# Shadowfear36/SegHiero

Hardware: AMD Instinct MI355X
Metric: images/sec at 512x512 (ResNet-50 2-level), full train step (higher is better)
Workload: dtype f32 (convolutions: exact 3-way bf16 split of every fp32 operand, 6 bf16 MFMA products, f32 accumulate; rest plain f32)

## Files before the change

### include/seghiero_hip.h

```cpp
#ifndef SEGHIERO_HIP_H
#define SEGHIERO_HIP_H
#include <stdint.h>
#ifdef __cplusplus
extern "C" {
#endif

#define SH_OK 0
#define SH_EINVAL (-1)
#define SH_ELAUNCH (-2)
#define SH_EUNSUPPORTED (-3)

int sh_abi_version(void);
int sh_conv_tile_rows(void);

int sh_nchw_to_nhwc(const float* x, float* y, int N, int C, int H, int W, int Cpad, void* stream);
int sh_nhwc_to_nchw(const float* x, float* y, int N, int C, int H, int W, int Cpad, void* stream);

int sh_ingest_image_u8(const uint8_t* rgb, float* out, const uint8_t* flip, int N, int H, int W,
                       const float* mean3_host, const float* std3_host, void* stream);
int sh_resize_bilinear_coeffs(int in_size, int out_size, int* bounds, int* kk, int kk_capacity);
int sh_resize_bilinear_u8(const uint8_t* src, uint8_t* tmp, uint8_t* dst, int N, int H, int W, int Ho, int Wo,
                          const int* bounds_x, const int* kk_x, int ksize_x, const int* bounds_y, const int* kk_y,
                          int ksize_y, void* stream);
int sh_ingest_mask(const void* mask, int is_i64, uint8_t* out, const uint8_t* flip, int N, int Hs, int Ws, int H,
                   int W, void* stream);

int sh_conv_fprop(const float* x, int ldx, const float* w, const float* bias, float* y, int ldy,
                  float* stat_partials, int N, int H, int W, int Cin, int Cout, int KH, int KW,
                  int stride, int pad, int dil, void* stream);
int sh_conv_dgrad(const float* dy, int lddy, const float* w, const float* addend, int ldadd,
                  float* dx, int lddx, int N, int H, int W, int Cin, int Cout, int KH, int KW,
                  int stride, int pad, int dil, int mode, void* stream);
int64_t sh_conv_wgrad_workspace(int N, int H, int W, int Cin, int Cout, int KH, int KW,
                                int stride, int pad, int dil);
int sh_conv_wgrad(const float* x, int ldx, const float* dy, int lddy, float* dw, float* workspace,
                  int N, int H, int W, int Cin, int Cout, int KH, int KW, int stride, int pad,
                  int dil, void* stream);

int64_t sh_conv_x6_workspace(int which , int N, int H, int W, int Cin, int Cout, int KH, int KW,
                             int stride, int pad, int dil, int dgrad_mode);
int sh_conv_fprop_x6(const float* x, int ldx, const float* w, const float* bias, float* y, int ldy,
                     float* stat_partials, int N, int H, int W, int Cin, int Cout, int KH, int KW,
                     int stride, int pad, int dil, float* workspace, int64_t workspace_bytes, int act_flags, void* stream);
int sh_conv_fprop_x6_act(const float* x, int ldx, const float* w, const float* scale, const float* shift,
                         const float* residual, int ldr, int relu, float* out, int ldo, int N, int H, int W,
                         int Cin, int Cout, int KH, int KW, int stride, int pad, int dil, void* stream);
int sh_conv_fprop_x6_aff(const float* x, int ldx, const float* in_scale, const float* in_shift, const float* w,
                         const float* bias, float* y, int ldy, float* stat_partials, int N, int H, int W, int Cin, int Cout,
                         int KH, int KW, int stride, int pad, int dil, float* workspace, int64_t workspace_bytes, int act_flags,
                         void* stream);
int sh_conv1x1_grouped_fprop_x6(int ngroups, const float* const* x, const int* ldx, const float* const* in_scale,
                                const float* const* in_shift, const float* const* w, float* y, int ldy,
                                float* stat_partials, int N, int H, int W, int Cin, int Cout, void* stream);
int sh_weight_transpose(const float* w, float* wt, int Cout, int KH, int KW, int Cin, void* stream);
#define SH_WT_MAX 40
int sh_weight_transpose_multi(int n, const float* const* w, float* const* wt, const int* cout, const int* taps,
                              const int* cin, void* stream);
int sh_conv_dgrad_x6(const float* dy, int lddy, const float* wt, const float* addend, int ldadd,
                     float* dx, int lddx, int N, int H, int W, int Cin, int Cout, int KH, int KW,
                     int stride, int pad, int dil, int mode, float* workspace, int64_t workspace_bytes,
                     void* stream);
int sh_conv_dgrad_x6_bnb(const float* dy, int lddy, const float* wt, const float* addend, int ldadd, float* g, int ldg,
                         const float* y_prev, int ldyp, const float* out_prev, int ldop, const float* mean,
                         const float* invstd, const float* scale, const float* shift, int relu, float* stat_partials,
                         int N, int H, int W, int Cin, int Cout,
                         int KH, int KW, int stride, int pad, int dil, float* workspace, int64_t workspace_bytes, int act_flags,
                         void* stream);
int sh_conv_dgrad_x6_lin(const float* g, int ldg, const float* y, int ldy, const float* lin, const float* wt, const float* addend,
                         int ldadd, float* dx, int lddx, const float* y_prev, int ldyp, const float* mean, const float* invstd,
                         const float* scale, const float* shift, int relu, float* stat_partials, int N, int H, int W, int Cin,
                         int Cout, float* workspace, int64_t workspace_bytes, int act_flags, void* stream);
int sh_conv_wgrad_x6_lin(const float* x, int ldx, const float* in_scale, const float* in_shift, const float* g, int ldg,
                         const float* y, int ldy, const float* lin, float* dw, float* workspace, int N, int H, int W, int Cin,
                         int Cout, int KH, int KW, int stride, int pad, int dil, int act_flags, void* stream);
int64_t sh_conv_wgrad_x6_workspace(int N, int H, int W, int Cin, int Cout, int KH, int KW,
                                   int stride, int pad, int dil);
int sh_conv_wgrad_x6(const float* x, int ldx, const float* dy, int lddy, float* dw, float* workspace,
                     int N, int H, int W, int Cin, int Cout, int KH, int KW, int stride, int pad,
                     int dil, int act_flags, void* stream);
int sh_conv_wgrad_x6_aff(const float* x, int ldx, const float* in_scale, const float* in_shift, const float* dy, int lddy,
                         float* dw, float* workspace, int N, int H, int W, int Cin, int Cout, int KH, int KW,
                         int stride, int pad, int dil, int act_flags, void* stream);

int sh_dw_partials(int N, int H, int W);
int sh_dw_tile_rows(void);
int sh_dwconv_fprop(const float* x, int ldx, const float* in_scale, const float* in_shift, const float* w, float* y, int ldy,
                    float* stat_partials, int N, int H, int W, int C, int dil, int act_flags, void* stream);
int sh_dwconv_dgrad(const float* dy, int lddy, const float* y_lin, int ldyl, const float* lin, const float* w, float* dx, int lddx,
                    int N, int H, int W, int C, int dil, int accumulate, int act_flags, void* stream);
int sh_dwconv_dgrad_bnb(const float* dy, int lddy, const float* y_lin, int ldyl, const float* lin, const float* w, float* g, int ldg,
                        const float* y_prev, int ldyp, const float* mean, const float* invstd, const float* scale, const float* shift,
                        float* stat_partials, int N, int H, int W, int C, int dil, int act_flags, void* stream);
int sh_dwconv_wgrad(const float* x, int ldx, const float* in_scale, const float* in_shift, const float* dy, int lddy,
                    const float* y_lin, int ldyl, const float* lin, float* dw_partials, float* dw, int N, int H, int W, int C, int dil,
                    int act_flags, void* stream);

int sh_bn_finalize(const float* partials, int n_partials, int C, double count, const float* gamma,
                   const float* beta, float eps, float momentum, float* running_mean,
                   float* running_var, float* mean, float* invstd, float* scale, float* shift,
                   int rows_per_partial, int partials_ld, void* stream);
int sh_bn_finalize_scaled(const float* partials, int n_partials, int C, double count, const float* chan_mul,
                          int chan_stride, const float* gamma, const float* beta, float eps, float momentum,
                          float* running_mean, float* running_var, float* mean, float* invstd, float* scale,
                          float* shift, float* isy, int rows_per_partial, void* stream);
int sh_bn_finalize_multi(int k, const float* partials, int n_partials, int C, double count, int rows_per_partial,
                         int partials_ld, const int* partials_col, const float* const* gamma, const float* const* beta,
                         float* const* running_mean, float* const* running_var, float* const* mean, float* const* invstd,
                         float* const* scale, float* const* shift, const float* const* chan_mul, int chan_stride,
                         float* const* isy, float eps, float momentum, void* stream);
int sh_dw_center_wgrad(const float* dgamma, const float* gamma, const float* isy, const float* w, float eps, float* dw,
                       int C, const float* g, int ldg, const float* x, int ldx, const float* mean_x, int64_t M, void* stream);
int sh_bn_fold_partials(const float* partials, int n_partials, int C, double count, int rows_per_partial, int chunk,
                        float* out, void* stream);
int sh_bn_reduce_partials(const float* partials, int n_partials, int C, double count, int rows_per_partial, double* sq,
                          void* stream);
int sh_bn_finalize_sq(const double* sq, int C, const float* gamma, const float* beta, float eps,
                      float momentum, float* running_mean, float* running_var, float* mean, float* invstd,
                      float* scale, float* shift, void* stream);
int sh_bn_bwd_finalize_sq(const double* local_sq, const double* global_sq, int C, float* dgamma,
                          float* dbeta, float* c1, float* c2, const float* gamma, const float* invstd, const float* mean,
                          float* lin, void* stream);
int sh_bn_eval_coefs(const float* gamma, const float* beta, const float* running_mean,
                     const float* running_var, float eps, int C, float* scale, float* shift, void* stream);
int sh_stats_partials_count(int64_t M);
int sh_stats_tile_rows(void);
int sh_channel_stats(const float* y, int ldy, int64_t M, int C, float* partials, void* stream);
int sh_bn_act(const float* y, int ldy, const float* scale, const float* shift, const float* residual,
              int ldr, const float* res_scale, const float* res_shift, float* out, int ldo, int64_t M, int C, int relu,
              uint8_t* relu_mask, int act_flags, void* stream);
int sh_bn_bwd_reduce(const float* dout, int lddo, const float* out, int ldo, const float* y, int ldy,
                     const float* mean, const float* invstd, const float* scale, const float* shift,
                     float* partials, int64_t M, int C, int relu, float* g_out, int ldg, int act_flags, void* stream);
int sh_bn_bwd_finalize(const float* partials, int n_partials, int C, const float* gamma,
                       const float* invstd, double count, float* dgamma, float* dbeta, float* c1,
                       float* c2, const float* mean, float* lin, void* stream);
int sh_bn_bwd_apply(const float* dout, int lddo, const float* out, int ldo, const float* y, int ldy,
                    const float* mean, const float* invstd, const float* scale, const float* shift,
                    const float* gamma, const float* c1, const float* c2, float* dy, int lddy, float* dres,
                    int lddres, int64_t M, int C, int relu, int act_flags, void* stream);

int sh_maxpool_fwd(const float* x, const float* in_scale, const float* in_shift, float* y, uint8_t* argmax, int N, int H,
                   int W, int C, int act_flags, void* stream);
int sh_maxpool_bwd(const uint8_t* argmax, const float* dy, float* dx, int N, int H, int W, int C, void* stream);
int sh_avgpool_fwd(const float* x, int ldx, float* y, int N, int HW, int C, void* stream);
int sh_avgpool_bwd(const float* dy, float* dx, int lddx, int N, int HW, int C, float scale, int accumulate, void* stream);
int sh_broadcast_hw(const float* x, float* y, int ldy, int N, int HW, int C, void* stream);
int sh_sum_hw(const float* dy, int lddy, float* dx, int N, int HW, int C, void* stream);
int sh_bilinear_fwd(const float* x, int ldx, float* y, int ldy, int N, int h, int w, int H, int W, int C, int act_flags, void* stream);
int64_t sh_bilinear_bwd_workspace(int N, int h, int w, int C);
int sh_bilinear_bwd(const float* dy, int lddy, float* dx, int lddx, int N, int h, int w, int H, int W, int C, float* workspace,
                    int64_t workspace_bytes, void* stream);
int sh_l2norm_fwd(const float* x, float* y, float* norm, int64_t M, int C, void* stream);
int sh_l2norm_bwd(const float* dy, const float* y, const float* norm, float* dx, int64_t M, int C, void* stream);

int sh_hiera2_partials(int N, int H, int W);
int sh_label_counts(const uint8_t* labels, const int* buckets_host, int n_fine, int n_coarse, int64_t total, int64_t* counts,
                    void* stream);
int sh_hiera2_loss_fwd(const float* logits, int ldl, const uint8_t* labels, const int* buckets_host, int n_fine,
                       int n_coarse, double* sums, float* loss_out, float* partials, uint8_t* coarse_out,
                       int N, int h, int w, int H, int W, float* grad_out, int64_t grad_out_bytes, int ldg,
                       const int64_t* norm_counts, void* stream);
int64_t sh_loss_bwd_workspace(int N, int H, int W, int lddl);
int sh_hiera2_loss_bwd(const float* logits, int ldl, const uint8_t* labels, const int* buckets_host, int n_fine,
                       int n_coarse, const double* sums, const float* gscale_dev, float gscale, float* dlogits,
                       int lddl, int N, int h, int w, int H, int W, float* workspace, int64_t workspace_bytes,
                       int workspace_has_grad, void* stream);
int sh_ce_loss_fwd(const float* logits, int ldl, const uint8_t* labels, int C, double* sums, float* loss_out,
                   float* partials, int N, int h, int w, int H, int W, float* grad_out, int64_t grad_out_bytes, int ldg,
                   const int64_t* norm_count, void* stream);
int sh_ce_loss_bwd(const float* logits, int ldl, const uint8_t* labels, int C, const double* sums,
                   const float* gscale_dev, float gscale, float* dlogits, int lddl, int N, int h, int w, int H,
                   int W, float* workspace, int64_t workspace_bytes, int workspace_has_grad,
                   void* stream);
int sh_labels_to_u8(const int64_t* in, uint8_t* out, int64_t n, void* stream);
int64_t sh_triplet_workspace(int64_t M);
int sh_triplet_fwd(const float* emb, const uint8_t* labels, const uint64_t* masks, const uint64_t* anchor_ok,
                   int max_triplet, float margin, float* out, void* workspace, int N, int h, int w, int D, int H,
                   int W, void* stream);
int sh_triplet_bwd(const float* emb, const void* workspace, const float* out, const float* gscale_dev, float gscale,
                   float* demb, int N, int h, int w, int D, void* stream);
int sh_combine_loss(const float* main_loss, const float* trip_out, const float* ready_count, float factor,
                    float loss_weight, float* out, void* stream);
int sh_hiera3_loss_fwd(const float* logits, int ldl, const uint8_t* labels, const int* f2m_host, const int* f2h_host,
                       int n_fine, int n_mid, int n_high, double* sums, float* loss_out, float* partials, float* probs,
                       uint8_t* mid_out, uint8_t* high_out, int N, int h, int w, int H, int W, float* grad_out,
                       int64_t grad_out_bytes, int ldg, void* stream);
int64_t sh_rmi_workspace(int N, int C, int H, int W);
int64_t sh_rmi_values_offset(int N, int C, int H, int W);
int sh_rmi_loss(const float* probs, const uint8_t* labels, const int* f2m_host, const int* f2h_host, int n_fine, int n_mid,
                int n_high, void* workspace, float* rmi_out, float* dprob, int N, int H, int W, void* stream);
int sh_hiera3_loss_bwd(const float* logits, int ldl, const uint8_t* labels, const int* f2m_host, const int* f2h_host,
                       int n_fine, int n_mid, int n_high, const double* sums, const float* dprob, float rmi_coef,
                       const float* gscale_dev, float gscale, float* dlogits, int lddl, int N, int h, int w, int H, int W,
                       float* workspace, int64_t workspace_bytes, int workspace_has_grad, const float* probs, void* stream);
int sh_scalar_axpy(const float* a, const float* b, float alpha, float* out, void* stream);

int sh_pixel_metrics(const float* logits, int ldl, const uint8_t* labels, int n_fine, long long* counts,
                     int N, int h, int w, int H, int W, void* stream);

#define SH_SGD_MAX 48
int sh_sgd_step(int n_tensors, float* const* w, const float* const* g, float* const* v, const int64_t* numel,
                float lr, float momentum, float weight_decay, int first_step, float gscale, void* stream);

int sh_fill(float* p, float v, int64_t n, void* stream);
int sh_axpy(float* y, const float* x, float a, int64_t n, void* stream);
int sh_copy(void* dst, const void* src, int64_t bytes, void* stream);

int sh_weights_to_bf16_multi(int n, const float* const* w, void* const* wb, void* const* wtb, const int* cout, const int* taps,
                             const int* cin, void* stream);
int sh_conv_fprop_b16(const void* x, int ldx, const float* in_scale, const float* in_shift, const void* w_bf16, const float* bias,
                      void* y, int ldy, float* stat_partials, int N, int H, int W, int Cin, int Cout, int KH, int KW, int stride,
                      int pad, int dil, float* workspace, int64_t workspace_bytes, int act_flags, void* stream);
int sh_conv1x1_grouped_fprop_b16(int ngroups, const void* const* x, const int* ldx, const float* const* in_scale,
                                 const float* const* in_shift, const void* const* w_bf16, void* y, int ldy, float* stat_partials,
                                 int N, int H, int W, int Cin, int Cout, int act_flags, void* stream);
int sh_conv_dgrad_b16(const void* dy, int lddy, const void* y_lin, int ldyl, const float* lin, const void* wt_bf16, const void* addend,
                      int ldadd, void* dx, int lddx, const void* y_prev, int ldyp, const void* out_prev, int ldop, const float* mean,
                      const float* invstd, const float* scale, const float* shift, int relu, float* stat_partials, int N, int H,
                      int W, int Cin, int Cout, int KH, int KW, int stride, int pad, int dil, float* workspace,
                      int64_t workspace_bytes, int act_flags, void* stream);
int sh_conv_wgrad_b16(const void* x, int ldx, const float* in_scale, const float* in_shift, const void* dy, int lddy, const void* y_lin,
                      int ldyl, const float* lin, float* dw, float* workspace, int N, int H, int W, int Cin, int Cout, int KH, int KW,
                      int stride, int pad, int dil, int act_flags, void* stream);

int sh_comm_unique_id(void* id128);
int sh_comm_init(const void* id128, int world, int rank, void** comm_out);
int sh_comm_destroy(void* comm);
int sh_comm_all_reduce(void* comm, void* buf, int64_t count, int dtype, int op, void* stream);
int sh_comm_all_reduce_async(void* comm, void* buf, int64_t count, int dtype, int op, void* producer_stream);
int sh_comm_wait(void* comm, void* consumer_stream);
int sh_comm_broadcast(void* comm, void* buf, int64_t bytes, int root, void* stream);

#ifdef __cplusplus
}
#endif
#endif
```

### seghiero_amd/csrc/common.h

```cpp
#pragma once
#include <hip/hip_runtime.h>
#include <stdint.h>
#include "../../include/seghiero_hip.h"

typedef float f32x4 __attribute__((ext_vector_type(4)));
typedef float f32x16 __attribute__((ext_vector_type(16)));

#define SH_WAVE 64

static inline int sh_launch_status() {
    hipError_t e = hipGetLastError();
    return e == hipSuccess ? SH_OK : SH_ELAUNCH;
}

static inline int64_t sh_cdiv(int64_t a, int64_t b) { return (a + b - 1) / b; }

__device__ __forceinline__ float wave_sum(float v) {
#pragma unroll
    for (int o = 32; o > 0; o >>= 1) v += __shfl_xor(v, o, 64);
    return v;
}
__device__ __forceinline__ double wave_sum_d(double v) {
#pragma unroll
    for (int o = 32; o > 0; o >>= 1) v += __shfl_xor(v, o, 64);
    return v;
}

__device__ __forceinline__ unsigned xcd_remap(unsigned bid, unsigned nblk) {
    const unsigned q = nblk >> 3, r = nblk & 7u, xcd = bid & 7u, loc = bid >> 3;
    const unsigned base = xcd < r ? xcd * (q + 1) : r * (q + 1) + (xcd - r) * q;
    return base + loc;
}

__device__ __forceinline__ f32x4 ld4(const float* p) { return *reinterpret_cast<const f32x4*>(p); }
__device__ __forceinline__ void st4(float* p, f32x4 v) { *reinterpret_cast<f32x4*>(p) = v; }

typedef unsigned int sh_u32x2 __attribute__((ext_vector_type(2)));
__device__ __forceinline__ f32x4 bf16x4_to_f32(sh_u32x2 v) {
    return f32x4{__uint_as_float(v[0] << 16), __uint_as_float(v[0] & 0xffff0000u), __uint_as_float(v[1] << 16), __uint_as_float(v[1] & 0xffff0000u)};
}
__device__ __forceinline__ unsigned f32_to_bf16_rne(float f) {
    const unsigned u = __float_as_uint(f);
    return (f != f) ? ((u >> 16) | 0x40u) : ((u + 0x7fffu + ((u >> 16) & 1u)) >> 16);
}
__device__ __forceinline__ sh_u32x2 f32_to_bf16x4(f32x4 v) {
    return sh_u32x2{f32_to_bf16_rne(v[0]) | (f32_to_bf16_rne(v[1]) << 16), f32_to_bf16_rne(v[2]) | (f32_to_bf16_rne(v[3]) << 16)};
}
__device__ __forceinline__ f32x4 lda4(const float* base, long long idx, int bf) {
    if (bf) return bf16x4_to_f32(*reinterpret_cast<const sh_u32x2*>(reinterpret_cast<const unsigned short*>(base) + idx));
    return ld4(base + idx);
}
__device__ __forceinline__ unsigned quad_mask_bits(f32x4 v) {
    return (v[0] > 0.f ? 1u : 0u) | (v[1] > 0.f ? 2u : 0u) | (v[2] > 0.f ? 4u : 0u) | (v[3] > 0.f ? 8u : 0u);
}
__device__ __forceinline__ f32x4 quad_mask_load(const void* base, long long byte_idx) {
    const unsigned b = reinterpret_cast<const unsigned char*>(base)[byte_idx];
    return f32x4{(b & 1u) ? 1.f : 0.f, (b & 2u) ? 1.f : 0.f, (b & 4u) ? 1.f : 0.f, (b & 8u) ? 1.f : 0.f};
}
__device__ __forceinline__ void sta4(float* base, long long idx, f32x4 v, int bf) {
    if (bf) *reinterpret_cast<sh_u32x2*>(reinterpret_cast<unsigned short*>(base) + idx) = f32_to_bf16x4(v);
    else st4(base + idx, v);
}

struct sh_f8 { f32x4 lo, hi; };
typedef unsigned int sh_u32x4 __attribute__((ext_vector_type(4)));
__device__ __forceinline__ sh_f8 lda8(const float* base, long long idx, int bf) {
    sh_f8 r;
    if (bf) {
        const sh_u32x4 v = *reinterpret_cast<const sh_u32x4*>(reinterpret_cast<const unsigned short*>(base) + idx);
        r.lo = bf16x4_to_f32(sh_u32x2{v[0], v[1]}); r.hi = bf16x4_to_f32(sh_u32x2{v[2], v[3]});
    } else { r.lo = ld4(base + idx); r.hi = ld4(base + idx + 4); }
    return r;
}
__device__ __forceinline__ void sta8(float* base, long long idx, const sh_f8& v, int bf) {
    if (bf) {
        const sh_u32x2 a = f32_to_bf16x4(v.lo), b = f32_to_bf16x4(v.hi);
        *reinterpret_cast<sh_u32x4*>(reinterpret_cast<unsigned short*>(base) + idx) = sh_u32x4{a[0], a[1], b[0], b[1]};
    } else { st4(base + idx, v.lo); st4(base + idx + 4, v.hi); }
}
```

### seghiero_amd/csrc/dwconv.hip

```cpp
#include "common.h"
#include <stdlib.h>

#define DW_PIX 64
#define DW_CH 64

__device__ __forceinline__ f32x4 dw_in(const float* p, const float* isc, const float* ish, int c) {
    f32x4 v = ld4(p);
    if (isc != nullptr) {
        v = v * ld4(isc + c) + ld4(ish + c);
        v[0] = fmaxf(v[0], 0.f); v[1] = fmaxf(v[1], 0.f); v[2] = fmaxf(v[2], 0.f); v[3] = fmaxf(v[3], 0.f);
    }
    return v;
}

struct DwBnb { const float* y; long long ldy; const float* mean; const float* invstd; const float* scale; const float* shift; float* partials;
               int y_bf; };
struct DwBnbC { f32x4 scale, shift, mean, invstd; };
__device__ __forceinline__ DwBnbC dw_bnb_coefs(const DwBnb& b, int c, bool cok) {
    DwBnbC k; k.scale = k.shift = k.mean = k.invstd = f32x4{0.f, 0.f, 0.f, 0.f};
    if (b.y != nullptr && cok) { k.scale = ld4(b.scale + c); k.shift = ld4(b.shift + c); k.mean = ld4(b.mean + c); k.invstd = ld4(b.invstd + c); }
    return k;
}
__device__ __forceinline__ f32x4 dw_bnb_apply(const DwBnbC& k, f32x4 yv, f32x4 dx, f32x4& sg, f32x4& sq) {
    const f32x4 a = yv * k.scale + k.shift;
#pragma unroll
    for (int j = 0; j < 4; ++j) if (!(a[j] > 0.f)) dx[j] = 0.f;
    sg += dx;
    sq += dx * ((yv - k.mean) * k.invstd);
    return dx;
}
__device__ __forceinline__ f32x4 dw_bnb_apply(const DwBnb& b, long long m, int c, f32x4 dx, f32x4& sg, f32x4& sq) {
    const f32x4 yv = lda4(b.y, m * b.ldy + c, b.y_bf);
    const f32x4 a = yv * ld4(b.scale + c) + ld4(b.shift + c);
#pragma unroll
    for (int j = 0; j < 4; ++j) if (!(a[j] > 0.f)) dx[j] = 0.f;
    sg += dx;
    sq += dx * ((yv - ld4(b.mean + c)) * ld4(b.invstd + c));
    return dx;
}
__device__ __forceinline__ void dw_bnb_store(const DwBnb& b, float (*red)[64], f32x4 sg, f32x4 sq, long long pidx, int C, int c0, int t, int cq, int pl) {
#pragma unroll
    for (int pass = 0; pass < 2; ++pass) {
        __syncthreads();
#pragma unroll
        for (int j = 0; j < 4; ++j) red[pl][cq * 4 + j] = pass == 0 ? sg[j] : sq[j];
        __syncthreads();
        if (t < 64 && c0 + t < C) {
            float a = 0.f;
#pragma unroll
            for (int k = 0; k < 16; ++k) a += red[k][t];
            b.partials[(pidx * 2 + pass) * C + c0 + t] = a;
        }
    }
}

extern "C" int sh_dw_partials(int N, int H, int W) { return (int)sh_cdiv((long long)N * H * W, DW_PIX); }
extern "C" int sh_dw_tile_rows(void) { return DW_PIX; }

template <int MODE>
__global__ __launch_bounds__(256) void dwconv_kernel(const float* __restrict__ x, long long ldx, const float* __restrict__ w,
                                                     float* __restrict__ y, long long ldy, float* __restrict__ partials,
                                                     int H, int W, int C, int dil, long long M, int accumulate,
                                                     const float* __restrict__ isc, const float* __restrict__ ish, const DwBnb bnb) {
    __shared__ float ws[9][DW_CH];
    __shared__ float red[16][DW_CH];
    __shared__ float colmean[DW_CH];
    const int t = threadIdx.x, cq = t & 15, pl = t >> 4;
    const int c0 = blockIdx.y * DW_CH;
    for (int i = t; i < 9 * DW_CH; i += 256) {
        const int tap = i / DW_CH, cc = i % DW_CH;
        const int src_tap = MODE == 0 ? tap : 8 - tap;
        ws[tap][cc] = (c0 + cc < C) ? w[(long long)(c0 + cc) * 9 + src_tap] : 0.f;
    }
    __syncthreads();
    const int c = c0 + cq * 4;
    const bool cok = c < C;
    f32x4 s = {0.f, 0.f, 0.f, 0.f};
    f32x4 bsg = s, bsq = s;
    f32x4 kept[DW_PIX / 16];
    bool kept_ok[DW_PIX / 16];
    const bool tap_row_ok = dil < H, tap_col_ok = dil < W;
#pragma unroll
    for (int it = 0; it < DW_PIX / 16; ++it) {
        const long long m = (long long)blockIdx.x * DW_PIX + it * 16 + pl;
        kept_ok[it] = false;
        kept[it] = f32x4{0.f, 0.f, 0.f, 0.f};
        if (m < M && cok) {
            const int ow = (int)(m % W);
            const long long r = m / W;
            const int oh = (int)(r % H);
            const long long n = r / H;
            f32x4 acc = {0.f, 0.f, 0.f, 0.f};
#pragma unroll
            for (int kh = 0; kh < 3; ++kh) {
                if (kh != 1 && !tap_row_ok) continue;
                const int ih = oh + (kh - 1) * dil;
                if ((unsigned)ih >= (unsigned)H) continue;
#pragma unroll
                for (int kw = 0; kw < 3; ++kw) {
                    if (kw != 1 && !tap_col_ok) continue;
                    const int iw = ow + (kw - 1) * dil;
                    if ((unsigned)iw >= (unsigned)W) continue;
                    const f32x4 v = dw_in(x + ((n * H + ih) * W + iw) * ldx + c, isc, ish, c);
                    const f32x4 wv = ld4(&ws[kh * 3 + kw][cq * 4]);
                    acc += v * wv;
                }
            }
            if (MODE == 1 && accumulate) acc += ld4(y + m * ldy + c);
            if (MODE == 1 && bnb.y != nullptr) acc = dw_bnb_apply(bnb, m, c, acc, bsg, bsq);
            st4(y + m * ldy + c, acc);
            s += acc; kept[it] = acc; kept_ok[it] = true;
        }
    }
    if (MODE == 1 && bnb.y != nullptr) dw_bnb_store(bnb, red, bsg, bsq, blockIdx.x, C, c0, t, cq, pl);
    if (MODE == 0 && partials != nullptr) {
        const long long left = M - (long long)blockIdx.x * DW_PIX;
        const float nvalid = (float)(left < DW_PIX ? left : DW_PIX);
#pragma unroll
        for (int j = 0; j < 4; ++j) red[pl][cq * 4 + j] = s[j];
        __syncthreads();
        float colsum = 0.f;
        if (t < DW_CH) {
#pragma unroll
            for (int k = 0; k < 16; ++k) colsum += red[k][t];
            colmean[t] = colsum / nvalid;
        }
        __syncthreads();
        f32x4 q = {0.f, 0.f, 0.f, 0.f};
        const f32x4 mu = ld4(&colmean[cq * 4]);
#pragma unroll
        for (int it = 0; it < DW_PIX / 16; ++it)
            if (kept_ok[it]) { const f32x4 dv = kept[it] - mu; q += dv * dv; }
#pragma unroll
        for (int j = 0; j < 4; ++j) red[pl][cq * 4 + j] = q[j];
        __syncthreads();
        if (t < DW_CH && c0 + t < C) {
            float m2 = 0.f;
#pragma unroll
            for (int k = 0; k < 16; ++k) m2 += red[k][t];
            partials[((long long)blockIdx.x * 2 + 0) * C + c0 + t] = colsum;
            partials[((long long)blockIdx.x * 2 + 1) * C + c0 + t] = m2;
        }
    }
}

#define DT 8
template <int MODE>
__global__ __launch_bounds__(256) void dwconv_tile_kernel(const float* __restrict__ x, long long ldx, const float* __restrict__ w,
                                                          float* __restrict__ y, long long ldy, float* __restrict__ partials,
                                                          int H, int W, int C, int accumulate,
                                                          const float* __restrict__ isc, const float* __restrict__ ish, const DwBnb bnb) {
    __shared__ __attribute__((aligned(16))) float xs[(DT + 2) * (DT + 2)][DW_CH];
    __shared__ float ws[9][DW_CH];
    __shared__ float red[16][DW_CH];
    __shared__ float colmean[DW_CH];
    const int t = threadIdx.x, cq = t & 15, pl = t >> 4;
    const unsigned nch = (unsigned)((C + DW_CH - 1) / DW_CH);
    const unsigned tile = blockIdx.x / nch;
    const int c0 = (int)(blockIdx.x % nch) * DW_CH;
    const int tiles_x = W / DT, tiles_y = H / DT;
    const int tx = tile % tiles_x, ty = (tile / tiles_x) % tiles_y;
    const long long n = tile / (tiles_x * tiles_y);
    for (int i = t; i < 9 * DW_CH; i += 256) {
        const int tap = i / DW_CH, cc = i % DW_CH;
        ws[tap][cc] = (c0 + cc < C) ? w[(long long)(c0 + cc) * 9 + (MODE == 0 ? tap : 8 - tap)] : 0.f;
    }
    const int c = c0 + cq * 4;
    const bool cok = c < C;
    for (int i = pl; i < (DT + 2) * (DT + 2); i += 16) {
        const int hy = i / (DT + 2), hx = i - hy * (DT + 2);
        const int iy = ty * DT + hy - 1, ix = tx * DT + hx - 1;
        f32x4 v = {0.f, 0.f, 0.f, 0.f};
        if (cok && (unsigned)iy < (unsigned)H && (unsigned)ix < (unsigned)W) v = dw_in(x + ((n * H + iy) * W + ix) * ldx + c, isc, ish, c);
        st4(&xs[i][cq * 4], v);
    }
    __syncthreads();
    f32x4 s = {0.f, 0.f, 0.f, 0.f};
    f32x4 bsg = s, bsq = s;
    f32x4 kept[4];
#pragma unroll
    for (int it = 0; it < 4; ++it) {
        const int pidx = it * 16 + pl, py = pidx / DT, px = pidx - py * DT;
        f32x4 acc = {0.f, 0.f, 0.f, 0.f};
#pragma unroll
        for (int kh = 0; kh < 3; ++kh)
#pragma unroll
            for (int kw = 0; kw < 3; ++kw)
                acc += ld4(&xs[(py + kh) * (DT + 2) + px + kw][cq * 4]) * ld4(&ws[kh * 3 + kw][cq * 4]);
        kept[it] = acc;
        if (cok) {
            const long long m = (n * H + ty * DT + py) * W + tx * DT + px;
            float* dst = y + m * ldy + c;
            if (MODE == 1 && accumulate) acc += ld4(dst);
            if (MODE == 1 && bnb.y != nullptr) acc = dw_bnb_apply(bnb, m, c, acc, bsg, bsq);
            st4(dst, acc);
        }
        s += kept[it];
    }
    if (MODE == 1 && bnb.y != nullptr) dw_bnb_store(bnb, red, bsg, bsq, tile, C, c0, t, cq, pl);
    if (MODE == 0 && partials != nullptr) {
#pragma unroll
        for (int j = 0; j < 4; ++j) red[pl][cq * 4 + j] = s[j];
        __syncthreads();
        float colsum = 0.f;
        if (t < DW_CH) {
#pragma unroll
            for (int k = 0; k < 16; ++k) colsum += red[k][t];
            colmean[t] = colsum / (float)(DT * DT);
        }
        __syncthreads();
        f32x4 q = {0.f, 0.f, 0.f, 0.f};
        const f32x4 mu = ld4(&colmean[cq * 4]);
#pragma unroll
        for (int it = 0; it < 4; ++it) { const f32x4 dv = kept[it] - mu; q += dv * dv; }
#pragma unroll
        for (int j = 0; j < 4; ++j) red[pl][cq * 4 + j] = q[j];
        __syncthreads();
        if (t < DW_CH && c0 + t < C) {
            float m2 = 0.f;
#pragma unroll
            for (int k = 0; k < 16; ++k) m2 += red[k][t];
            partials[((long long)tile * 2 + 0) * C + c0 + t] = colsum;
            partials[((long long)tile * 2 + 1) * C + c0 + t] = m2;
        }
    }
}
__global__ __launch_bounds__(256) void dwconv_wgrad_tile_kernel(const float* __restrict__ x, long long ldx, const float* __restrict__ dy,
                                                               long long lddy, float* __restrict__ partials, int H, int W, int C,
                                                               long long ntiles, const float* __restrict__ isc, const float* __restrict__ ish) {
    __shared__ __attribute__((aligned(16))) float xs[(DT + 2) * (DT + 2)][DW_CH];
    __shared__ float red[16][DW_CH];
    const int t = threadIdx.x, cq = t & 15, pl = t >> 4;
    const unsigned nch = (unsigned)((C + DW_CH - 1) / DW_CH), group = blockIdx.x / nch, ngroups = gridDim.x / nch;
    const int c0 = (int)(blockIdx.x % nch) * DW_CH, c = c0 + cq * 4;
    const bool cok = c < C;
    const int tiles_x = W / DT, tiles_y = H / DT;
    f32x4 acc[9];
#pragma unroll
    for (int k = 0; k < 9; ++k) acc[k] = f32x4{0.f, 0.f, 0.f, 0.f};
    for (long long tile = group; tile < ntiles; tile += ngroups) {
        const int tx = (int)(tile % tiles_x), ty = (int)((tile / tiles_x) % tiles_y);
        const long long n = tile / (tiles_x * tiles_y);
        __syncthreads();
        for (int i = pl; i < (DT + 2) * (DT + 2); i += 16) {
            const int hy = i / (DT + 2), hx = i - hy * (DT + 2);
            const int iy = ty * DT + hy - 1, ix = tx * DT + hx - 1;
            f32x4 v = {0.f, 0.f, 0.f, 0.f};
            if (cok && (unsigned)iy < (unsigned)H && (unsigned)ix < (unsigned)W) v = dw_in(x + ((n * H + iy) * W + ix) * ldx + c, isc, ish, c);
            st4(&xs[i][cq * 4], v);
        }
        __syncthreads();
        if (cok) {
#pragma unroll
            for (int it = 0; it < 4; ++it) {
                const int pidx = it * 16 + pl, py = pidx / DT, px = pidx - py * DT;
                const f32x4 g = ld4(dy + ((n * H + ty * DT + py) * W + tx * DT + px) * lddy + c);
#pragma unroll
                for (int kh = 0; kh < 3; ++kh)
#pragma unroll
                    for (int kw = 0; kw < 3; ++kw) acc[kh * 3 + kw] += g * ld4(&xs[(py + kh) * (DT + 2) + px + kw][cq * 4]);
            }
        }
    }
#pragma unroll
    for (int k = 0; k < 9; ++k) {
        __syncthreads();
#pragma unroll
        for (int j = 0; j < 4; ++j) red[pl][cq * 4 + j] = acc[k][j];
        __syncthreads();
        if (t < DW_CH) {
            float a = 0.f;
#pragma unroll
            for (int r = 0; r < 16; ++r) a += red[r][t];
            if (c0 + t < C) partials[((long long)group * 9 + k) * C + c0 + t] = a;
        }
    }
}

#define DWR 10
__device__ __forceinline__ int dw_slot(int base, int k) { const int i = base + k; return i >= DWR ? i - DWR : i; }
struct DwWalk {
    int n, ty, c0, c, tiles_x, tiles_y;
    bool cok;
    long long t0, t1;
};
__device__ __forceinline__ void dw_walk_init(DwWalk& q, int H, int W, int C, int N, int cq) {
    const unsigned nch = (unsigned)((C + DW_CH - 1) / DW_CH), nb = gridDim.x / nch, k = blockIdx.x / nch;
    q.c0 = (int)(blockIdx.x % nch) * DW_CH; q.c = q.c0 + cq * 4; q.cok = q.c < C;
    q.tiles_x = W / DT; q.tiles_y = H / DT;
    const long long T = (long long)N * q.tiles_y * q.tiles_x;
    q.t0 = T * k / nb; q.t1 = T * (k + 1) / nb;
}
__device__ __forceinline__ void dw_walk_strip(DwWalk& q, long long strip) { q.ty = (int)(strip % q.tiles_y); q.n = (int)(strip / q.tiles_y); }
__device__ __forceinline__ bool dw_walk_inside(const DwWalk& q, int H, int W, int hy, int ix) {
    return q.cok && (unsigned)(q.ty * DT + hy - 1) < (unsigned)H && (unsigned)ix < (unsigned)W;
}
__device__ __forceinline__ f32x4 dw_walk_fetch(const float* __restrict__ x, long long ldx, const DwWalk& q, int H, int W, int hy, int ix, int bf = 0) {
    f32x4 v = {0.f, 0.f, 0.f, 0.f};
    if (dw_walk_inside(q, H, W, hy, ix)) v = lda4(x, (((long long)q.n * H + q.ty * DT + hy - 1) * W + ix) * ldx + q.c, bf);
    return v;
}
struct DwLin { const float* y; long long ldy; const float* lin; int y_bf; };
struct DwLinC { f32x4 a, b, mu, d; };
__device__ __forceinline__ DwLinC dw_lin_coefs(const DwLin& L, int C, int c, bool cok) {
    DwLinC k; k.a = k.b = k.mu = k.d = f32x4{0.f, 0.f, 0.f, 0.f};
    if (L.lin != nullptr && cok) { k.a = ld4(L.lin + c); k.b = ld4(L.lin + C + c); k.mu = ld4(L.lin + 2 * C + c); k.d = ld4(L.lin + 3 * C + c); }
    return k;
}
__device__ __forceinline__ f32x4 dw_lin_eval(f32x4 g, f32x4 y, bool inside, const DwLinC& k) {
    f32x4 r;
#pragma unroll
    for (int e = 0; e < 4; ++e) r[e] = inside ? fmaf(y[e] - k.mu[e], k.b[e], fmaf(g[e], k.a[e], k.d[e])) : 0.f;
    return r;
}
__device__ __forceinline__ f32x4 dw_walk_act(f32x4 v, bool aff, bool inside, const f32x4& sc, const f32x4& sh) {
    if (aff && inside) {
        v = v * sc + sh;
        v[0] = fmaxf(v[0], 0.f); v[1] = fmaxf(v[1], 0.f); v[2] = fmaxf(v[2], 0.f); v[3] = fmaxf(v[3], 0.f);
    }
    return v;
}
template <int LIN, int XBF, int YBF>
__device__ __forceinline__ void dw_walk_prologue(float (*xs)[DWR][DW_CH], const float* __restrict__ x, long long ldx, bool aff,
                                                 const f32x4& sc, const f32x4& sh, const DwWalk& q, int H, int W, int tx, int rb, int pl, int cq,
                                                 const DwLin* L = nullptr, const DwLinC* lc = nullptr) {
    for (int i = pl; i < (DT + 2) * (DT + 2); i += 16) {
        const int hy = i / (DT + 2), hx = i - hy * (DT + 2), ix = tx * DT + hx - 1;
        f32x4 v = dw_walk_fetch(x, ldx, q, H, W, hy, ix, XBF);
        if constexpr (LIN) v = dw_lin_eval(v, dw_walk_fetch(L->y, L->ldy, q, H, W, hy, ix, YBF), dw_walk_inside(q, H, W, hy, ix), *lc);
        st4(&xs[hy][dw_slot(rb, hx)][cq * 4], dw_walk_act(v, aff, dw_walk_inside(q, H, W, hy, ix), sc, sh));
    }
}
template <int MODE, int LIN, int BNB, int BF>
__global__ __launch_bounds__(256, (LIN && BNB) ? 2 : 3) void dwconv_walk_kernel(const float* __restrict__ x, long long ldx, const float* __restrict__ w,
                                                          float* __restrict__ y, long long ldy, float* __restrict__ partials,
                                                          int N, int H, int W, int C, int accumulate,
                                                          const float* __restrict__ isc, const float* __restrict__ ish, const DwBnb bnb,
                                                          const DwLin lin, int af) {
    __shared__ __attribute__((aligned(16))) float xs[DT + 2][DWR][DW_CH];
    __shared__ float red[16][DW_CH];
    __shared__ float colmean[DW_CH];
    static_assert(MODE == 1 || (LIN == 0 && BNB == 0), "the loader / epilogue hooks belong to the dgrad");
    constexpr int x_bf = MODE == 0 ? (BF & 1) : 0, y_bf = MODE == 0 ? (BF & 2) : 0, ly_bf = MODE == 1 ? (BF & 1) : 0, by_bf = MODE == 1 ? (BF & 2) : 0;
    constexpr bool has_lin = LIN != 0;
    (void)af;
    const int t = threadIdx.x, cq = t & 15, pl = t >> 4;
    DwWalk q;
    dw_walk_init(q, H, W, C, N, cq);
    const DwLinC lc = dw_lin_coefs(lin, C, q.c, q.cok);
    const DwBnbC bc = dw_bnb_coefs(bnb, q.c, q.cok);
    f32x4 wr[9];
#pragma unroll
    for (int k = 0; k < 9; ++k)
#pragma unroll
        for (int j = 0; j < 4; ++j) wr[k][j] = q.cok ? w[(long long)(q.c + j) * 9 + (MODE == 0 ? k : 8 - k)] : 0.f;
    const bool aff = MODE == 0 && isc != nullptr;
    f32x4 sc = {0.f, 0.f, 0.f, 0.f}, sh = sc;
    if (aff && q.cok) { sc = ld4(isc + q.c); sh = ld4(ish + q.c); }
    int tx = (int)(q.t0 % q.tiles_x), rb = (tx * DT) % DWR;
    for (long long tile = q.t0; tile < q.t1; ++tile) {
        if (tile == q.t0 || tx == 0) {
            dw_walk_strip(q, tile / q.tiles_x);
            dw_walk_prologue<LIN, x_bf, ly_bf>(xs, x, ldx, aff, sc, sh, q, H, W, tx, rb, pl, cq, &lin, &lc);
            __syncthreads();
        }
        f32x4 nx[5];
        [[maybe_unused]] f32x4 ny[5];
        const bool more = tx + 1 < q.tiles_x && tile + 1 < q.t1;
        if (more) {
#pragma unroll
            for (int it = 0; it < 5; ++it) {
                const int i = it * 16 + pl;
                nx[it] = dw_walk_fetch(x, ldx, q, H, W, i >> 3, tx * DT + 9 + (i & 7), x_bf);
                if constexpr (has_lin) ny[it] = dw_walk_fetch(lin.y, lin.ldy, q, H, W, i >> 3, tx * DT + 9 + (i & 7), ly_bf);
            }
        }
        f32x4 s = {0.f, 0.f, 0.f, 0.f};
        f32x4 bsg = s, bsq = s;
        f32x4 kept[4];
#pragma unroll
        for (int it = 0; it < 4; ++it) {
            const int pidx = it * 16 + pl, py = pidx / DT, px = pidx - py * DT;
            f32x4 acc = {0.f, 0.f, 0.f, 0.f};
#pragma unroll
            for (int kh = 0; kh < 3; ++kh)
#pragma unroll
                for (int kw = 0; kw < 3; ++kw)
                    acc += ld4(&xs[py + kh][dw_slot(rb, px + kw)][cq * 4]) * wr[kh * 3 + kw];
            kept[it] = acc;
            if (q.cok) {
                const long long m = (((long long)q.n * H + q.ty * DT + py) * W + tx * DT + px);
                float* dst = y + m * ldy + q.c;
                if (MODE == 1 && accumulate) acc += ld4(dst);
                if constexpr (BNB) acc = dw_bnb_apply(bc, lda4(bnb.y, m * bnb.ldy + q.c, by_bf), acc, bsg, bsq);
                if (MODE == 0) sta4(y, m * ldy + q.c, acc, y_bf);
                else st4(dst, acc);
            }
            s += kept[it];
        }
        if constexpr (BNB) dw_bnb_store(bnb, red, bsg, bsq, tile, C, q.c0, t, cq, pl);
        if (MODE == 0 && partials != nullptr) {
#pragma unroll
            for (int j = 0; j < 4; ++j) red[pl][cq * 4 + j] = s[j];
            __syncthreads();
            float colsum = 0.f;
            if (t < DW_CH) {
#pragma unroll
                for (int k = 0; k < 16; ++k) colsum += red[k][t];
                colmean[t] = colsum / (float)(DT * DT);
            }
            __syncthreads();
            f32x4 qq = {0.f, 0.f, 0.f, 0.f};
            const f32x4 mu = ld4(&colmean[cq * 4]);
#pragma unroll
            for (int it = 0; it < 4; ++it) { const f32x4 dv = kept[it] - mu; qq += dv * dv; }
#pragma unroll
            for (int j = 0; j < 4; ++j) red[pl][cq * 4 + j] = qq[j];
            __syncthreads();
            if (t < DW_CH && q.c0 + t < C) {
                float m2 = 0.f;
#pragma unroll
                for (int k = 0; k < 16; ++k) m2 += red[k][t];
                partials[(tile * 2 + 0) * C + q.c0 + t] = colsum;
                partials[(tile * 2 + 1) * C + q.c0 + t] = m2;
            }
        }
        __syncthreads();
        if (more) {
#pragma unroll
            for (int it = 0; it < 5; ++it) {
                const int i = it * 16 + pl;
                const bool inside = dw_walk_inside(q, H, W, i >> 3, tx * DT + 9 + (i & 7));
                f32x4 v = nx[it];
                if constexpr (has_lin) v = dw_lin_eval(v, ny[it], inside, lc);
                st4(&xs[i >> 3][dw_slot(rb, i & 7)][cq * 4], dw_walk_act(v, aff, inside, sc, sh));
            }
            __syncthreads();
        }
        if (++tx == q.tiles_x) { tx = 0; rb = 0; } else rb = rb >= 2 ? rb - 2 : rb + 8;
    }
}
template <int LIN, int BF>
__global__ __launch_bounds__(256, 3) void dwconv_wgrad_walk_kernel(const float* __restrict__ x, long long ldx, const float* __restrict__ dy,
                                                               long long lddy, float* __restrict__ partials, int N, int H, int W, int C,
                                                               const float* __restrict__ isc, const float* __restrict__ ish, const DwLin lin) {
    constexpr int x_bf = BF & 1, ly_bf = BF & 2;
    __shared__ __attribute__((aligned(16))) float xs[DT + 2][DWR][DW_CH];
    __shared__ float red[16][DW_CH];
    const int t = threadIdx.x, cq = t & 15, pl = t >> 4;
    DwWalk q;
    dw_walk_init(q, H, W, C, N, cq);
    constexpr bool has_lin = LIN != 0;
    const DwLinC lc = dw_lin_coefs(lin, C, q.c, q.cok);
    f32x4 acc[9];
#pragma unroll
    for (int k = 0; k < 9; ++k) acc[k] = f32x4{0.f, 0.f, 0.f, 0.f};
    const bool aff = isc != nullptr;
    f32x4 sc = {0.f, 0.f, 0.f, 0.f}, sh = sc;
    if (aff && q.cok) { sc = ld4(isc + q.c); sh = ld4(ish + q.c); }
    f32x4 g[4];
    [[maybe_unused]] f32x4 gy[4];
    auto fetch_dy = [&](long long tile) {
        const long long strip = tile / q.tiles_x;
        const int ftx = (int)(tile - strip * q.tiles_x), fty = (int)(strip % q.tiles_y);
        const long long fn = strip / q.tiles_y;
#pragma unroll
        for (int it = 0; it < 4; ++it) {
            const int pidx = it * 16 + pl, py = pidx / DT, px = pidx - py * DT;
            const long long m = (fn * H + fty * DT + py) * W + ftx * DT + px;
            g[it] = q.cok ? ld4(dy + m * lddy + q.c) : f32x4{0.f, 0.f, 0.f, 0.f};
            if constexpr (has_lin) gy[it] = q.cok ? lda4(lin.y, m * lin.ldy + q.c, ly_bf) : f32x4{0.f, 0.f, 0.f, 0.f};
        }
    };
    if (q.t0 < q.t1) fetch_dy(q.t0);
    int tx = (int)(q.t0 % q.tiles_x), rb = (tx * DT) % DWR;
    for (long long tile = q.t0; tile < q.t1; ++tile) {
        if (tile == q.t0 || tx == 0) {
            dw_walk_strip(q, tile / q.tiles_x);
            dw_walk_prologue<0, x_bf, 0>(xs, x, ldx, aff, sc, sh, q, H, W, tx, rb, pl, cq);
            __syncthreads();
        }
        f32x4 nx[5];
        const bool more = tx + 1 < q.tiles_x && tile + 1 < q.t1;
        if (more) {
#pragma unroll
            for (int it = 0; it < 5; ++it) {
                const int i = it * 16 + pl;
                nx[it] = dw_walk_fetch(x, ldx, q, H, W, i >> 3, tx * DT + 9 + (i & 7), x_bf);
            }
        }
#pragma unroll
        for (int it = 0; it < 4; ++it) {
            const int pidx = it * 16 + pl, py = pidx / DT, px = pidx - py * DT;
            f32x4 gv = g[it];
            if constexpr (has_lin) gv = dw_lin_eval(g[it], gy[it], q.cok, lc);
#pragma unroll
            for (int kh = 0; kh < 3; ++kh)
#pragma unroll
                for (int kw = 0; kw < 3; ++kw)
                    acc[kh * 3 + kw] += gv * ld4(&xs[py + kh][dw_slot(rb, px + kw)][cq * 4]);
#pragma unroll
            for (int k = 0; k < 9; ++k) asm volatile("" : "+v"(acc[k]));
        }
        if (tile + 1 < q.t1) fetch_dy(tile + 1);
        __syncthreads();
        if (more) {
#pragma unroll
            for (int it = 0; it < 5; ++it) {
                const int i = it * 16 + pl;
                st4(&xs[i >> 3][dw_slot(rb, i & 7)][cq * 4],
                    dw_walk_act(nx[it], aff, dw_walk_inside(q, H, W, i >> 3, tx * DT + 9 + (i & 7)), sc, sh));
            }
            __syncthreads();
        }
        if (++tx == q.tiles_x) { tx = 0; rb = 0; } else rb = rb >= 2 ? rb - 2 : rb + 8;
    }
#pragma unroll
    for (int k = 0; k < 9; ++k) {
        __syncthreads();
#pragma unroll
        for (int j = 0; j < 4; ++j) red[pl][cq * 4 + j] = acc[k][j];
        __syncthreads();
        if (t < DW_CH) {
            float a = 0.f;
#pragma unroll
            for (int r = 0; r < 16; ++r) a += red[r][t];
            if (q.c0 + t < C) partials[((long long)(blockIdx.x / ((C + DW_CH - 1) / DW_CH)) * 9 + k) * C + q.c0 + t] = a;
        }
    }
}

__global__ __launch_bounds__(256) void dwconv_wgrad_kernel(const float* __restrict__ x, long long ldx, const float* __restrict__ dy,
                                                           long long lddy, float* __restrict__ partials, int H, int W, int C,
                                                           int dil, long long M, const float* __restrict__ isc, const float* __restrict__ ish) {
    __shared__ float red[16][DW_CH];
    const int t = threadIdx.x, cq = t & 15, pl = t >> 4;
    const int c0 = blockIdx.y * DW_CH, c = c0 + cq * 4;
    const bool cok = c < C;
    f32x4 acc[9];
#pragma unroll
    for (int k = 0; k < 9; ++k) acc[k] = f32x4{0.f, 0.f, 0.f, 0.f};
    const long long nchunks = (M + DW_PIX - 1) / DW_PIX;
    for (long long chunk = blockIdx.x; chunk < nchunks; chunk += gridDim.x) {
#pragma unroll
        for (int it = 0; it < DW_PIX / 16; ++it) {
            const long long m = chunk * DW_PIX + it * 16 + pl;
            if (m < M && cok) {
                const int ow = (int)(m % W);
                const long long r = m / W;
                const int oh = (int)(r % H);
                const long long n = r / H;
                const f32x4 g = ld4(dy + m * lddy + c);
#pragma unroll
                for (int kh = 0; kh < 3; ++kh) {
                    const int ih = oh + (kh - 1) * dil;
                    if ((unsigned)ih >= (unsigned)H) continue;
#pragma unroll
                    for (int kw = 0; kw < 3; ++kw) {
                        const int iw = ow + (kw - 1) * dil;
                        if ((unsigned)iw >= (unsigned)W) continue;
                        acc[kh * 3 + kw] += g * dw_in(x + ((n * H + ih) * W + iw) * ldx + c, isc, ish, c);
                    }
                }
            }
        }
    }
#pragma unroll
    for (int k = 0; k < 9; ++k) {
        __syncthreads();
#pragma unroll
        for (int j = 0; j < 4; ++j) red[pl][cq * 4 + j] = acc[k][j];
        __syncthreads();
        if (t < DW_CH) {
            float a = 0.f;
#pragma unroll
            for (int r = 0; r < 16; ++r) a += red[r][t];
            if (c0 + t < C) partials[((long long)blockIdx.x * 9 + k) * C + c0 + t] = a;
        }
    }
}
__global__ __launch_bounds__(256) void dwconv_wgrad_reduce_kernel(const float* __restrict__ partials, float* __restrict__ dw, int P, int C) {
    __shared__ double red[4][64];
    const int t = threadIdx.x, cl = t & 63, g = t >> 6;
    const int col = blockIdx.x * 64 + cl;
    double s = 0;
    if (col < 9 * C)
        for (int p = g; p < P; p += 4) s += (double)partials[(long long)p * 9 * C + col];
    red[g][cl] = s;
    __syncthreads();
    if (t < 64 && col < 9 * C) {
        const int tap = col / C, c = col % C;
        dw[(long long)c * 9 + tap] = (float)((red[0][t] + red[1][t]) + (red[2][t] + red[3][t]));
    }
}

template <typename... A>
static void dw_launch_fprop_walk(int bf, unsigned blocks, hipStream_t st, A... a) {
    switch (bf & 3) {
    case 0: dwconv_walk_kernel<0, 0, 0, 0><<<blocks, 256, 0, st>>>(a...); break;
    case 1: dwconv_walk_kernel<0, 0, 0, 1><<<blocks, 256, 0, st>>>(a...); break;
    case 2: dwconv_walk_kernel<0, 0, 0, 2><<<blocks, 256, 0, st>>>(a...); break;
    default: dwconv_walk_kernel<0, 0, 0, 3><<<blocks, 256, 0, st>>>(a...); break;
    }
}
template <int LIN, int BNB, typename... A>
static void dw_launch_dgrad_walk_bf(int bf, unsigned blocks, hipStream_t st, A... a) {
    switch (bf & 3) {
    case 0: dwconv_walk_kernel<1, LIN, BNB, 0><<<blocks, 256, 0, st>>>(a...); break;
    case 1: dwconv_walk_kernel<1, LIN, BNB, 1><<<blocks, 256, 0, st>>>(a...); break;
    case 2: dwconv_walk_kernel<1, LIN, BNB, 2><<<blocks, 256, 0, st>>>(a...); break;
    default: dwconv_walk_kernel<1, LIN, BNB, 3><<<blocks, 256, 0, st>>>(a...); break;
    }
}
template <typename... A>
static void dw_launch_dgrad_walk(bool lin, bool bnb, int bf, unsigned blocks, hipStream_t st, A... a) {
    if (!lin) bf &= ~1;
    if (!bnb) bf &= ~2;
    if (lin && bnb) dw_launch_dgrad_walk_bf<1, 1>(bf, blocks, st, a...);
    else if (lin) dw_launch_dgrad_walk_bf<1, 0>(bf, blocks, st, a...);
    else if (bnb) dw_launch_dgrad_walk_bf<0, 1>(bf, blocks, st, a...);
    else dw_launch_dgrad_walk_bf<0, 0>(bf, blocks, st, a...);
}
template <typename... A>
static void dw_launch_wgrad_walk(bool lin, int bf, unsigned blocks, hipStream_t st, A... a) {
    if (!lin) bf &= ~2;
    if (lin) {
        switch (bf & 3) {
        case 0: dwconv_wgrad_walk_kernel<1, 0><<<blocks, 256, 0, st>>>(a...); break;
        case 1: dwconv_wgrad_walk_kernel<1, 1><<<blocks, 256, 0, st>>>(a...); break;
        case 2: dwconv_wgrad_walk_kernel<1, 2><<<blocks, 256, 0, st>>>(a...); break;
        default: dwconv_wgrad_walk_kernel<1, 3><<<blocks, 256, 0, st>>>(a...); break;
        }
    } else if (bf & 1) dwconv_wgrad_walk_kernel<0, 1><<<blocks, 256, 0, st>>>(a...);
    else dwconv_wgrad_walk_kernel<0, 0><<<blocks, 256, 0, st>>>(a...);
}
static bool dw_walk_on() {
    static const bool on = [] { const char* e = getenv("SEGHIERO_DW_WALK"); return !(e && e[0] == '0'); }();
    return on;
}
static unsigned dw_walk_blocks(int N, int H, int W, int C) { (void)W; (void)C; return (unsigned)(N * (H / DT)); }
static bool dw_args_ok(const void* a, const void* b, const void* c, int N, int H, int W, int C, int dil, int ld1, int ld2) {
    return a && b && c && N > 0 && H > 0 && W > 0 && C > 0 && (C & 3) == 0 && dil > 0 && ld1 >= C && ld2 >= C && !(ld1 & 3) && !(ld2 & 3);
}
extern "C" int sh_dwconv_fprop(const float* x, int ldx, const float* in_scale, const float* in_shift, const float* w, float* y, int ldy,
                               float* stat_partials, int N, int H, int W, int C, int dil, int act_flags, void* stream) {
    if (!dw_args_ok(x, w, y, N, H, W, C, dil, ldx, ldy) || (act_flags & ~3)) return SH_EINVAL;
    if (act_flags && !(dil == 1 && H % DT == 0 && W % DT == 0 && dw_walk_on())) return SH_EUNSUPPORTED;
    if ((in_scale == nullptr) != (in_shift == nullptr) || (((uintptr_t)in_scale | (uintptr_t)in_shift) & 15)) return SH_EINVAL;
    const long long M = (long long)N * H * W;
    dim3 grid((unsigned)sh_cdiv(M, DW_PIX), (unsigned)sh_cdiv(C, DW_CH));
    if (dil == 1 && H % DT == 0 && W % DT == 0 && dw_walk_on())
        dw_launch_fprop_walk(act_flags, dw_walk_blocks(N, H, W, C) * grid.y, (hipStream_t)stream, x, (long long)ldx, w, y, (long long)ldy, stat_partials, N, H, W, C, 0, in_scale,
                             in_shift, DwBnb{}, DwLin{}, act_flags);
    else if (dil == 1 && H % DT == 0 && W % DT == 0)
        dwconv_tile_kernel<0><<<grid.x * grid.y, 256, 0, (hipStream_t)stream>>>(x, ldx, w, y, ldy, stat_partials, H, W, C, 0, in_scale, in_shift, DwBnb{});
    else
        dwconv_kernel<0><<<grid, 256, 0, (hipStream_t)stream>>>(x, ldx, w, y, ldy, stat_partials, H, W, C, dil, M, 0, in_scale, in_shift, DwBnb{});
    return sh_launch_status();
}
static bool dw_lin_args_ok(const float* y_lin, int ldyl, const float* lin, int C) {
    return (lin == nullptr && y_lin == nullptr) || (lin && y_lin && ldyl >= C && !(ldyl & 3) && !(((uintptr_t)y_lin | (uintptr_t)lin) & 15));
}
static int dw_dgrad_any(const float* dy, int lddy, const float* w, float* dx, int lddx, int N, int H, int W, int C, int dil, int accumulate,
                        const DwBnb& bnb, void* stream, const DwLin lin = DwLin{}) {
    const long long M = (long long)N * H * W;
    dim3 grid((unsigned)sh_cdiv(M, DW_PIX), (unsigned)sh_cdiv(C, DW_CH));
    if (dil == 1 && H % DT == 0 && W % DT == 0 && dw_walk_on())
        dw_launch_dgrad_walk(lin.lin != nullptr, bnb.y != nullptr, (lin.y_bf ? 1 : 0) | (bnb.y_bf ? 2 : 0), dw_walk_blocks(N, H, W, C) * grid.y, (hipStream_t)stream,
                             dy, (long long)lddy, w, dx, (long long)lddx, (float*)nullptr, N, H, W, C, accumulate, (const float*)nullptr, (const float*)nullptr, bnb, lin, 0);
    else if (lin.lin != nullptr || bnb.y_bf) return SH_EUNSUPPORTED;
    else if (dil == 1 && H % DT == 0 && W % DT == 0)
        dwconv_tile_kernel<1><<<grid.x * grid.y, 256, 0, (hipStream_t)stream>>>(dy, lddy, w, dx, lddx, nullptr, H, W, C, accumulate, nullptr, nullptr, bnb);
    else
        dwconv_kernel<1><<<grid, 256, 0, (hipStream_t)stream>>>(dy, lddy, w, dx, lddx, nullptr, H, W, C, dil, M, accumulate, nullptr, nullptr, bnb);
    return sh_launch_status();
}
extern "C" int sh_dwconv_dgrad(const float* dy, int lddy, const float* y_lin, int ldyl, const float* lin, const float* w, float* dx, int lddx,
                               int N, int H, int W, int C, int dil, int accumulate, int act_flags, void* stream) {
    if (!dw_args_ok(dy, w, dx, N, H, W, C, dil, lddy, lddx) || !dw_lin_args_ok(y_lin, ldyl, lin, C) || (act_flags & ~1)) return SH_EINVAL;
    return dw_dgrad_any(dy, lddy, w, dx, lddx, N, H, W, C, dil, accumulate, DwBnb{}, stream, DwLin{y_lin, ldyl, lin, act_flags & 1});
}
extern "C" int sh_dwconv_dgrad_bnb(const float* dy, int lddy, const float* y_lin, int ldyl, const float* lin, const float* w, float* g, int ldg,
                                   const float* y_prev, int ldyp, const float* mean, const float* invstd, const float* scale, const float* shift,
                                   float* stat_partials, int N, int H, int W, int C, int dil, int act_flags, void* stream) {
    if (!dw_args_ok(dy, w, g, N, H, W, C, dil, lddy, ldg) || !y_prev || !mean || !invstd || !scale || !shift || !stat_partials ||
        !dw_lin_args_ok(y_lin, ldyl, lin, C) || (act_flags & ~3)) return SH_EINVAL;
    if (ldyp < C || (ldyp & 3) || (((uintptr_t)y_prev | (uintptr_t)mean | (uintptr_t)invstd | (uintptr_t)scale | (uintptr_t)shift) & 15)) return SH_EINVAL;
    return dw_dgrad_any(dy, lddy, w, g, ldg, N, H, W, C, dil, 0, DwBnb{y_prev, ldyp, mean, invstd, scale, shift, stat_partials, (act_flags >> 1) & 1}, stream,
                        DwLin{y_lin, ldyl, lin, act_flags & 1});
}
extern "C" int sh_dwconv_wgrad(const float* x, int ldx, const float* in_scale, const float* in_shift, const float* dy, int lddy,
                               const float* y_lin, int ldyl, const float* lin, float* dw_partials, float* dw, int N, int H, int W, int C, int dil,
                               int act_flags, void* stream) {
    if (!dw_args_ok(x, dy, dw, N, H, W, C, dil, ldx, lddy) || !dw_partials || !dw_lin_args_ok(y_lin, ldyl, lin, C) || (act_flags & ~3)) return SH_EINVAL;
    if (act_flags && !(dil == 1 && H % DT == 0 && W % DT == 0 && dw_walk_on())) return SH_EUNSUPPORTED;
    if ((in_scale == nullptr) != (in_shift == nullptr) || (((uintptr_t)in_scale | (uintptr_t)in_shift) & 15)) return SH_EINVAL;
    const long long M = (long long)N * H * W;
    int P = (int)sh_cdiv(M, DW_PIX);
    const int cap = (int)sh_cdiv(1024, sh_cdiv(C, DW_CH));
    if (P > cap) P = cap < 1 ? 1 : cap;
    dim3 grid((unsigned)P, (unsigned)sh_cdiv(C, DW_CH));
    if (dil == 1 && H % DT == 0 && W % DT == 0 && dw_walk_on()) {
        P = (int)dw_walk_blocks(N, H, W, C);
        dw_launch_wgrad_walk(lin != nullptr, act_flags & 3, (unsigned)P * grid.y, (hipStream_t)stream, x, (long long)ldx, dy, (long long)lddy, dw_partials, N, H, W, C, in_scale,
                             in_shift, DwLin{y_lin, ldyl, lin, (act_flags >> 1) & 1});
    } else if (lin != nullptr) return SH_EUNSUPPORTED;
    else if (dil == 1 && H % DT == 0 && W % DT == 0)
        dwconv_wgrad_tile_kernel<<<grid.x * grid.y, 256, 0, (hipStream_t)stream>>>(x, ldx, dy, lddy, dw_partials, H, W, C, M / (DT * DT), in_scale, in_shift);
    else
        dwconv_wgrad_kernel<<<grid, 256, 0, (hipStream_t)stream>>>(x, ldx, dy, lddy, dw_partials, H, W, C, dil, M, in_scale, in_shift);
    int rc = sh_launch_status();
    if (rc != SH_OK) return rc;
    dwconv_wgrad_reduce_kernel<<<(unsigned)sh_cdiv(9 * C, 64), 256, 0, (hipStream_t)stream>>>(dw_partials, dw, P, C);
    return sh_launch_status();
}
```

### seghiero_amd/csrc/loss_common.h

```cpp
#pragma once
#include "common.h"

#define IGN 255
#define LOSS_PIX_PER_BLOCK 1024

struct Lerp { int i0, i1; float w0, w1; };
__device__ __forceinline__ Lerp lerp_src(int dst, float scale, int in) {
    float s = scale * ((float)dst + 0.5f) - 0.5f;
    s = s < 0.f ? 0.f : s;
    Lerp L;
    L.i0 = (int)s;
    if (L.i0 > in - 1) L.i0 = in - 1;
    L.i1 = L.i0 + (L.i0 < in - 1 ? 1 : 0);
    L.w1 = s - (float)L.i0;
    L.w0 = 1.f - L.w1;
    return L;
}
__device__ __forceinline__ void contrib_range(int i, float inv_scale, int out, int& lo, int& hi) {
    lo = (int)floorf(((float)i - 0.5f) * inv_scale - 0.5f);
    hi = (int)ceilf(((float)i + 1.5f) * inv_scale - 0.5f);
    if (i == 0) lo = 0;
    lo = lo < 0 ? 0 : lo;
    hi = hi > out - 1 ? out - 1 : hi;
}
__device__ __forceinline__ float sigmoidf_(float x) { return 1.f / (1.f + expf(-x)); }

template <int MAXC>
__device__ __forceinline__ void fetch_logits(const float* __restrict__ base, long long ldl, int w, const Lerp& ly, const Lerp& lx,
                                             bool identity, int C, float (&z)[MAXC]) {
    const bool vec = (MAXC % 4 == 0) && (ldl & 3) == 0 && ldl >= ((C + 3) & ~3) && ((uintptr_t)base & 15) == 0;
    if (identity) {
        const float* p = base + ((long long)ly.i0 * w + lx.i0) * ldl;
        if (vec) {
#pragma unroll
            for (int j = 0; j < MAXC; j += 4) {
                if (j < C) {
                    const f32x4 v = ld4(p + j);
#pragma unroll
                    for (int e = 0; e < 4; ++e) z[j + e] = j + e < C ? v[e] : 0.f;
                } else {
#pragma unroll
                    for (int e = 0; e < 4; ++e) z[j + e] = 0.f;
                }
            }
            return;
        }
#pragma unroll
        for (int j = 0; j < MAXC; ++j) z[j] = j < C ? p[j] : 0.f;
    } else {
        const float* p00 = base + ((long long)ly.i0 * w + lx.i0) * ldl;
        const float* p01 = base + ((long long)ly.i0 * w + lx.i1) * ldl;
        const float* p10 = base + ((long long)ly.i1 * w + lx.i0) * ldl;
        const float* p11 = base + ((long long)ly.i1 * w + lx.i1) * ldl;
        if (vec) {
#pragma unroll
            for (int j = 0; j < MAXC; j += 4) {
                if (j < C) {
                    const f32x4 a = ld4(p00 + j), b = ld4(p01 + j), c = ld4(p10 + j), d = ld4(p11 + j);
#pragma unroll
                    for (int e = 0; e < 4; ++e)
                        z[j + e] = j + e < C ? ly.w0 * (lx.w0 * a[e] + lx.w1 * b[e]) + ly.w1 * (lx.w0 * c[e] + lx.w1 * d[e]) : 0.f;
                } else {
#pragma unroll
                    for (int e = 0; e < 4; ++e) z[j + e] = 0.f;
                }
            }
            return;
        }
#pragma unroll
        for (int j = 0; j < MAXC; ++j)
            z[j] = j < C ? ly.w0 * (lx.w0 * p00[j] + lx.w1 * p01[j]) + ly.w1 * (lx.w0 * p10[j] + lx.w1 * p11[j]) : 0.f;
    }
}

int sh_launch_resize_adjoint_gather(const float* gfull, float* dlogits, int lddl, int N, int h, int w, int H, int W, hipStream_t st);
int sh_launch_gather_from_grad(const float* gfull, const float* gscale_dev, float gscale, float* dlogits, int lddl, int N, int h, int w,
                               int H, int W, hipStream_t st);

template <int MAXC, bool GRAD>
__device__ __forceinline__ float softmax_ce(const float (&z)[MAXC], int off, int n, int tgt, float coef, float (&g)[MAXC]) {
    float mx = -INFINITY;
#pragma unroll
    for (int j = 0; j < MAXC; ++j) if (j >= off && j < off + n) mx = fmaxf(mx, z[j]);
    float se = 0.f;
#pragma unroll
    for (int j = 0; j < MAXC; ++j) if (j >= off && j < off + n) se += expf(z[j] - mx);
    const float lse = mx + logf(se);
    float zt = 0.f;
#pragma unroll
    for (int j = 0; j < MAXC; ++j) {
        if (j >= off && j < off + n) {
            if (j - off == tgt) zt = z[j];
            if (GRAD) g[j] += coef * (expf(z[j] - lse) - (j - off == tgt ? 1.f : 0.f));
        }
    }
    return lse - zt;
}

template <int NV>
__device__ __forceinline__ void block_reduce_store(float (&v)[NV], float* __restrict__ partials) {
    __shared__ float red[NV][4];
    const int t = threadIdx.x;
#pragma unroll
    for (int j = 0; j < NV; ++j) v[j] = wave_sum(v[j]);
    if ((t & 63) == 0) {
#pragma unroll
        for (int j = 0; j < NV; ++j) red[j][t >> 6] = v[j];
    }
    __syncthreads();
    if (t < 8) partials[(long long)blockIdx.x * 8 + t] = t < NV ? (red[t][0] + red[t][1]) + (red[t][2] + red[t][3]) : 0.f;
}
```

### seghiero_amd/csrc/pool_resample.hip

```cpp
#include "common.h"

static inline unsigned grid_for(long long work_items, int block = 256, int cap = 8192) {
    long long g = sh_cdiv(work_items, block);
    if (g > cap) g = cap;
    if (g < 1) g = 1;
    return (unsigned)g;
}
#define GRID_STRIDE(i, total) for (long long i = (long long)blockIdx.x * 256 + threadIdx.x; i < (total); i += (long long)gridDim.x * 256)

__global__ __launch_bounds__(256) void maxpool_fwd_kernel(const float* __restrict__ x, float* __restrict__ y, unsigned* __restrict__ argmax,
                                                          int H, int W, int Ho, int Wo, int C4, long long total,
                                                          const float* __restrict__ isc, const float* __restrict__ ish, int af) {
    GRID_STRIDE(i, total) {
        const int c = (int)(i % C4);
        long long q = i / C4;
        const int ow = (int)(q % Wo); q /= Wo;
        const int oh = (int)(q % Ho);
        const long long n = q / Ho;
        f32x4 m = {-INFINITY, -INFINITY, -INFINITY, -INFINITY};
        unsigned idx = 0;
#pragma unroll
        for (int kh = 0; kh < 3; ++kh) {
            const int ih = oh * 2 - 1 + kh;
            if ((unsigned)ih >= (unsigned)H) continue;
#pragma unroll
            for (int kw = 0; kw < 3; ++kw) {
                const int iw = ow * 2 - 1 + kw;
                if ((unsigned)iw >= (unsigned)W) continue;
                f32x4 v = lda4(x, (((n * H + ih) * W + iw) * C4 + c) * 4, af & 1);
                if (isc != nullptr) {
                    v = v * ld4(isc + 4 * c) + ld4(ish + 4 * c);
                    v[0] = fmaxf(v[0], 0.f); v[1] = fmaxf(v[1], 0.f); v[2] = fmaxf(v[2], 0.f); v[3] = fmaxf(v[3], 0.f);
                }
#pragma unroll
                for (int j = 0; j < 4; ++j)
                    if (v[j] > m[j] || v[j] != v[j]) { m[j] = v[j]; idx = (idx & ~(0xffu << (8 * j))) | ((unsigned)(kh * 3 + kw) << (8 * j)); }
            }
        }
        sta4(y, i * 4, m, af & 2);
        if (argmax != nullptr) argmax[i] = idx;
    }
}
__global__ __launch_bounds__(256) void maxpool_bwd_kernel(const unsigned* __restrict__ argmax, const float* __restrict__ dy,
                                                          float* __restrict__ dx, int H, int W, int Ho, int Wo, int C4,
                                                          long long total) {
    GRID_STRIDE(i, total) {
        const int c = (int)(i % C4);
        long long q = i / C4;
        const int iw = (int)(q % W); q /= W;
        const int ih = (int)(q % H);
        const long long n = q / H;
        f32x4 acc = {0.f, 0.f, 0.f, 0.f};
        for (int oh = (ih + 1) / 2 - 1; oh <= (ih + 1) / 2; ++oh) {
            if (oh < 0 || oh >= Ho) continue;
            const int kh = ih - (oh * 2 - 1);
            if (kh < 0 || kh > 2) continue;
            for (int ow = (iw + 1) / 2 - 1; ow <= (iw + 1) / 2; ++ow) {
                if (ow < 0 || ow >= Wo) continue;
                const int kw = iw - (ow * 2 - 1);
                if (kw < 0 || kw > 2) continue;
                const long long o = ((n * Ho + oh) * Wo + ow) * C4 + c;
                const unsigned idx = argmax[o], want = (unsigned)(kh * 3 + kw);
                const f32x4 g = ld4(dy + o * 4);
#pragma unroll
                for (int j = 0; j < 4; ++j)
                    if (((idx >> (8 * j)) & 0xffu) == want) acc[j] += g[j];
            }
        }
        st4(dx + i * 4, acc);
    }
}
extern "C" int sh_maxpool_fwd(const float* x, const float* in_scale, const float* in_shift, float* y, uint8_t* argmax, int N, int H, int W,
                              int C, int act_flags, void* stream) {
    if (!x || !y || N <= 0 || H <= 0 || W <= 0 || C <= 0 || (C & 3) || ((uintptr_t)argmax & 3)) return SH_EINVAL;
    if ((in_scale == nullptr) != (in_shift == nullptr) || (((uintptr_t)in_scale | (uintptr_t)in_shift) & 15)) return SH_EINVAL;
    const int Ho = (H + 2 - 3) / 2 + 1, Wo = (W + 2 - 3) / 2 + 1;
    const long long total = (long long)N * Ho * Wo * (C / 4);
    maxpool_fwd_kernel<<<grid_for(total), 256, 0, (hipStream_t)stream>>>(x, y, reinterpret_cast<unsigned*>(argmax), H, W, Ho, Wo, C / 4, total,
                                                                         in_scale, in_shift, act_flags);
    return sh_launch_status();
}
extern "C" int sh_maxpool_bwd(const uint8_t* argmax, const float* dy, float* dx, int N, int H, int W, int C, void* stream) {
    if (!argmax || !dy || !dx || N <= 0 || H <= 0 || W <= 0 || C <= 0 || (C & 3) || ((uintptr_t)argmax & 3)) return SH_EINVAL;
    const int Ho = (H + 2 - 3) / 2 + 1, Wo = (W + 2 - 3) / 2 + 1;
    const long long total = (long long)N * H * W * (C / 4);
    maxpool_bwd_kernel<<<grid_for(total), 256, 0, (hipStream_t)stream>>>(reinterpret_cast<const unsigned*>(argmax), dy, dx, H, W, Ho, Wo, C / 4, total);
    return sh_launch_status();
}

__global__ __launch_bounds__(256) void avgpool_fwd_kernel(const float* __restrict__ x, long long ldx, float* __restrict__ y,
                                                          int HW, int C, float inv) {
    __shared__ double red[4][64];
    const int t = threadIdx.x, cl = t & 63, g = t >> 6, c = blockIdx.y * 64 + cl;
    const long long n = blockIdx.x;
    double s = 0;
    if (c < C) {
        const float* base = x + n * HW * ldx + c;
        int r = g;
        for (; r + 28 < HW; r += 32) {
            float v[8];
#pragma unroll
            for (int u = 0; u < 8; ++u) v[u] = base[(long long)(r + 4 * u) * ldx];
            s += (double)(((v[0] + v[1]) + (v[2] + v[3])) + ((v[4] + v[5]) + (v[6] + v[7])));
        }
        float part = 0.f;
        for (; r < HW; r += 4) part += base[(long long)r * ldx];
        s += part;
    }
    red[g][cl] = s;
    __syncthreads();
    if (t < 64 && c < C) y[n * C + c] = (float)(((red[0][t] + red[1][t]) + (red[2][t] + red[3][t])) * (double)inv);
}
extern "C" int sh_avgpool_fwd(const float* x, int ldx, float* y, int N, int HW, int C, void* stream) {
    if (!x || !y || N <= 0 || HW <= 0 || C <= 0 || ldx < C) return SH_EINVAL;
    dim3 grid(N, (unsigned)sh_cdiv(C, 64));
    avgpool_fwd_kernel<<<grid, 256, 0, (hipStream_t)stream>>>(x, ldx, y, HW, C, 1.0f / (float)HW);
    return sh_launch_status();
}
extern "C" int sh_sum_hw(const float* dy, int lddy, float* dx, int N, int HW, int C, void* stream) {
    if (!dy || !dx || N <= 0 || HW <= 0 || C <= 0 || lddy < C) return SH_EINVAL;
    dim3 grid(N, (unsigned)sh_cdiv(C, 64));
    avgpool_fwd_kernel<<<grid, 256, 0, (hipStream_t)stream>>>(dy, lddy, dx, HW, C, 1.0f);
    return sh_launch_status();
}
__global__ __launch_bounds__(256) void bcast_kernel(const float* __restrict__ v, float* __restrict__ out, long long ldo, int HW,
                                                    int C, float scale, int accumulate, long long total) {
    GRID_STRIDE(i, total) {
        const int c = (int)(i % C);
        const long long q = i / C, n = q / HW;
        const float val = v[n * C + c] * scale;
        float* dst = out + q * ldo + c;
        *dst = accumulate ? *dst + val : val;
    }
}
extern "C" int sh_avgpool_bwd(const float* dy, float* dx, int lddx, int N, int HW, int C, float scale, int accumulate, void* stream) {
    if (!dy || !dx || N <= 0 || HW <= 0 || C <= 0 || lddx < C) return SH_EINVAL;
    const long long total = (long long)N * HW * C;
    bcast_kernel<<<grid_for(total), 256, 0, (hipStream_t)stream>>>(dy, dx, lddx, HW, C, scale, accumulate, total);
    return sh_launch_status();
}
extern "C" int sh_broadcast_hw(const float* x, float* y, int ldy, int N, int HW, int C, void* stream) {
    return sh_avgpool_bwd(x, y, ldy, N, HW, C, 1.0f, 0, stream);
}

struct Lerp { int i0, i1; float w0, w1; };
__device__ __forceinline__ Lerp lerp_src(int dst, float scale, int in) {
    float s = scale * ((float)dst + 0.5f) - 0.5f;
    s = s < 0.f ? 0.f : s;
    Lerp L;
    L.i0 = (int)s;
    if (L.i0 > in - 1) L.i0 = in - 1;
    L.i1 = L.i0 + (L.i0 < in - 1 ? 1 : 0);
    L.w1 = s - (float)L.i0;
    L.w0 = 1.f - L.w1;
    return L;
}
__global__ __launch_bounds__(256) void bilinear_fwd_kernel(const float* __restrict__ x, long long ldx, float* __restrict__ y,
                                                           long long ldy, int h, int w, int H, int W, int C4, float sy, float sx,
                                                           long long total, int y_bf) {
    GRID_STRIDE(i, total) {
        const int c = (int)(i % C4) * 4;
        long long q = i / C4;
        const int ox = (int)(q % W); q /= W;
        const int oy = (int)(q % H);
        const long long n = q / H;
        const Lerp ly = lerp_src(oy, sy, h), lx = lerp_src(ox, sx, w);
        const float* b = x + n * h * w * ldx + c;
        const f32x4 v00 = ld4(b + ((long long)ly.i0 * w + lx.i0) * ldx), v01 = ld4(b + ((long long)ly.i0 * w + lx.i1) * ldx);
        const f32x4 v10 = ld4(b + ((long long)ly.i1 * w + lx.i0) * ldx), v11 = ld4(b + ((long long)ly.i1 * w + lx.i1) * ldx);
        const f32x4 r = ly.w0 * (lx.w0 * v00 + lx.w1 * v01) + ly.w1 * (lx.w0 * v10 + lx.w1 * v11);
        sta4(y, ((n * H + oy) * W + ox) * ldy + c, r, y_bf);
    }
}
__device__ __forceinline__ void contrib_range(int i, float inv_scale, int out, int& lo, int& hi) {
    lo = (int)floorf(((float)i - 0.5f) * inv_scale - 0.5f) - 1;
    hi = (int)ceilf(((float)i + 1.5f) * inv_scale - 0.5f) + 1;
    if (i == 0) lo = 0;
    lo = lo < 0 ? 0 : lo;
    hi = hi > out - 1 ? out - 1 : hi;
}
__global__ __launch_bounds__(256) void bilinear_bwd_kernel(const float* __restrict__ dy, long long lddy, float* __restrict__ dx,
                                                           long long lddx, int h, int w, int H, int W, int C4, float sy, float sx,
                                                           long long total) {
    GRID_STRIDE(i, total) {
        const int c = (int)(i % C4) * 4;
        long long q = i / C4;
        const int ix = (int)(q % w); q /= w;
        const int iy = (int)(q % h);
        const long long n = q / h;
        int ylo, yhi, xlo, xhi;
        contrib_range(iy, 1.f / sy, H, ylo, yhi);
        contrib_range(ix, 1.f / sx, W, xlo, xhi);
        f32x4 acc = {0.f, 0.f, 0.f, 0.f};
        for (int oy = ylo; oy <= yhi; ++oy) {
            const Lerp ly = lerp_src(oy, sy, h);
            const float wy = (ly.i0 == iy ? ly.w0 : 0.f) + (ly.i1 == iy ? ly.w1 : 0.f);
            if (wy == 0.f) continue;
            const float* row = dy + ((n * H + oy) * W) * lddy + c;
            for (int ox = xlo; ox <= xhi; ++ox) {
                const Lerp lx = lerp_src(ox, sx, w);
                const float wx = (lx.i0 == ix ? lx.w0 : 0.f) + (lx.i1 == ix ? lx.w1 : 0.f);
                if (wx == 0.f) continue;
                acc += (wy * wx) * ld4(row + (long long)ox * lddy);
            }
        }
        st4(dx + ((n * h + iy) * w + ix) * lddx + c, acc);
    }
}
extern "C" int sh_bilinear_fwd(const float* x, int ldx, float* y, int ldy, int N, int h, int w, int H, int W, int C, int act_flags, void* stream) {
    if (!x || !y || N <= 0 || h <= 0 || w <= 0 || H <= 0 || W <= 0 || C <= 0 || (C & 3) || ldx < C || ldy < C || (ldx & 3) || (ldy & 3)) return SH_EINVAL;
    const long long total = (long long)N * H * W * (C / 4);
    bilinear_fwd_kernel<<<grid_for(total), 256, 0, (hipStream_t)stream>>>(x, ldx, y, ldy, h, w, H, W, C / 4, (float)h / (float)H, (float)w / (float)W, total, act_flags & 1);
    return sh_launch_status();
}
__global__ __launch_bounds__(256) void bilinear_bwd_rows_kernel(const float* __restrict__ dy, long long lddy, float* __restrict__ p0,
                                                                float* __restrict__ p1, int h, int w, int H, int W, int C, float sy, float sx) {
    const int t = threadIdx.x, cq = t & 15, il = t >> 4;
    const unsigned nch = (unsigned)((C + 63) / 64), nxb = (unsigned)((w + 15) / 16);
    unsigned b = blockIdx.x;
    const int c = (int)(b % nch) * 64 + cq * 4; b /= nch;
    const int ix = (int)(b % nxb) * 16 + il; b /= nxb;
    const int iy = (int)(b % (unsigned)h);
    const long long n = b / (unsigned)h;
    if (c >= C || ix >= w) return;
    int ylo, yhi, xlo, xhi;
    contrib_range(iy, 1.f / sy, H, ylo, yhi);
    contrib_range(ix, 1.f / sx, W, xlo, xhi);
    f32x4 a0 = {0.f, 0.f, 0.f, 0.f}, a1 = a0;
    for (int oy = ylo; oy <= yhi; ++oy) {
        const Lerp ly = lerp_src(oy, sy, h);
        if (ly.i0 != iy) continue;
        const float wy0 = ly.w0 + (ly.i1 == iy ? ly.w1 : 0.f), wy1 = ly.i1 != iy ? ly.w1 : 0.f;
        const float* row = dy + ((n * H + oy) * W) * lddy + c;
        f32x4 r = {0.f, 0.f, 0.f, 0.f};
        for (int ox0 = xlo; ox0 <= xhi; ox0 += 8) {
            f32x4 v[8];
            float wx[8];
#pragma unroll
            for (int k = 0; k < 8; ++k) {
                const int ox = ox0 + k, oxc = ox <= xhi ? ox : xhi;
                const Lerp lx = lerp_src(oxc, sx, w);
                wx[k] = ox <= xhi ? (lx.i0 == ix ? lx.w0 : 0.f) + (lx.i1 == ix ? lx.w1 : 0.f) : 0.f;
                v[k] = ld4(row + (long long)oxc * lddy);
            }
#pragma unroll
            for (int k = 0; k < 8; ++k) r += wx[k] * v[k];
        }
        a0 += wy0 * r;
        a1 += wy1 * r;
    }
    const long long o = ((n * h + iy) * w + ix) * (long long)C + c;
    st4(p0 + o, a0);
    st4(p1 + o, a1);
}
__global__ __launch_bounds__(256) void bilinear_bwd_combine_kernel(const float* __restrict__ p0, const float* __restrict__ p1, float* __restrict__ dx,
                                                                   long long lddx, int h, int w, int C4, long long total) {
    GRID_STRIDE(i, total) {
        const int c = (int)(i % C4) * 4;
        const long long pix = i / C4;
        const int iy = (int)((pix / w) % h);
        f32x4 v = ld4(p0 + pix * C4 * 4 + c);
        if (iy > 0) v += ld4(p1 + (pix - w) * C4 * 4 + c);
        st4(dx + pix * lddx + c, v);
    }
}
extern "C" int64_t sh_bilinear_bwd_workspace(int N, int h, int w, int C) {
    if (N <= 0 || h <= 0 || w <= 0 || C <= 0) return SH_EINVAL;
    return (int64_t)2 * N * h * w * C * 4;
}
extern "C" int sh_bilinear_bwd(const float* dy, int lddy, float* dx, int lddx, int N, int h, int w, int H, int W, int C, float* workspace,
                               int64_t workspace_bytes, void* stream) {
    if (!dy || !dx || N <= 0 || h <= 0 || w <= 0 || H <= 0 || W <= 0 || C <= 0 || (C & 3) || lddx < C || lddy < C || (lddx & 3) || (lddy & 3)) return SH_EINVAL;
    const long long total = (long long)N * h * w * (C / 4);
    const float sy = (float)h / (float)H, sx = (float)w / (float)W;
    const long long nblk = (long long)N * h * sh_cdiv(w, 16) * sh_cdiv(C, 64);
    if (workspace && ((uintptr_t)workspace & 15) == 0 && workspace_bytes >= sh_bilinear_bwd_workspace(N, h, w, C) && H >= 2 * h && W >= 2 * w &&
        nblk < (1LL << 31)) {
        float* p0 = workspace;
        float* p1 = workspace + (long long)N * h * w * C;
        bilinear_bwd_rows_kernel<<<(unsigned)nblk, 256, 0, (hipStream_t)stream>>>(dy, lddy, p0, p1, h, w, H, W, C, sy, sx);
        bilinear_bwd_combine_kernel<<<grid_for(total), 256, 0, (hipStream_t)stream>>>(p0, p1, dx, lddx, h, w, C / 4, total);
        return sh_launch_status();
    }
    bilinear_bwd_kernel<<<grid_for(total), 256, 0, (hipStream_t)stream>>>(dy, lddy, dx, lddx, h, w, H, W, C / 4, sy, sx, total);
    return sh_launch_status();
}

__global__ __launch_bounds__(256) void l2norm_fwd_kernel(const float* __restrict__ x, float* __restrict__ y, float* __restrict__ norm,
                                                         long long M, int C) {
    const int lane = threadIdx.x & 63;
    const long long row = (long long)blockIdx.x * 4 + (threadIdx.x >> 6);
    if (row >= M) return;
    const float* xr = x + row * C;
    float s = 0.f;
    for (int c = lane; c < C; c += 64) { const float v = xr[c]; s += v * v; }
    s = wave_sum(s);
    const float nrm = fmaxf(sqrtf(s), 1e-12f);
    for (int c = lane; c < C; c += 64) y[row * C + c] = xr[c] / nrm;
    if (lane == 0) norm[row] = nrm;
}
__global__ __launch_bounds__(256) void l2norm_bwd_kernel(const float* __restrict__ dy, const float* __restrict__ y,
                                                         const float* __restrict__ norm, float* __restrict__ dx, long long M, int C) {
    const int lane = threadIdx.x & 63;
    const long long row = (long long)blockIdx.x * 4 + (threadIdx.x >> 6);
    if (row >= M) return;
    float d = 0.f;
    for (int c = lane; c < C; c += 64) d += dy[row * C + c] * y[row * C + c];
    d = wave_sum(d);
    const float nrm = norm[row];
    const bool clamped = !(nrm > 1e-12f);
    for (int c = lane; c < C; c += 64) {
        const float g = dy[row * C + c];
        dx[row * C + c] = clamped ? g / nrm : (g - y[row * C + c] * d) / nrm;
    }
}
extern "C" int sh_l2norm_fwd(const float* x, float* y, float* norm, int64_t M, int C, void* stream) {
    if (!x || !y || !norm || M <= 0 || C <= 0) return SH_EINVAL;
    l2norm_fwd_kernel<<<(unsigned)sh_cdiv(M, 4), 256, 0, (hipStream_t)stream>>>(x, y, norm, M, C);
    return sh_launch_status();
}
extern "C" int sh_l2norm_bwd(const float* dy, const float* y, const float* norm, float* dx, int64_t M, int C, void* stream) {
    if (!dy || !y || !norm || !dx || M <= 0 || C <= 0) return SH_EINVAL;
    l2norm_bwd_kernel<<<(unsigned)sh_cdiv(M, 4), 256, 0, (hipStream_t)stream>>>(dy, y, norm, dx, M, C);
    return sh_launch_status();
}

__global__ __launch_bounds__(256) void ingest_image_kernel(const unsigned char* __restrict__ rgb, float* __restrict__ out,
                                                           const unsigned char* __restrict__ flip, long long NHW, int HW, int W,
                                                           float m0, float m1, float m2, float s0, float s1, float s2) {
    for (long long i = (long long)blockIdx.x * 256 + threadIdx.x; i < NHW; i += (long long)gridDim.x * 256) {
        const long long n = i / HW;
        const int x = (int)(i % W);
        long long src = i;
        if (flip != nullptr && flip[n]) src = i - x + (W - 1 - x);
        const unsigned char* q = rgb + src * 3;
        f32x4 v;
        v[0] = ((float)q[0] / 255.0f - m0) / s0;
        v[1] = ((float)q[1] / 255.0f - m1) / s1;
        v[2] = ((float)q[2] / 255.0f - m2) / s2;
        v[3] = 0.f;
        st4(out + i * 4, v);
    }
}
extern "C" int sh_ingest_image_u8(const uint8_t* rgb, float* out, const uint8_t* flip, int N, int H, int W, const float* mean3_host,
                                  const float* std3_host, void* stream) {
    if (!rgb || !out || !mean3_host || !std3_host || N <= 0 || H <= 0 || W <= 0) return SH_EINVAL;
    if (std3_host[0] == 0.f || std3_host[1] == 0.f || std3_host[2] == 0.f) return SH_EINVAL;
    const long long nhw = (long long)N * H * W;
    long long g = sh_cdiv(nhw, 256);
    if (g > 16384) g = 16384;
    ingest_image_kernel<<<(unsigned)g, 256, 0, (hipStream_t)stream>>>(rgb, out, flip, nhw, H * W, W, mean3_host[0], mean3_host[1], mean3_host[2],
                                                                      std3_host[0], std3_host[1], std3_host[2]);
    return sh_launch_status();
}
template <typename T>
__global__ __launch_bounds__(256) void ingest_mask_kernel(const T* __restrict__ mask, unsigned char* __restrict__ out,
                                                          const unsigned char* __restrict__ flip, int N, int Hs, int Ws, int H, int W) {
    const float sy = (float)Hs / (float)H, sx = (float)Ws / (float)W;
    const long long total = (long long)N * H * W;
    for (long long i = (long long)blockIdx.x * 256 + threadIdx.x; i < total; i += (long long)gridDim.x * 256) {
        int x = (int)(i % W);
        const long long r = i / W;
        const int y = (int)(r % H);
        const long long n = r / H;
        if (flip != nullptr && flip[n]) x = W - 1 - x;
        const int yy = min((int)floorf((float)y * sy), Hs - 1), xx = min((int)floorf((float)x * sx), Ws - 1);
        out[i] = (unsigned char)mask[(n * Hs + yy) * Ws + xx];
    }
}
extern "C" int sh_ingest_mask(const void* mask, int is_i64, uint8_t* out, const uint8_t* flip, int N, int Hs, int Ws, int H, int W,
                              void* stream) {
    if (!mask || !out || N <= 0 || Hs <= 0 || Ws <= 0 || H <= 0 || W <= 0) return SH_EINVAL;
    long long g = sh_cdiv((long long)N * H * W, 256);
    if (g > 16384) g = 16384;
    if (is_i64) ingest_mask_kernel<long long><<<(unsigned)g, 256, 0, (hipStream_t)stream>>>((const long long*)mask, out, flip, N, Hs, Ws, H, W);
    else ingest_mask_kernel<unsigned char><<<(unsigned)g, 256, 0, (hipStream_t)stream>>>((const unsigned char*)mask, out, flip, N, Hs, Ws, H, W);
    return sh_launch_status();
}

#define SH_RZ_BITS 22
extern "C" int sh_resize_bilinear_coeffs(int in_size, int out_size, int* bounds, int* kk, int kk_capacity) {
    if (in_size <= 0 || out_size <= 0) return SH_EINVAL;
    double scale, filterscale;
    filterscale = scale = (double)in_size / (double)out_size;
    if (filterscale < 1.0) filterscale = 1.0;
    const double support = 1.0 * filterscale;
    const int ksize = (int)ceil(support) * 2 + 1;
    if (!bounds || !kk) return ksize;
    if ((long long)ksize * out_size > kk_capacity) return SH_EINVAL;
    const double ss = 1.0 / filterscale;
    for (int xx = 0; xx < out_size; ++xx) {
        const double center = (xx + 0.5) * scale;
        double ww = 0.0;
        int xmin = (int)(center - support + 0.5);
        if (xmin < 0) xmin = 0;
        int xmax = (int)(center + support + 0.5);
        if (xmax > in_size) xmax = in_size;
        xmax -= xmin;
        int* k = kk + (long long)xx * ksize;
        double w[64];
        if (xmax > 64) return SH_EINVAL;
        for (int x = 0; x < xmax; ++x) {
            double t = (x + xmin - center + 0.5) * ss;
            if (t < 0.0) t = -t;
            w[x] = t < 1.0 ? 1.0 - t : 0.0;
            ww += w[x];
        }
        for (int x = 0; x < ksize; ++x) {
            if (x < xmax) {
                const double v = ww != 0.0 ? w[x] / ww : w[x];
                k[x] = v < 0 ? (int)(-0.5 + v * (1 << SH_RZ_BITS)) : (int)(0.5 + v * (1 << SH_RZ_BITS));
            } else k[x] = 0;
        }
        bounds[2 * xx] = xmin; bounds[2 * xx + 1] = xmax;
    }
    return ksize;
}
template <int AXIS>
__global__ __launch_bounds__(256) void resize_u8_pass_kernel(const unsigned char* __restrict__ src, unsigned char* __restrict__ dst,
                                                             const int* __restrict__ bounds, const int* __restrict__ kk, int ksize,
                                                             int H, int W, int Ho, int Wo, long long total) {
    GRID_STRIDE(i, total) {
        const int ox = (int)(i % Wo);
        const long long q = i / Wo;
        const int oy = (int)(q % Ho);
        const long long n = q / Ho;
        const int o = AXIS == 0 ? ox : oy;
        const int lo = bounds[2 * o], cnt = bounds[2 * o + 1];
        const int* k = kk + (long long)o * ksize;
        int a0 = 1 << (SH_RZ_BITS - 1), a1 = a0, a2 = a0;
        for (int t = 0; t < cnt; ++t) {
            const long long pix = AXIS == 0 ? (n * H + oy) * W + lo + t : (n * H + lo + t) * W + ox;
            const unsigned char* sp = src + pix * 3;
            const int kv = k[t];
            a0 += sp[0] * kv; a1 += sp[1] * kv; a2 += sp[2] * kv;
        }
        unsigned char* dp = dst + i * 3;
        dp[0] = (unsigned char)min(255, max(0, a0 >> SH_RZ_BITS));
        dp[1] = (unsigned char)min(255, max(0, a1 >> SH_RZ_BITS));
        dp[2] = (unsigned char)min(255, max(0, a2 >> SH_RZ_BITS));
    }
}
extern "C" int sh_resize_bilinear_u8(const uint8_t* src, uint8_t* tmp, uint8_t* dst, int N, int H, int W, int Ho, int Wo,
                                     const int* bounds_x, const int* kk_x, int ksize_x, const int* bounds_y, const int* kk_y, int ksize_y,
                                     void* stream) {
    if (!src || !dst || N <= 0 || H <= 0 || W <= 0 || Ho <= 0 || Wo <= 0) return SH_EINVAL;
    if ((Wo != W && (!bounds_x || !kk_x || ksize_x <= 0)) || (Ho != H && (!bounds_y || !kk_y || ksize_y <= 0))) return SH_EINVAL;
    if (Wo != W && Ho != H && !tmp) return SH_EINVAL;
    hipStream_t st = (hipStream_t)stream;
    const uint8_t* cur = src;
    if (Wo != W) {
        uint8_t* out = Ho != H ? tmp : dst;
        const long long total = (long long)N * H * Wo;
        resize_u8_pass_kernel<0><<<grid_for(total), 256, 0, st>>>(cur, out, bounds_x, kk_x, ksize_x, H, W, H, Wo, total);
        cur = out;
    }
    if (Ho != H) {
        const long long total = (long long)N * Ho * Wo;
        resize_u8_pass_kernel<1><<<grid_for(total), 256, 0, st>>>(cur, dst, bounds_y, kk_y, ksize_y, H, Wo, Ho, Wo, total);
// ... 6 lines not shown
```

### seghiero_amd/head.py

```python
import torch
import torch.nn as nn

from . import layers as L
from . import ops
from ._lib import SegHieroHipError

G1 = (1, 0, 1)


def _cbr(cin, cout):
    return nn.Sequential(nn.Conv2d(cin, cout, 1, bias=False), nn.BatchNorm2d(cout), nn.ReLU(inplace=True))


class ProjectionHead(nn.Module):
    def __init__(self, dim_in, proj_dim=256, proj="convmlp"):
        super().__init__()
        if proj == "linear":
            self.proj = nn.Conv2d(dim_in, proj_dim, kernel_size=1, bias=False)
        elif proj == "convmlp":
            self.proj = nn.Sequential(nn.Conv2d(dim_in, dim_in, kernel_size=1, bias=False), nn.BatchNorm2d(dim_in),
                                      nn.ReLU(inplace=True), nn.Conv2d(dim_in, proj_dim, kernel_size=1, bias=False))
        else:
            raise ValueError(f"Unknown proj type: {proj}")


class DepthwiseSeparableConv(nn.Module):
    def __init__(self, in_channels, out_channels, kernel_size=3, dilation=1, padding=1, bias=False):
        super().__init__()
        if kernel_size != 3 or padding != dilation or bias:
            raise SegHieroHipError("HIP depthwise kernel: 3x3, padding == dilation, no bias (all the reference uses)")
        self.depthwise = nn.Conv2d(in_channels, in_channels, kernel_size=kernel_size, padding=padding,
                                   dilation=dilation, groups=in_channels, bias=bias)
        self.bn_dw = nn.BatchNorm2d(in_channels)
        self.act_dw = nn.ReLU(inplace=True)
        self.pointwise = nn.Conv2d(in_channels, out_channels, kernel_size=1, bias=bias)
        self.bn_pw = nn.BatchNorm2d(out_channels)
        self.act_pw = nn.ReLU(inplace=True)


class DepthwiseSeparableASPPModule(nn.Module):

    def __init__(self, dilations, in_channels, channels):
        super().__init__()
        self.dilations = dilations
        self.branches = nn.ModuleList([_cbr(in_channels, channels)])
        for d in dilations[1:]:
            nn.Conv2d(in_channels, channels, kernel_size=3, padding=d, dilation=d, bias=False)
            self.branches.append(None)
        self.image_pool = nn.AdaptiveAvgPool2d(1)
        self.image_pool_conv = _cbr(in_channels, channels)
        for i, d in enumerate(dilations[1:], start=1):
            self.branches[i] = nn.Sequential(DepthwiseSeparableConv(in_channels, channels, kernel_size=3,
                                                                    dilation=d, padding=d, bias=False))


ASPP_GROUPED = True


def _aspp_branches_grouped(aspp, c4, cat, A, training, R, c4b=None):
    n, cin, h, w = c4.shape
    nbr = len(aspp.dilations)
    if not (ASPP_GROUPED and training and not ops._sync_on() and A % 128 == 0 and cin % 16 == 0
            and nbr <= 6):
        return False
    dev = c4.device
    m = n * h * w
    src4 = c4 if c4b is None else c4b
    sources, weights, bns = [(src4, None)], [aspp.branches[0][0].weight], [aspp.branches[0][1]]
    centre = [i for i, d in enumerate(aspp.dilations[1:], start=1) if d >= h and d >= w]
    if centre:
        x_stats = ops.channel_stats(c4)
        cfs = [torch.empty((4, cin), device=dev, dtype=torch.float32) for _ in centre]
        isys = [torch.empty((cin,), device=dev, dtype=torch.float32) for _ in centre]
        ops.bn_finalize_multi(x_stats, m, ops.LIB.raw("sh_stats_tile_rows")(), [aspp.branches[i][0].bn_dw for i in centre], cfs,
                              dw_weights=[aspp.branches[i][0].depthwise.weight for i in centre], isy_list=isys)
        for i, cf, isy in zip(centre, cfs, isys):
            R[f"dwc{i}"] = (cf, isy)
    for i, d in enumerate(aspp.dilations[1:], start=1):
        ds = aspp.branches[i][0]
        if i in centre:
            sources.append((src4, R[f"dwc{i}"][0]))
        else:
            with ops.stored_as(torch.float32):
                t, R[f"dw{i}"] = L.dw_fwd(c4, ds.depthwise.weight, d, ds.bn_dw, training, lazy=True)
            sources.append((t.y if c4b is None else t.y.to(torch.bfloat16), t.coefs))
        weights.append(ds.pointwise.weight)
        bns.append(ds.bn_pw)
    ycat = ops.new_act(n, nbr * A, h, w, dev)
    partials = ops.conv_partials(m, nbr * A, dev)
    if not ops.conv1x1_grouped_fprop(sources, weights, ycat, partials):
        raise SegHieroHipError("grouped ASPP launch rejected an eligible geometry")
    coefs_cat = torch.empty((4, nbr * A), device=dev, dtype=torch.float32)
    ops.bn_finalize_multi(partials, m, 64, bns, [coefs_cat[:, g * A:(g + 1) * A] for g in range(nbr)], partials_ld=nbr * A,
                          cols=[g * A for g in range(nbr)])
    ops.bn_act(ycat, coefs_cat, cat[:, A:(nbr + 1) * A], True)
    for g in range(nbr):
        rec = L.CBARec()
        src, cf = sources[g]
        rec.x = src if cf is None else L.Lazy(src, cf, grad32=True)
        rec.y, rec.out, rec.coefs = ycat[:, g * A:(g + 1) * A], None, coefs_cat[:, g * A:(g + 1) * A]
        rec.relu, rec.geom, rec.weight, rec.has_res, rec.mask = True, G1, weights[g], False, None
        R["b0" if g == 0 else f"pw{g}"] = rec
    return True


class _HeadFn(torch.autograd.Function):
    @staticmethod
    def forward(ctx, mod, c1, c4, *params):
        with ops.compute_as(mod.compute_dtype):
            return _HeadFn._forward(ctx, mod, c1, c4, *params)

    @staticmethod
    def backward(ctx, dlogits, demb):
        with ops.compute_as(ctx.mod.compute_dtype):
            return _HeadFn._backward(ctx, dlogits, demb)

    @staticmethod
    def _forward(ctx, mod, c1, c4, *params):
        training = mod.training
        c4 = ops.to_nhwc(c4)
        if ops.pm(c4)[1] != c4.shape[1]:
            c4 = ops.dense_copy(c4)
        n, cin, h, w = c4.shape
        dev = c4.device
        R = {}
        b16 = ops.b16() and training and mod.act_dtype == torch.bfloat16 and cin % 8 == 0
        c4b = c4.to(torch.bfloat16) if b16 else None
        proj = mod.proj_head.proj
        with ops.stored_as(torch.bfloat16 if b16 else torch.float32):
            if isinstance(proj, nn.Sequential):
                p1, R["p1"] = L.cba_fwd(c4b if b16 else c4, proj[0].weight, G1, proj[1], True, training, lazy=True)
                e_raw = L.conv_fwd(p1, proj[3].weight, None, G1)
                R["p1_out"] = p1
            else:
                e_raw = L.conv_fwd(c4b if b16 else c4, proj.weight, None, G1)
                R["emb_in"] = c4b if b16 else c4
        if ops.pm(e_raw)[1] != e_raw.shape[1]:
            e_raw = ops.dense_copy(e_raw)
        emb, norm = ops.l2norm_fwd(e_raw)
        R["emb"], R["norm"] = emb, norm
        aspp = mod.aspp
        A = aspp.image_pool_conv[0].out_channels
        nb = len(aspp.dilations) + 1
        cat = ops.new_act(n, A * nb, h, w, dev, dtype=torch.bfloat16 if b16 else torch.float32)
        pooled = ops.avgpool_fwd(c4)
        ip, R["ip"] = L.cba_fwd(pooled, aspp.image_pool_conv[0].weight, G1, aspp.image_pool_conv[1], True, training)
        if b16:
            cat[:, 0:A].copy_(ip.expand(n, A, h, w))
        else:
            ops.broadcast_hw(ip, cat[:, 0:A])
        if not _aspp_branches_grouped(aspp, c4, cat, A, training, R, c4b):
            _, R["b0"] = L.cba_fwd(c4, aspp.branches[0][0].weight, G1, aspp.branches[0][1], True, training, out=cat[:, A:2 * A])
            for i, d in enumerate(aspp.dilations[1:], start=1):
                ds = aspp.branches[i][0]
                t, R[f"dw{i}"] = L.dw_fwd(c4, ds.depthwise.weight, d, ds.bn_dw, training, lazy=True)
                _, R[f"pw{i}"] = L.cba_fwd(t, ds.pointwise.weight, G1, ds.bn_pw, True, training, out=cat[:, (i + 1) * A:(i + 2) * A])
        b, R["bt"] = L.cba_fwd(cat, mod.bottleneck[0].weight, G1, mod.bottleneck[1], True, training)
        H1, W1 = (c1.shape[2:] if mod.c1_bottleneck is not None else (h, w))
        stored = mod.act_dtype if (training and ops.dw_lin_ok((n, A, H1, W1), 1)) else torch.float32
        with ops.stored_as(stored):
            if mod.c1_bottleneck is not None:
                c1 = ops.to_nhwc(c1)
                c1ch = mod.c1_bottleneck[0].out_channels
                cat2 = ops.new_act(n, A + c1ch, H1, W1, dev, dtype=stored)
                _, R["c1"] = L.cba_fwd(c1, mod.c1_bottleneck[0].weight, G1, mod.c1_bottleneck[1], True, training, out=cat2[:, A:])
                ops.bilinear_fwd(b, cat2[:, :A])
                xin = cat2
            else:
                xin = b
            for j, ds in enumerate(mod.sep_bottleneck):
                t, R[f"sdw{j}"] = L.dw_fwd(xin, ds.depthwise.weight, 1, ds.bn_dw, training, lazy=True)
                xin, R[f"spw{j}"] = L.cba_fwd(t, ds.pointwise.weight, G1, ds.bn_pw, True, training, lazy=True)
        logits = L.conv_fwd(xin, mod.cls_seg.weight, mod.cls_seg.bias, G1)
        R["cls_in"] = xin
        if training:
            bns = mod.__dict__.get("_bn_list")
            if bns is None:
                bns = mod.__dict__["_bn_list"] = [m for m in mod.modules() if isinstance(m, nn.BatchNorm2d)]
            L.bump_bn_counters(bns)
        ctx.mod, ctx.R, ctx.params, ctx.training = mod, R, params, training
        ctx.hw = (h, w)
        ctx.c1_needs = c1 is not None and torch.is_tensor(c1) and ctx.needs_input_grad[1]
        return logits, emb

    @staticmethod
    def _backward(ctx, dlogits, demb):
        if not ctx.training:
            raise SegHieroHipError("backward through eval-mode BatchNorm is not on the SegHiero hot path")
        mod, R = ctx.mod, ctx.R
        aspp = mod.aspp
        A = aspp.image_pool_conv[0].out_channels
        h, w = ctx.hw
        gm = L.GradMap()

        def put_cba(conv_w, bn, res):
            gm.put(conv_w, res[1]); gm.put(bn.weight, res[2]); gm.put(bn.bias, res[3])

        dc1 = dc4 = None
        if dlogits is not None:
            C = mod.cls_seg.out_channels
            dl = L.grad_as_nhwc_padded(dlogits, C)
            dx, dw = L.conv_bwd(R["cls_in"], mod.cls_seg.weight, G1, dl)
            gm.put(mod.cls_seg.weight, dw)
            part = ops.channel_stats(dl)
            red = torch.empty((4, C), device=dl.device, dtype=torch.float32)
            ops._call("sh_bn_bwd_finalize", part.data_ptr(), part.shape[0], C, None, None, 1.0, red[0].data_ptr(),
                      red[1].data_ptr(), red[2].data_ptr(), red[3].data_ptr(), None, None, ops._st())
            gm.put(mod.cls_seg.bias, red[1])
            for j in range(len(mod.sep_bottleneck) - 1, -1, -1):
                ds = mod.sep_bottleneck[j]
                res = L.cba_bwd(R[f"spw{j}"], ds.bn_pw, dx)
                put_cba(ds.pointwise.weight, ds.bn_pw, res)
                dx, dww, dg, db = L.dw_bwd(R[f"sdw{j}"], ds.bn_dw, res[0])
                gm.put(ds.depthwise.weight, dww); gm.put(ds.bn_dw.weight, dg); gm.put(ds.bn_dw.bias, db)
            if mod.c1_bottleneck is not None:
                dbt = ops.bilinear_bwd(dx[:, :A], h, w)
                res = L.cba_bwd(R["c1"], mod.c1_bottleneck[1], dx[:, A:], need_dx=ctx.c1_needs)
                put_cba(mod.c1_bottleneck[0].weight, mod.c1_bottleneck[1], res)
                dc1 = res[0]
            else:
                dbt = dx
            res = L.cba_bwd(R["bt"], mod.bottleneck[1], dbt)
            put_cba(mod.bottleneck[0].weight, mod.bottleneck[1], res)
            dcat = res[0]
            res = L.cba_bwd(R["b0"], aspp.branches[0][1], dcat[:, A:2 * A], dx32=True)
            put_cba(aspp.branches[0][0].weight, aspp.branches[0][1], res)
            dc4 = res[0]
            for i in range(1, len(aspp.dilations)):
                ds = aspp.branches[i][0]
                res = L.cba_bwd(R[f"pw{i}"], ds.bn_pw, dcat[:, (i + 1) * A:(i + 2) * A])
                put_cba(ds.pointwise.weight, ds.bn_pw, res)
                if f"dwc{i}" in R:
                    coefs_x, isy = R[f"dwc{i}"]
                    xin = R[f"pw{i}"].x.y
                    dxc, dg, db, _ = ops.bn_backward(res[0], None, xin, coefs_x, ds.bn_dw.weight, 2, grad32=True)
                    ops._call("sh_axpy", dc4.data_ptr(), dxc.data_ptr(), 1.0, dc4.numel(), ops._st())
                    dww = L.new_grad(ds.depthwise.weight)
                    gmask = res[0].g if isinstance(res[0], L.GradPack) and xin.dtype == torch.float32 else None
                    ops.dw_center_wgrad(dg, ds.bn_dw.weight, isy, ds.depthwise.weight, ds.bn_dw.eps, dww, g=gmask, x=xin, mean_x=coefs_x[0])
                else:
                    _, dww, dg, db = L.dw_bwd(R[f"dw{i}"], ds.bn_dw, res[0], dx_accumulate_into=dc4)
                gm.put(ds.depthwise.weight, dww); gm.put(ds.bn_dw.weight, dg); gm.put(ds.bn_dw.bias, db)
            dip = ops.sum_hw(ops.f32(dcat[:, 0:A]))
            res = L.cba_bwd(R["ip"], aspp.image_pool_conv[1], dip)
            put_cba(aspp.image_pool_conv[0].weight, aspp.image_pool_conv[1], res)
            ops.avgpool_bwd(res[0], dc4, accumulate=True)
        if demb is not None:
            de = ops.l2norm_bwd(demb, R["emb"], R["norm"])
            proj = mod.proj_head.proj
            if isinstance(proj, nn.Sequential):
                dp1, dw3 = L.conv_bwd(R["p1_out"], proj[3].weight, G1, L.grad_as_nhwc_padded(de, de.shape[1]))
                gm.put(proj[3].weight, dw3)
                res = L.cba_bwd(R["p1"], proj[1], dp1, addend=dc4, dx32=True)
                put_cba(proj[0].weight, proj[1], res)
                dc4 = res[0]
            else:
                dc4n, dwp = L.conv_bwd(R["emb_in"], proj.weight, G1, L.grad_as_nhwc_padded(de, de.shape[1]), addend=dc4, dx32=True)
                gm.put(proj.weight, dwp)
                dc4 = dc4n
        ctx.R = None
        gm.flush(ctx.params)
        return (None, dc1, dc4) + gm.ordered(ctx.params)


class DepthwiseSeparableASPPContrastHead(nn.Module):
    def __init__(self, in_channels: int, c1_in_channels: int, c1_channels: int, aspp_channels: int, dilations: tuple,
                 num_classes: int, proj_dim: int = 256, proj_type: str = "convmlp"):
        super().__init__()
        self.proj_head = ProjectionHead(dim_in=in_channels, proj_dim=proj_dim, proj=proj_type)
        self.register_buffer("step", torch.zeros(1, dtype=torch.long))
        self.aspp = DepthwiseSeparableASPPModule(dilations=dilations, in_channels=in_channels, channels=aspp_channels)
        total_aspp_ch = aspp_channels * (len(dilations) + 1)
        self.bottleneck = _cbr(total_aspp_ch, aspp_channels)
        if c1_in_channels > 0:
            self.c1_bottleneck = _cbr(c1_in_channels, c1_channels)
        else:
            self.c1_bottleneck = None
            c1_channels = 0
        self.sep_bottleneck = nn.Sequential(
            DepthwiseSeparableConv(aspp_channels + c1_channels, aspp_channels, kernel_size=3, padding=1, bias=False),
            DepthwiseSeparableConv(aspp_channels, aspp_channels, kernel_size=3, padding=1, bias=False))
        self.cls_seg = nn.Conv2d(aspp_channels, num_classes, kernel_size=1)
        self.act_dtype = torch.float32
        self.compute_dtype = torch.float32
        self.align_corners = False
        for name, v in (("in_channels", in_channels), ("aspp_channels", aspp_channels), ("c1_channels", c1_channels),
                        ("proj_dim", proj_dim), ("c1_in_channels", max(c1_in_channels, 0))):
            if v % 4:
                raise SegHieroHipError(f"{name}={v}: the HIP kernels need channel counts that are multiples of 4")

    def forward(self, inputs: list):
        ops._require_gpu(inputs[-1])
        self.step += 1
        c1 = inputs[0] if self.c1_bottleneck is not None else None
        return _HeadFn.apply(self, c1, inputs[-1], *L.params_of(self))


class _AuxFn(torch.autograd.Function):
    @staticmethod
    def forward(ctx, mod, c3, *params):
        c3 = ops.to_nhwc(c3)
        out, rec = L.cba_fwd(c3, mod[0].weight, G1, mod[1], True, mod.training)
        if mod.training:
            L.bump_bn_counters([mod[1]])
        ctx.mod, ctx.rec, ctx.params, ctx.training = mod, rec, params, mod.training
        return out

    @staticmethod
    def backward(ctx, dout):
        if not ctx.training:
            raise SegHieroHipError("backward through eval-mode BatchNorm is not on the SegHiero hot path")
        mod = ctx.mod
        d = L.grad_as_nhwc_padded(dout, dout.shape[1])
        dx, dw, dg, db, _ = L.cba_bwd(ctx.rec, mod[1], d, need_dx=ctx.needs_input_grad[1])
        gm = L.GradMap()
        gm.put(mod[0].weight, dw); gm.put(mod[1].weight, dg); gm.put(mod[1].bias, db)
        ctx.rec = None
        gm.flush(ctx.params)
        return (None, dx) + gm.ordered(ctx.params)


class AuxHead(nn.Sequential):

    def __init__(self, in_channels: int, n_fine: int):
        super().__init__(nn.Conv2d(in_channels, n_fine, kernel_size=1, bias=False), nn.BatchNorm2d(n_fine),
                         nn.ReLU(inplace=True))

    def forward(self, c3):
        ops._require_gpu(c3)
        return _AuxFn.apply(self, c3, *L.params_of(self))
```

### seghiero_amd/layers.py

```python
import torch
import torch.nn as nn

from . import ops


def conv_geom(conv):
    return conv.stride[0], conv.padding[0], conv.dilation[0]


def W(m):
    return m._parameters["weight"]


def Bi(m):
    return m._parameters["bias"]


def to_native_layout(module):
    for m in module.modules():
        if isinstance(m, nn.Conv2d) and m.groups == 1 and m.kernel_size != (1, 1) and m.in_channels % 4 == 0:
            if not m.weight.data.is_contiguous(memory_format=torch.channels_last):
                m.weight.data = m.weight.data.contiguous(memory_format=torch.channels_last)
    return module


def params_of(mod):
    ps = mod.__dict__.get("_param_list")
    if ps is None:
        ps = mod.__dict__["_param_list"] = list(mod.parameters())
    return ps


def bump_bn_counters(bns):
    ctrs = [b.num_batches_tracked for b in bns if b.num_batches_tracked is not None]
    if ctrs:
        torch._foreach_add_(ctrs, 1)


class Lazy:
    __slots__ = ("y", "coefs", "_out", "grad32")

    def __init__(self, y, coefs, grad32=False):
        self.y, self.coefs, self._out, self.grad32 = y, coefs, None, grad32

    @property
    def shape(self):
        return self.y.shape

    @property
    def device(self):
        return self.y.device

    def materialize(self):
        if self._out is None:
            n, c, h, w = self.y.shape
            ld = ops.pad4(c)
            self._out = ops.new_act(n, c, h, w, self.y.device, ld=ld, zero=ld != c, dtype=self.y.dtype)
            ops.bn_act(self.y, self.coefs, self._out, True)
        return self._out


class LazyAffine:
    __slots__ = ("y", "coefs")

    def __init__(self, y, coefs):
        self.y, self.coefs = y, coefs


class GradPack:
    __slots__ = ("g", "partials")

    def __init__(self, g, partials):
        self.g, self.partials = g, partials


def dense(x):
    return x.materialize() if isinstance(x, Lazy) else x


class CBARec:
    __slots__ = ("x", "y", "out", "coefs", "relu", "geom", "weight", "has_res", "mask")


def _bn_coefs(bn, partials, count, training, c, device):
    if training:
        mom = 0.1 if bn.momentum is None else bn.momentum
        pr, bf = bn._parameters, bn._buffers
        return ops.bn_finalize(partials, count, pr["weight"], pr["bias"], bn.eps, mom, bf["running_mean"], bf["running_var"], c, device)
    return ops.bn_eval_coefs(bn.weight, bn.bias, bn.running_mean, bn.running_var, bn.eps)


def _fprop(x, weight, bias, y, partials, s, p, d):
    if isinstance(x, Lazy):
        if ops.conv_fprop_aff(x.y, x.coefs, weight, bias, y, partials, s, p, d):
            return
        x = x.materialize()
    ops.conv_fprop(x, weight, bias, y, partials, s, p, d)


def _wgrad(x, dy, dw, s, p, d):
    if isinstance(dy, ops.DeferredDy) and isinstance(x, Lazy) and not (x._out is None and ops.wgrad_aff_ok(x.y, dw, s, p, d)):
        dy = dy.materialize()
    if isinstance(x, Lazy):
        if x._out is None and ops.wgrad_aff_ok(x.y, dw, s, p, d):
            ops.conv_wgrad(x.y, dy, dw, s, p, d, side=True, aff=x.coefs)
            return
        x = x.materialize()
    ops.conv_wgrad(x, dy, dw, s, p, d, side=True)


def _dgrad(rec_x, dy, weight, s, p, d, addend=None, pack_for=None, grad32=False):
    like = rec_x.y if isinstance(rec_x, Lazy) else rec_x
    g32 = grad32 or (isinstance(rec_x, Lazy) and rec_x.grad32)
    if ops.grad_dtype(like, g32) == torch.bfloat16:
        out = _dgrad_as(torch.bfloat16, rec_x, dy, weight, s, p, d, addend, pack_for)
        if out is not None:
            return out
    return _dgrad_as(torch.float32, rec_x, dy, weight, s, p, d, addend, pack_for)


def _dgrad_as(gdt, rec_x, dy, weight, s, p, d, addend, pack_for):
    n, c, h, w = rec_x.shape
    dev = (rec_x.y if isinstance(rec_x, Lazy) else rec_x).device
    strict = gdt != torch.float32
    new = lambda: ops.new_act(n, c, h, w, dev, dtype=gdt)
    parts = lambda: torch.empty((-(-n * h * w // 64), 2, c), device=dev, dtype=torch.float32)

    def plain(cur, dx):
        if not strict:
            ops.conv_dgrad(cur, weight, dx, s, p, d, addend=addend)
            return dx
        return dx if ops._dgrad_b16(cur, weight, dx, s, p, d, addend=addend) else None

    if isinstance(dy, ops.DeferredDy):
        if pack_for is None:
            if isinstance(rec_x, Lazy):
                g, partials = new(), parts()
                if ops.conv_dgrad_lin(dy, weight, g, addend=addend, bnb=(rec_x.y, rec_x.coefs, partials)):
                    return GradPack(g, partials)
            else:
                dx = new()
                if ops.conv_dgrad_lin(dy, weight, dx, addend=addend):
                    return dx
        dy = dy.materialize()
    if pack_for is not None and not isinstance(rec_x, Lazy):
        g, partials = new(), parts()
        if ops.conv_dgrad_bnb(dy, weight, g, pack_for.y, pack_for.coefs, True, partials, s, p, d, addend=addend,
                              out_prev=pack_for.out if pack_for.mask is None else pack_for.mask):
            return GradPack(g, partials)
        return plain(dy, g)
    if isinstance(rec_x, Lazy):
        g, partials = new(), parts()
        if ops.conv_dgrad_bnb(dy, weight, g, rec_x.y, rec_x.coefs, True, partials, s, p, d, addend=addend):
            return GradPack(g, partials)
        return plain(dy, g)
    return plain(dy, new())


def cba_fwd(x, weight, geom, bn, relu, training, residual=None, out=None, lazy=False):
    s, p, d = geom
    n, _, h, w = x.shape
    o, _, kh, kw = weight.shape
    ho, wo = ops.conv_out_hw(h, w, kh, kw, s, p, d)
    ld = ops.pad4(o)
    m = n * ho * wo
    mask = None
    if not training and ops.FUSE_EVAL:
        coefs = _bn_coefs(bn, None, m, False, o, x.device)
        if out is None:
            out = ops.new_act(n, o, ho, wo, x.device, ld=ld, zero=ld != o)
        ops.conv_fprop_act(dense(x), weight, coefs, out, relu, residual, s, p, d)
        y = None
    else:
        y = ops.new_act(n, o, ho, wo, x.device, ld=ld, zero=ld != o, dtype=ops.stored_dtype())
        partials = ops.conv_partials(m, o, x.device) if training else None
        _fprop(x, weight, None, y, partials, s, p, d)
        coefs = _bn_coefs(bn, partials, m, training, o, x.device)
        if lazy and training and relu and residual is None and out is None:
            out = Lazy(y, coefs)
        elif lazy and training and not relu and residual is None and out is None:
            out = LazyAffine(y, coefs)
        else:
            if out is None:
                out = ops.new_act(n, o, ho, wo, x.device, ld=ld, zero=ld != o, dtype=ops.stored_dtype())
            if training and relu and residual is not None and o % 4 == 0:
                mask = ops.new_relu_mask(n, o, ho, wo, x.device)
            if isinstance(residual, LazyAffine):
                ops.bn_act(y, coefs, out, relu, residual.y, res_coefs=residual.coefs, mask=mask)
            else:
                ops.bn_act(y, coefs, out, relu, residual, mask=mask)
    rec = CBARec()
    rec.x, rec.y, rec.coefs, rec.relu, rec.geom, rec.weight = x, y, coefs, relu, geom, weight
    rec.out = None if isinstance(out, (Lazy, LazyAffine)) else out
    rec.has_res = residual is not None
    rec.mask = mask
    return out, rec


def new_grad(param):
    from . import ddp
    buf = ddp.grad_buffer(param)
    return torch.empty_like(param) if buf is None else buf


def cba_bwd(rec, bn, dout, need_dx=True, addend=None, want_dres=False, scatter_into=None, pack_for=None, dx32=False):
    s, p, d = rec.geom
    xin = rec.x.y if isinstance(rec.x, Lazy) else rec.x
    strided = s > 1 or scatter_into is not None
    dy32 = xin.dtype == torch.float32 or (strided and not ops.strided_dgrad_b16_ok(rec.weight, xin.shape[1], s, p, d, scatter_into is not None))
    mode = 0 if not rec.relu else (1 if rec.has_res else 2)
    defer = scatter_into is None and pack_for is None and ops.lin_ok(rec.x.shape, rec.weight, s, p, d)
    dy, dgamma, dbeta, dres = ops.bn_backward(dout, (rec.out if rec.mask is None else rec.mask) if mode == 1 else None, rec.y, rec.coefs,
                                              W(bn), mode, want_dres, defer=defer, grad32=dy32)
    dw = new_grad(rec.weight)
    dx = None
    if scatter_into is not None:
        ops.conv_dgrad(dy, rec.weight, scatter_into, s, p, d, mode=1)
        dx = scatter_into
    elif need_dx:
        dx = _dgrad(rec.x, dy, rec.weight, s, p, d, addend=addend, pack_for=pack_for, grad32=dx32)
    _wgrad(rec.x, dy, dw, s, p, d)
    return dx, dw, dgamma, dbeta, dres


class DWRec:
    __slots__ = ("x", "y", "out", "coefs", "dil", "weight")


def dw_fwd(x, weight, dil, bn, training, lazy=False):
    n, c, h, w = x.shape
    y = ops.new_act(n, c, h, w, x.device, dtype=ops.stored_dtype())
    partials = torch.empty((ops.dw_partials_rows(n, h, w), 2, c), device=x.device) if training else None
    if isinstance(x, Lazy) and x._out is None:
        ops.dwconv_fprop(x.y, weight, y, partials, dil, aff=x.coefs)
    else:
        x = dense(x)
        ops.dwconv_fprop(x, weight, y, partials, dil)
    coefs = _bn_coefs(bn, partials, n * h * w, training, c, x.device)
    if lazy and training:
        out = Lazy(y, coefs, grad32=True)
    else:
        out = ops.new_act(n, c, h, w, x.device)
        ops.bn_act(y, coefs, out, True)
    rec = DWRec()
    rec.x, rec.y, rec.coefs, rec.dil, rec.weight = x, y, coefs, dil, weight
    rec.out = None if isinstance(out, Lazy) else out
    return out, rec


def dw_bwd(rec, bn, dout, dx_accumulate_into=None):
    if hasattr(dout, "partials"):
        dout.g = ops.f32(dout.g)
    else:
        dout = ops.f32(dout)
    dy, dgamma, dbeta, _ = ops.bn_backward(dout, None, rec.y, rec.coefs, W(bn), 2, defer=ops.dw_lin_ok(rec.y.shape, rec.dil),
                                           grad32=True)
    dw = new_grad(rec.weight)
    if isinstance(rec.x, Lazy) and rec.x._out is None:
        ops.dwconv_wgrad(rec.x.y, dy, dw, rec.dil, side=True, aff=rec.x.coefs)
    else:
        ops.dwconv_wgrad(dense(rec.x), dy, dw, rec.dil, side=True)
    if dx_accumulate_into is not None:
        ops.dwconv_dgrad(dy, rec.weight, dx_accumulate_into, rec.dil, accumulate=True)
        dx = dx_accumulate_into
    else:
        n, c, h, w = rec.x.shape
        dx = ops.new_act(n, c, h, w, rec.x.device)
        if isinstance(rec.x, Lazy):
            partials = torch.empty((ops.dw_partials_rows(n, h, w), 2, c), device=dx.device, dtype=torch.float32)
            ops.dwconv_dgrad_bnb(dy, rec.weight, dx, rec.x.y, rec.x.coefs, partials, rec.dil)
            dx = GradPack(dx, partials)
        else:
            ops.dwconv_dgrad(dy, rec.weight, dx, rec.dil)
    return dx, dw, dgamma, dbeta


def conv_fwd(x, weight, bias, geom):
    s, p, d = geom
    n, _, h, w = x.shape
    o, _, kh, kw = weight.shape
    ho, wo = ops.conv_out_hw(h, w, kh, kw, s, p, d)
    ld = ops.pad8(o) if ops.b16() else ops.pad4(o)
    y = ops.new_act(n, o, ho, wo, x.device, ld=ld, zero=ld != o)
    _fprop(x, weight, bias, y, None, s, p, d)
    return y


def conv_bwd(x, weight, geom, dy, need_dx=True, addend=None, dx32=False):
    s, p, d = geom
    dw = new_grad(weight)
    _wgrad(x, dy, dw, s, p, d)
    dx = None
    if need_dx:
        dx = _dgrad(x, dy, weight, s, p, d, addend=addend, grad32=dx32)
    return dx, dw


def grad_as_nhwc_padded(g, c):
    g = ops.to_nhwc(g)
    ld = ops.pm(g)[1]
    q = 8 if ops.b16() else 4
    if ld == c and c % q == 0:
        return g
    return ops.dense_copy(g, ld=ops.pad8(c) if q == 8 else ops.pad4(c))


class GradMap:

    def __init__(self):
        self.g = {}

    def put(self, param, grad):
        if grad is None:
            return
        if grad.shape != param.shape:
            grad = grad.reshape(param.shape)
        key = id(param)
        if key in self.g:
            ops.join_wgrad()
            grad = self.g[key] + grad
        self.g[key] = grad

    def ordered(self, params):
        ops.join_wgrad()
        return tuple(self.g.get(id(p)) for p in params)

    def flush(self, params):
        from . import ddp
        if ddp._ACTIVE is not None:
            ops.join_wgrad()
            ddp.early_flush([(p, self.g.get(id(p))) for p in params])
```

### seghiero_amd/ops.py

```python
import contextlib
import ctypes

import torch

from ._lib import LIB, SegHieroHipError, status_text

import os

_PROF = None


def _call(name, *args, cost=None, key=None):
    if _PROF is None:
        return LIB.call(name, *args)
    e0, e1 = torch.cuda.Event(enable_timing=True), torch.cuda.Event(enable_timing=True)
    e0.record()
    rc = LIB.call(name, *args)
    e1.record()
    _PROF.append((name, cost, e0, e1, key))
    return rc


class profile:

# ... 362 lines not shown
        _call("sh_weights_to_bf16_multi", *args, st)


def prepare_bf16_weights(weights, cache):
    global _WB_ACTIVE
    sig = tuple(w.data_ptr() for w in weights)
    plan = cache.get("__plan__")
    if plan is None or plan[0] != sig:
        todo = []
        for w in weights:
            hit = cache.get(id(w))
            if hit is None or hit[0] is not w or hit[1].device != w.device:
                hit = (w,) + _wb_buffers(w)
                cache[id(w)] = hit
            todo.append(hit)
        plan = cache["__plan__"] = (sig, _wb_tables(todo))
    st = _st()
    for args in plan[1]:
        _call("sh_weights_to_bf16_multi", *args, st)
    _WB_ACTIVE = cache


def weights_bf16(weight):
    if _WB_ACTIVE is not None:
        hit = _WB_ACTIVE.get(id(weight))
        if hit is not None and hit[0] is weight:
            return hit[1], hit[2]
    item = (weight,) + _wb_buffers(weight)
    _wb_launch([item])
    return item[1], item[2]


def _dgrad_b16(dy, weight, dx, stride, pad, dil, addend=None, lin=None, bnb=None, scatter=False):
    n, cin, h, w = dx.shape
    o, _, kh, kw = weight.shape
    dyp, lddy, dyb = pmx(dy)
    if lddy < pad8(o):
        return False
    if (stride != 1 or scatter) and (addend is not None or lin is not None or bnb is not None):
        return False
    dxp, lddx, dxb = pmx(dx)
    ap, lda, ab = (None, 0, 0) if addend is None else pmx(addend)
    flags = dyb | (dxb << 1) | (ab << 2) | (64 if scatter else 0)
    ylp, ldyl, linp = None, 0, None
    if lin is not None:
        ylp, ldyl, ylb = pmx(lin[0])
        if not (ylb and dyb):
            return False
        linp = lin[1].data_ptr()
    bargs = (None, 0, None, 0, None, None, None, None, 0, None)
    if bnb is not None:
        y_prev, cf, relu, partials, out_prev = bnb
        ypp, ldyp, ypb = pmx(y_prev)
        flags |= ypb << 3
        if out_prev is not None and out_prev.dtype == torch.uint8:
            opp, ldop = out_prev.data_ptr(), cin // 4
            flags |= 32
        elif out_prev is not None:
            opp, ldop, opb = pmx(out_prev)
            flags |= opb << 4
        else:
            opp, ldop = None, 0
        bargs = (ypp, ldyp, opp, ldop, _rp(cf, 0), _rp(cf, 1), _rp(cf, 2), _rp(cf, 3), int(bool(relu)), partials.data_ptr())
    ho, wo = conv_out_hw(h, w, kh, kw, stride, pad, dil)
    m = n * ho * wo
    ws, nb = _splitk_ws(1, n, h, w, cin, o, kh, kw, stride, pad, dil, 0, dx.device)
    _, wtb = weights_bf16(weight)
    cost = (2.0 * m * o * cin * kh * kw, float((2 if dxb else 4) * n * h * w * cin * (1 + (addend is not None)) + (2 if dyb else 4) * m * o * (2 if lin else 1)
                                                + 2 * o * cin * kh * kw + (2 * n * h * w * cin if bnb else 0)))
    return _call_fused("sh_conv_dgrad_b16", dyp, lddy, ylp, ldyl, linp, wtb.data_ptr(), ap, lda, dxp, lddx, *bargs, n, h, w, cin, o, kh, kw,
                       stride, pad, dil, ws, nb, flags, _st(), cost=cost, key=_ckey(n, h, w, cin, o, kh, stride, dil))


def conv_dgrad(dy, weight, dx, stride, pad, dil, addend=None, mode=0):
    n, cin, h, w = dx.shape
    o, _, kh, kw = weight.shape
    if _B16 and mode == 0 and _dgrad_b16(dy, weight, dx, stride, pad, dil, addend=addend):
        return
    if _B16 and mode == 1 and addend is None and _dgrad_b16(dy, weight, dx, stride, pad, dil, scatter=True):
        return
    if dx.dtype != torch.float32:
        raise SegHieroHipError("the fp32-accurate input-gradient kernels write fp32 tensors")
    dy, addend = f32(dy), f32(addend)
    dyp, lddy = pm(dy)
    dxp, lddx = pm(dx)
    ap, lda = (None, 0) if addend is None else pm(addend)
    ho, wo = conv_out_hw(h, w, kh, kw, stride, pad, dil)
    m = n * ho * wo
    x6 = lddy >= pad4(o)
    wptr = weight_transpose(weight).data_ptr() if x6 else w_ohwi(weight).data_ptr()
    cost = (2.0 * m * o * cin * kh * kw, 4.0 * (n * h * w * cin * (2 if addend is not None or mode else 1) + m * o + o * cin * kh * kw))
    args = (dyp, lddy, wptr, ap, lda, dxp, lddx, n, h, w, cin, o, kh, kw, stride, pad, dil, mode)
    if x6:
        ws, nb = _splitk_ws(1, n, h, w, cin, o, kh, kw, stride, pad, dil, mode, dx.device)
        _call("sh_conv_dgrad_x6", *args, ws, nb, _st(), cost=cost, key=_ckey(n, h, w, cin, o, kh, stride, dil))
    else:
        _call("sh_conv_dgrad", *args, _st(), cost=cost, key=_ckey(n, h, w, cin, o, kh, stride, dil))


def conv_dgrad_bnb(dy, weight, g, y_prev, coefs, relu, partials, stride, pad, dil, addend=None, out_prev=None):
    n, cin, h, w = g.shape
    o, _, kh, kw = weight.shape
    if _B16 and _dgrad_b16(dy, weight, g, stride, pad, dil, addend=addend, bnb=(y_prev, coefs, relu, partials, out_prev)):
        return True
    if g.dtype != torch.float32:
        return False
    dy, addend = f32(dy), f32(addend)
    dyp, lddy = pm(dy)
    gp, ldg = pm(g)
    ypp, ldyp, ypb = pmx(y_prev)
    if lddy < pad4(o):
        return False
    ap, lda = (None, 0) if addend is None else pm(addend)
    if out_prev is not None and out_prev.dtype == torch.uint8:
        opp, ldop, opb = out_prev.data_ptr(), cin // 4, 2
    else:
        opp, ldop, opb = (None, 0, 0) if out_prev is None else pmx(out_prev)
    ho, wo = conv_out_hw(h, w, kh, kw, stride, pad, dil)
    m = n * ho * wo
    cost = (2.0 * m * o * cin * kh * kw, 4.0 * (n * h * w * cin * (3 if addend is not None else 2) + m * o + o * cin * kh * kw))
    ws, nb = _splitk_ws(1, n, h, w, cin, o, kh, kw, stride, pad, dil, 0, g.device)
    return _call_fused("sh_conv_dgrad_x6_bnb", dyp, lddy, weight_transpose(weight).data_ptr(), ap, lda, gp, ldg, ypp, ldyp, opp, ldop,
                       _rp(coefs, 0), _rp(coefs, 1), _rp(coefs, 2), _rp(coefs, 3), int(bool(relu)),
                       partials.data_ptr(), n, h, w, cin, o, kh, kw, stride, pad, dil, ws, nb, ypb | (opb << 1), _st(), cost=cost,
                       key=_ckey(n, h, w, cin, o, kh, stride, dil))


def conv_dgrad_lin(dd, weight, dx, addend=None, bnb=None):
    n, cin, h, w = dx.shape
    o = weight.shape[0]
    if _B16 and dd.g.dtype == torch.bfloat16:
        return _dgrad_b16(dd.g, weight, dx, 1, 0, 1, addend=addend, lin=(dd.y, dd.lin),
                          bnb=None if bnb is None else (bnb[0], bnb[1], True, bnb[2], None))
    if dx.dtype != torch.float32 or dd.g.dtype != torch.float32:
        return False
    addend = f32(addend)
    gp, ldg = pm(dd.g)
    yp, ldy, yb = pmx(dd.y)
    dxp, lddx = pm(dx)
    ap, lda = (None, 0) if addend is None else pm(addend)
    ypb = 0
    if bnb is None:
        bargs = (None, 0, None, None, None, None, 0, None)
    else:
        y_prev, cf, partials = bnb
        ypp, ldyp, ypb = pmx(y_prev)
        bargs = (ypp, ldyp, _rp(cf, 0), _rp(cf, 1), _rp(cf, 2), _rp(cf, 3), 1, partials.data_ptr())
    m = n * h * w
    cost = (2.0 * m * o * cin, 4.0 * (m * cin * (1 + (addend is not None) + (bnb is not None)) + 2 * m * o + o * cin))
    ws, nb = _splitk_ws(1, n, h, w, cin, o, 1, 1, 1, 0, 1, 0, dx.device)
    return _call_fused("sh_conv_dgrad_x6_lin", gp, ldg, yp, ldy, dd.lin.data_ptr(), weight_transpose(weight).data_ptr(), ap, lda, dxp, lddx,
                       *bargs, n, h, w, cin, o, ws, nb, yb | (ypb << 1), _st(), cost=cost, key=_ckey(n, h, w, cin, o, 1, 1, 1))


_WS = {}


def workspace(nbytes, device, tag="ws"):
    st = _st()
    key = (device, tag, st)
    buf = _WS.get(key)
    if buf is None or buf.numel() < nbytes:
        side = _SIDE.get(device.index)
        with torch.cuda.stream(side) if side is not None and side.cuda_stream == st else contextlib.nullcontext():
            buf = torch.empty(max(int(nbytes), 1 << 20), dtype=torch.uint8, device=device)
        _WS[key] = buf
    return buf


WGRAD_ASYNC = os.environ.get("SEGHIERO_WGRAD_STREAM", "1") != "0"
_SIDE = {}
_PENDING = False


def _wgrad_launch(side, launch, reads):
    global _STREAM, _PENDING
    if not (side and WGRAD_ASYNC):
        return launch()
    dev = reads[0].device
    st = _SIDE.get(dev.index)
    if st is None:
        st = _SIDE[dev.index] = torch.cuda.Stream(device=dev)
    st.wait_stream(torch.cuda.current_stream(dev))
    prev, _STREAM = _STREAM, st.cuda_stream
    try:
        rc = launch()
    finally:
        _STREAM = prev
    for t in reads:
        t.record_stream(st)
    _PENDING = True
    return rc


def join_wgrad():
    global _PENDING
    if _PENDING:
        for idx, st in _SIDE.items():
            torch.cuda.current_stream(idx).wait_stream(st)
        _PENDING = False


def wgrad_aff_ok(x, dweight, stride, pad, dil):
    n, cin, h, w = x.shape
    o, _, kh, kw = dweight.shape
    return _wgrad_pipelined_ok(x, o, kh, kw, stride, pad, dil)


def _wgrad_pipelined_ok(x, o, kh, kw, stride, pad, dil):
    n, cin, h, w = x.shape
    ho, wo = conv_out_hw(h, w, kh, kw, stride, pad, dil)
    ldx = _pm(x, True)[1] if x.dim() == 4 else cin
    return (cin % 4 == 0 and wo >= 16 and n * h * w * ldx * 4 < (1 << 31) and n * ho * wo * pad4(o) * 4 < (1 << 31))


def conv_wgrad(x, dy, dweight, stride, pad, dil, side=False, aff=None):
    n, cin, h, w = x.shape
    o, _, kh, kw = dweight.shape
    dd = dy if isinstance(dy, DeferredDy) else None
    if _B16 and x.dtype == torch.bfloat16 and _wgrad_b16(x, dy, dweight, stride, pad, dil, side, aff):
        return
    if dd is not None and dd.g.dtype != torch.float32:
        dy, dd = dd.materialize(), None
    if dd is None:
        dy = f32(dy)
    if (x.dtype == torch.bfloat16 or dd is not None) and not _wgrad_pipelined_ok(x, o, kh, kw, stride, pad, dil):
        if x.dtype == torch.bfloat16:
            x = x.float()
        if dd is not None:
            dy, dd = dd.materialize(), None
    if dd is not None and (dd.y.dtype == torch.bfloat16) != (x.dtype == torch.bfloat16):
        dy, dd = dd.materialize(), None
    if dd is not None:
        dy = dd.g
    x6 = o >= 32 and (cin * kh * kw >= 128 or (cin * kh * kw == 64 and o >= 128))
    if aff is not None or dd is not None or x.dtype == torch.bfloat16:
        x6 = True
    need = LIB.raw("sh_conv_wgrad_x6_workspace" if x6 else "sh_conv_wgrad_workspace")(n, h, w, cin, o, kh, kw, stride, pad, dil)
    if need < 0:
        raise SegHieroHipError("sh_conv_wgrad_workspace rejected the geometry")
    xp, ldx, xb = pmx(x)
    dyp, lddy = pm(dy)
    ho, wo = conv_out_hw(h, w, kh, kw, stride, pad, dil)
    m = n * ho * wo
    cost = (2.0 * m * o * cin * kh * kw, 4.0 * (n * h * w * cin + m * o + o * cin * kh * kw))
    aff2, aff3 = (None, None) if aff is None else (_rp(aff, 2), _rp(aff, 3))
    if dd is not None:
        y2p, ldy2, y2b = pmx(dd.y)
        name, head, flags = "sh_conv_wgrad_x6_lin", (xp, ldx, aff2, aff3, dyp, lddy, y2p, ldy2, dd.lin.data_ptr()), (xb | (y2b << 1),)
    elif aff is not None:
        name, head, flags = "sh_conv_wgrad_x6_aff", (xp, ldx, aff2, aff3, dyp, lddy), (xb,)
    else:
        name, head, flags = ("sh_conv_wgrad_x6", (xp, ldx, dyp, lddy), (xb,)) if x6 else ("sh_conv_wgrad", (xp, ldx, dyp, lddy), ())
    key = _ckey(n, h, w, cin, o, kh, stride, dil)
    launch = lambda: _call_fused(name, *head, dweight.data_ptr(), workspace(need, x.device, "wgrad").data_ptr(),
                                 n, h, w, cin, o, kh, kw, stride, pad, dil, *flags, _st(), cost=cost, key=key)
    if not _wgrad_launch(side, launch, (x, dy, dweight) + (() if dd is None else (dd.y, dd.lin))):
        raise SegHieroHipError(f"{name}: unsupported geometry (check lin_ok / wgrad_aff_ok before deferring dy / the activation)")


def _wgrad_b16(x, dy, dweight, stride, pad, dil, side, aff):
    n, cin, h, w = x.shape
    o, _, kh, kw = dweight.shape
    dd = dy if isinstance(dy, DeferredDy) else None
    g = dd.g if dd is not None else dy
    if dd is not None and not (dd.g.dtype == torch.bfloat16 and dd.y.dtype == torch.bfloat16):
        return False
    if cin % 8 or not dweight.is_contiguous(memory_format=torch.channels_last if kh * kw > 1 and cin > 1 else torch.contiguous_format):
        return False
    need = LIB.raw("sh_conv_wgrad_x6_workspace")(n, h, w, cin, o, kh, kw, stride, pad, dil)
    if need < 0:
        return False
    xp, ldx, _ = pmx(x)
    gp, ldg, gb = pmx(g)
    if ldg < pad8(o) or (o % 8 and dd is not None):
        return False
    ylp, ldyl = (None, 0) if dd is None else pmx(dd.y)[:2]
    ho, wo = conv_out_hw(h, w, kh, kw, stride, pad, dil)
    m = n * ho * wo
    cost = (2.0 * m * o * cin * kh * kw, float(2 * n * h * w * cin + (2 if gb else 4) * m * o * (2 if dd is not None else 1) + 4 * o * cin * kh * kw))
    key = _ckey(n, h, w, cin, o, kh, stride, dil)
    launch = lambda: _call_fused("sh_conv_wgrad_b16", xp, ldx, None if aff is None else _rp(aff, 2), None if aff is None else _rp(aff, 3),
                                 gp, ldg, ylp, ldyl, None if dd is None else dd.lin.data_ptr(), dweight.data_ptr(),
                                 workspace(need, x.device, "wgrad").data_ptr(), n, h, w, cin, o, kh, kw, stride, pad, dil, gb, _st(),
                                 cost=cost, key=key)
    return _wgrad_launch(side, launch, (x, g, dweight) + (() if dd is None else (dd.y, dd.lin)))


def conv_partials(m, cout, device):
    return torch.empty((-(-m // 64), 2, cout), device=device, dtype=torch.float32)


def dw_partials_rows(n, h, w):
    return LIB.raw("sh_dw_partials")(n, h, w)


def dwconv_fprop(x, weight, y, partials, dil, aff=None):
    n, c, h, w = x.shape
    xp, ldx, xb = pmx(x)
    yp, ldy, yb = pmx(y)
    _call("sh_dwconv_fprop", xp, ldx, None if aff is None else _rp(aff, 2), None if aff is None else _rp(aff, 3),
          weight.data_ptr(), yp, ldy, None if partials is None else partials.data_ptr(), n, h, w, c, dil, xb | (yb << 1), _st(),
          key=(None if _PROF is None else f"{n}x{h}x{w} C{c} d{dil}"))


def dw_lin_ok(shape, dil):
    n, c, h, w = shape
    return dil == 1 and h % 8 == 0 and w % 8 == 0 and c % 4 == 0


def _lin_args(dy):
    if isinstance(dy, DeferredDy):
        yp, ldy, yb = pmx(dy.y)
        return pm(dy.g) + (yp, ldy, dy.lin.data_ptr()), yb
    return pm(dy) + (None, 0, None), 0


def dwconv_dgrad(dy, weight, dx, dil, accumulate=False):
    n, c, h, w = dx.shape
    dxp, lddx = pm(dx)
    largs, yb = _lin_args(dy)
    _call("sh_dwconv_dgrad", *largs, weight.data_ptr(), dxp, lddx, n, h, w, c, dil, int(accumulate), yb, _st(), key=(None if _PROF is None else f"{n}x{h}x{w} C{c} d{dil}"))


def dwconv_dgrad_bnb(dy, weight, g, y_prev, coefs, partials, dil):
    n, c, h, w = g.shape
    gp, ldg = pm(g)
    ypp, ldyp, ypb = pmx(y_prev)
    largs, yb = _lin_args(dy)
    _call("sh_dwconv_dgrad_bnb", *largs, weight.data_ptr(), gp, ldg, ypp, ldyp, _rp(coefs, 0), _rp(coefs, 1),
          _rp(coefs, 2), _rp(coefs, 3), partials.data_ptr(), n, h, w, c, dil, yb | (ypb << 1), _st(), key=(None if _PROF is None else f"{n}x{h}x{w} C{c} d{dil}"))


def dwconv_wgrad(x, dy, dweight, dil, side=False, aff=None):
    n, c, h, w = x.shape
    p = dw_partials_rows(n, h, w)
    xp, ldx, xb = pmx(x)
    largs, yb = _lin_args(dy)
    key = None if _PROF is None else f"{n}x{h}x{w} C{c} d{dil}"
    launch = lambda: _call("sh_dwconv_wgrad", xp, ldx, None if aff is None else _rp(aff, 2), None if aff is None else _rp(aff, 3), *largs,
                           workspace(p * 9 * c * 4, x.device, "dwwgrad").data_ptr(), dweight.data_ptr(), n, h, w, c, dil, xb | (yb << 1),
                           _st(), key=key)
    _wgrad_launch(side, launch, (x, dy.g, dweight, dy.y, dy.lin) if isinstance(dy, DeferredDy) else (x, dy, dweight))


SYNC_BN = False


def _sync_on():
    if not SYNC_BN:
        return False
    from . import ddp
    return ddp.collectives_on()


def _all_reduce_sq(sq):
    from . import ddp
    ddp.all_reduce_small(sq)
    return sq


FOLD_MIN = 4096
FOLD_CHUNK = 64


def _fold_partials(partials, c, count, rows):
    p = partials.shape[0]
    if p < FOLD_MIN or partials.shape[-1] != c or not partials.is_contiguous():
        return partials, rows
    out = torch.empty((-(-p // FOLD_CHUNK), 2, c), device=partials.device, dtype=torch.float32)
    if not _call_fused("sh_bn_fold_partials", partials.data_ptr(), p, c, float(count), rows, FOLD_CHUNK, out.data_ptr(), _st(), key=(None if _PROF is None else f"P{p} C{c}")):
        return partials, rows
    return out, rows * FOLD_CHUNK


def bn_finalize(partials, count, gamma, beta, eps, momentum, running_mean, running_var, c, device, rows=64, coefs=None,
                partials_ld=0, partials_col=0):
    if coefs is None:
        coefs = torch.empty((4, c), device=device, dtype=torch.float32)
    pptr = partials.data_ptr() + 4 * partials_col
    if _sync_on():
        if partials_ld:
            raise SegHieroHipError("SyncBN does not take column slices of grouped partials")
        sq = torch.empty((2 * c + 1,), device=device, dtype=torch.float64)
        _call("sh_bn_reduce_partials", partials.data_ptr(), partials.shape[0], c, float(count), rows, sq.data_ptr(), _st())
        _all_reduce_sq(sq)
        _call("sh_bn_finalize_sq", sq.data_ptr(), c, None if gamma is None else gamma.data_ptr(),
              None if beta is None else beta.data_ptr(), eps, momentum,
              None if running_mean is None else running_mean.data_ptr(),
              None if running_var is None else running_var.data_ptr(),
              _rp(coefs, 0), _rp(coefs, 1), _rp(coefs, 2), _rp(coefs, 3), _st())
        return coefs
    if not partials_ld and not partials_col:
        partials, rows = _fold_partials(partials, c, count, rows)
        pptr = partials.data_ptr()
    _call("sh_bn_finalize", pptr, partials.shape[0], c, float(count),
          None if gamma is None else gamma.data_ptr(), None if beta is None else beta.data_ptr(), eps, momentum,
          None if running_mean is None else running_mean.data_ptr(),
          None if running_var is None else running_var.data_ptr(),
          _rp(coefs, 0), _rp(coefs, 1), _rp(coefs, 2), _rp(coefs, 3), rows, int(partials_ld), _st(),
          key=(None if _PROF is None else f"P{partials.shape[0]} C{c}"))
    return coefs


def bn_finalize_scaled(partials, count, dw_weight, gamma, beta, eps, momentum, running_mean, running_var, c, device, rows):
    coefs = torch.empty((4, c), device=device, dtype=torch.float32)
    isy = torch.empty((c,), device=device, dtype=torch.float32)
    _call("sh_bn_finalize_scaled", partials.data_ptr(), partials.shape[0], c, float(count), dw_weight.data_ptr() + 16, 9,
          gamma.data_ptr(), beta.data_ptr(), eps, momentum, None if running_mean is None else running_mean.data_ptr(),
          None if running_var is None else running_var.data_ptr(), _rp(coefs, 0), _rp(coefs, 1), _rp(coefs, 2),
          _rp(coefs, 3), isy.data_ptr(), rows, _st())
    return coefs, isy


def bn_finalize_multi(partials, count, rows, bns, coefs_list, partials_ld=0, cols=None, dw_weights=None, isy_list=None):
    k = len(bns)
    c = coefs_list[0].shape[1]
    eps, mom = bns[0].eps, 0.1 if bns[0].momentum is None else bns[0].momentum
    if any(b.eps != eps or (0.1 if b.momentum is None else b.momentum) != mom for b in bns) or k > 8:
        raise SegHieroHipError("bn_finalize_multi needs <= 8 layers with one eps / momentum")
    vp = ctypes.c_void_p
    arr = lambda vals: (vp * k)(*vals)
    ptr = lambda t: None if t is None else t.data_ptr()
    cols = [0] * k if cols is None else cols
    dw_weights = [None] * k if dw_weights is None else dw_weights
    isy_list = [None] * k if isy_list is None else isy_list
    _call("sh_bn_finalize_multi", k, partials.data_ptr(), partials.shape[0], c, float(count), rows, int(partials_ld),
          (ctypes.c_int * k)(*cols), arr([b.weight.data_ptr() for b in bns]), arr([b.bias.data_ptr() for b in bns]),
          arr([ptr(b.running_mean) for b in bns]), arr([ptr(b.running_var) for b in bns]),
          arr([_rp(cf, 0) for cf in coefs_list]), arr([_rp(cf, 1) for cf in coefs_list]),
          arr([_rp(cf, 2) for cf in coefs_list]), arr([_rp(cf, 3) for cf in coefs_list]),
          arr([None if w is None else w.data_ptr() + 16 for w in dw_weights]), 9, arr([ptr(t) for t in isy_list]),
          float(eps), float(mom), _st())


def dw_center_wgrad(dgamma, gamma, isy, dw_weight, eps, dweight, g=None, x=None, mean_x=None):
    gp, ldg = (None, 0) if g is None else pm(g)
    xp, ldx = (None, 0) if g is None else pm(x)
    m = 0 if g is None else g.shape[0] * g.shape[2] * g.shape[3]
    _call("sh_dw_center_wgrad", dgamma.data_ptr(), gamma.data_ptr(), isy.data_ptr(), dw_weight.data_ptr(), float(eps),
          dweight.data_ptr(), dw_weight.shape[0], gp, ldg, xp, ldx, None if g is None else mean_x.data_ptr(), m, _st())


def conv1x1_grouped_fprop(sources, weights, y, partials):
    k = len(sources)
    n, cin, h, w = sources[0][0].shape
    a = weights[0].shape[0]
    if _B16 and all(x.dtype == torch.bfloat16 for x, _ in sources):
        xs, lds = zip(*[pmx(x)[:2] for x, _ in sources])
        yp, ldy, yb = pmx(y)
        vp = ctypes.c_void_p
        arr = lambda vals: (vp * k)(*vals)
        cost = (2.0 * n * h * w * cin * a * k, float(n * h * w * (2 * cin + (2 if yb else 4) * a) * k + 2 * a * cin * k))
        wbs = [weights_bf16(wt)[0] for wt in weights]
        return _call_fused("sh_conv1x1_grouped_fprop_b16", k, arr(xs), (ctypes.c_int * k)(*lds),
                           arr([None if c is None else _rp(c, 2) for _, c in sources]),
                           arr([None if c is None else _rp(c, 3) for _, c in sources]),
                           arr([t.data_ptr() for t in wbs]), yp, ldy, partials.data_ptr(), n, h, w, cin, a, yb << 1, _st(),
                           cost=cost, key=(None if _PROF is None else f"{k} x ({n}x{h}x{w} {cin}->{a} k1)"))
    xs, lds = zip(*[pm(x) for x, _ in sources])
    yp, ldy = pm(y)
    vp = ctypes.c_void_p
    arr = lambda vals: (vp * k)(*vals)
    cost = (2.0 * n * h * w * cin * a * k, 4.0 * (n * h * w * (cin + a) * k + a * cin * k))
    return _call_fused("sh_conv1x1_grouped_fprop_x6", k, arr(xs), (ctypes.c_int * k)(*lds),
                       arr([None if c is None else _rp(c, 2) for _, c in sources]),
                       arr([None if c is None else _rp(c, 3) for _, c in sources]),
                       arr([w_ohwi(wt).data_ptr() for wt in weights]), yp, ldy, partials.data_ptr(), n, h, w, cin, a, _st(),
                       cost=cost, key=(None if _PROF is None else f"{k} x ({n}x{h}x{w} {cin}->{a} k1)"))



def bn_eval_coefs(gamma, beta, running_mean, running_var, eps):
    c = running_mean.numel()
    coefs = torch.empty((4, c), device=running_mean.device, dtype=torch.float32)
    _call("sh_bn_eval_coefs", gamma.data_ptr(), beta.data_ptr(), running_mean.data_ptr(), running_var.data_ptr(), eps, c,
          _rp(coefs, 2), _rp(coefs, 3), _st())
    return coefs


def channel_stats(y):
    n, c, h, w = y.shape
    m = n * h * w
    p = LIB.raw("sh_stats_partials_count")(m)
    partials = torch.empty((p, 2, c), device=y.device, dtype=torch.float32)
    yp, ldy = pm(y)
    _call("sh_channel_stats", yp, ldy, m, c, partials.data_ptr(), _st())
    return partials


def new_relu_mask(n, c, h, w, device):
    return torch.empty((n, h, w, c // 4), device=device, dtype=torch.uint8)


def bn_act(y, coefs, out, relu, residual=None, res_coefs=None, mask=None):
    n, c, h, w = y.shape
    yp, ldy, yb = pmx(y)
    op, ldo, ob = pmx(out)
    rp, ldr, rb = (None, 0, 0) if residual is None else pmx(residual)
    _call("sh_bn_act", yp, ldy, _rp(coefs, 2), _rp(coefs, 3), rp, ldr,
          None if res_coefs is None else _rp(res_coefs, 2), None if res_coefs is None else _rp(res_coefs, 3),
          op, ldo, n * h * w, c, int(relu), None if mask is None else mask.data_ptr(), yb | (rb << 1) | (ob << 2), _st(),
          key=(None if _PROF is None else f"{n}x{h}x{w} C{c}" + (" +res" if residual is not None else "")))


class DeferredDy:
    __slots__ = ("g", "y", "lin", "coefs", "gamma", "red", "_dy")

    def __init__(self, g, y, lin, coefs, gamma, red):
        self.g, self.y, self.lin, self.coefs, self.gamma, self.red, self._dy = g, y, lin, coefs, gamma, red, None

    @property
    def shape(self):
        return self.y.shape

    def materialize(self):
        if self._dy is None:
            n, c, h, w = self.y.shape
            gdt = self.g.dtype
            ld = pad8(c) if gdt == torch.bfloat16 else pad4(c)
            dy = new_act(n, c, h, w, self.y.device, ld=ld, zero=ld != c, dtype=gdt)
            gp, ldg, gb = pmx(self.g)
            yp, ldy, yb = pmx(self.y)
            dyp, lddy = pmx(dy)[:2]
            cf = self.coefs
            _call("sh_bn_bwd_apply", gp, ldg, None, 0, yp, ldy, _rp(cf, 0), _rp(cf, 1), _rp(cf, 2), _rp(cf, 3),
                  None if self.gamma is None else self.gamma.data_ptr(), _rp(self.red, 2), _rp(self.red, 3), dyp, lddy,
                  None, 0, n * h * w, c, 0, yb | (gb << 2) | (gb << 3), _st(), key=(None if _PROF is None else f"{n}x{h}x{w} C{c} (deferred)"))
            self._dy = dy
        return self._dy


DEFER_RATIO = 0.5


def grad_dtype(like, fp32_consumer=False):
    if _B16 and not fp32_consumer and like is not None and like.dtype == torch.bfloat16:
        return torch.bfloat16
    return torch.float32


def strided_dgrad_b16_ok(weight, cin, stride, pad, dil, scatter):
    o, _, kh, kw = weight.shape
    if not (_B16 and cin % 8 == 0 and o % 8 == 0):
        return False
    if scatter:
        return kh == 1 and kw == 1 and pad == 0
    return stride == 2 and dil == 1 and kh * kw > 1 and o % 64 == 0


def lin_ok(x_shape, weight, stride, pad, dil):
    n, cin, h, w = x_shape
    o, _, kh, kw = weight.shape
    return (kh == 1 and kw == 1 and stride == 1 and pad == 0 and o % 4 == 0 and cin % 4 == 0
            and o >= 32 and cin >= 64 and w >= 16 and n * h * w * max(pad4(o), pad4(cin)) * 4 < (1 << 31)
            and o * DEFER_RATIO >= cin)


def bn_backward(dout, out, y, coefs, gamma, relu, want_dres=False, dy_ld=None, defer=False, grad32=False):
    relu = int(relu)
    if relu == 2:
        out = None
    n, c, h, w = y.shape
    m = n * h * w
    dev = y.device
    yp, ldy, yb = pmx(y)
    if out is not None and out.dtype == torch.uint8:
        if relu != 1:
            raise SegHieroHipError("a ReLU quad mask stands in for `out` in mode 1 only")
        op, ldo, ob, relu = out.data_ptr(), c // 4, 0, 3
    else:
        op, ldo, ob = (None, 0, 0) if out is None else pmx(out)
    af = yb | (ob << 1)
    gdt = grad_dtype(y, grad32)
    packed = hasattr(dout, "partials")
    if packed:
        partials, dout, relu, op, ldo = dout.partials, dout.g, 0, None, 0
        p = partials.shape[0]
        dop, lddo, dob = pmx(dout)
    else:
        dop, lddo, dob = pmx(dout)
        p = LIB.raw("sh_stats_partials_count")(m)
        partials = torch.empty((p, 2, c), device=dev, dtype=torch.float32)
        gmask = None
        if defer and relu:
            gmask = new_act(n, c, h, w, dev, dtype=gdt)
            if not _call_fused("sh_bn_bwd_reduce", dop, lddo, op, ldo, yp, ldy, _rp(coefs, 0), _rp(coefs, 1), _rp(coefs, 2),
                               _rp(coefs, 3), partials.data_ptr(), m, c, relu, gmask.data_ptr(), c, af | (dob << 2) | (int(gdt == torch.bfloat16) << 3),
                               _st(), key=(None if _PROF is None else f"{n}x{h}x{w} C{c} +g")):
                gmask, defer = None, False
        if gmask is None:
            _call("sh_bn_bwd_reduce", dop, lddo, op, ldo, yp, ldy, _rp(coefs, 0), _rp(coefs, 1), _rp(coefs, 2),
                  _rp(coefs, 3), partials.data_ptr(), m, c, relu, None, 0, af | (dob << 2), _st(), key=(None if _PROF is None else f"{n}x{h}x{w} C{c}"))
        else:
            dout, relu, op, ldo = gmask, 0, None, 0
            dop, lddo, dob = pmx(dout)
            packed = True
    if defer and (lddo % 4 or dop % 16 or c % 4):
        defer = False
    if defer and _B16 and dout.dtype != y.dtype:
        defer = False
    red = torch.empty((4, c), device=dev, dtype=torch.float32)
    lin = torch.empty((4, c), device=dev, dtype=torch.float32) if defer else None
    linp = None if lin is None else lin.data_ptr()
    if _sync_on():
        local = torch.empty((2 * c + 1,), device=dev, dtype=torch.float64)
# ... 401 lines not shown
```

Before: 482.4.

## Fuse bilinear upsample and concat into depthwise conv fprop and wgrad

```diff
diff --git a/include/seghiero_hip.h b/include/seghiero_hip.h
--- a/include/seghiero_hip.h
+++ b/include/seghiero_hip.h
@@ -94,6 +94,12 @@
 int sh_dwconv_wgrad(const float* x, int ldx, const float* in_scale, const float* in_shift, const float* dy, int lddy,
                     const float* y_lin, int ldyl, const float* lin, float* dw_partials, float* dw, int N, int H, int W, int C, int dil,
                     int act_flags, void* stream);
+int sh_dwconv_up_ok(int N, int h, int w, int H, int W, int A, int C, int dil);
+int sh_dwconv_fprop_up(const float* low, int ldl, int h, int w, int A, const float* skip, int lds, const float* wt, float* y, int ldy,
+                       float* stat_partials, int N, int H, int W, int C, int dil, int act_flags, void* stream);
+int sh_dwconv_wgrad_up(const float* low, int ldl, int h, int w, int A, const float* skip, int lds, const float* dy, int lddy,
+                       const float* y_lin, int ldyl, const float* lin, float* dw_partials, float* dw, int N, int H, int W, int C, int dil,
+                       int act_flags, void* stream);
 
 int sh_bn_finalize(const float* partials, int n_partials, int C, double count, const float* gamma,
                    const float* beta, float eps, float momentum, float* running_mean,
diff --git a/seghiero_amd/csrc/common.h b/seghiero_amd/csrc/common.h
--- a/seghiero_amd/csrc/common.h
+++ b/seghiero_amd/csrc/common.h
@@ -34,6 +34,19 @@
 
 __device__ __forceinline__ f32x4 ld4(const float* p) { return *reinterpret_cast<const f32x4*>(p); }
 __device__ __forceinline__ void st4(float* p, f32x4 v) { *reinterpret_cast<f32x4*>(p) = v; }
+
+struct Lerp { int i0, i1; float w0, w1; };
+__host__ __device__ __forceinline__ Lerp lerp_src(int dst, float scale, int in) {
+    float s = scale * ((float)dst + 0.5f) - 0.5f;
+    s = s < 0.f ? 0.f : s;
+    Lerp L;
+    L.i0 = (int)s;
+    if (L.i0 > in - 1) L.i0 = in - 1;
+    L.i1 = L.i0 + (L.i0 < in - 1 ? 1 : 0);
+    L.w1 = s - (float)L.i0;
+    L.w0 = 1.f - L.w1;
+    return L;
+}
 
 typedef unsigned int sh_u32x2 __attribute__((ext_vector_type(2)));
 __device__ __forceinline__ f32x4 bf16x4_to_f32(sh_u32x2 v) {
diff --git a/seghiero_amd/csrc/dwconv.hip b/seghiero_amd/csrc/dwconv.hip
--- a/seghiero_amd/csrc/dwconv.hip
+++ b/seghiero_amd/csrc/dwconv.hip
@@ -284,9 +284,9 @@
     bool cok;
     long long t0, t1;
 };
-__device__ __forceinline__ void dw_walk_init(DwWalk& q, int H, int W, int C, int N, int cq) {
-    const unsigned nch = (unsigned)((C + DW_CH - 1) / DW_CH), nb = gridDim.x / nch, k = blockIdx.x / nch;
-    q.c0 = (int)(blockIdx.x % nch) * DW_CH; q.c = q.c0 + cq * 4; q.cok = q.c < C;
+__device__ __forceinline__ void dw_walk_init(DwWalk& q, int H, int W, int C, int N, int cq, int ch0 = 0, int nchl = 0) {
+    const unsigned nch = nchl ? (unsigned)nchl : (unsigned)((C + DW_CH - 1) / DW_CH), nb = gridDim.x / nch, k = blockIdx.x / nch;
+    q.c0 = (ch0 + (int)(blockIdx.x % nch)) * DW_CH; q.c = q.c0 + cq * 4; q.cok = q.c < C;
     q.tiles_x = W / DT; q.tiles_y = H / DT;
     const long long T = (long long)N * q.tiles_y * q.tiles_x;
     q.t0 = T * k / nb; q.t1 = T * (k + 1) / nb;
@@ -299,6 +299,34 @@
     f32x4 v = {0.f, 0.f, 0.f, 0.f};
     if (dw_walk_inside(q, H, W, hy, ix)) v = lda4(x, (((long long)q.n * H + q.ty * DT + hy - 1) * W + ix) * ldx + q.c, bf);
     return v;
+}
+#define DW_UP_PIX 48
+struct DwUp { const float* low; long long ldl; int h, w; float sy, sx; int ch0, nch; };
+__host__ __device__ __forceinline__ void dw_up_rows(int ty, int H, int h, float sy, int& r0, int& r1) {
+    const int o0 = ty * DT - 1 < 0 ? 0 : ty * DT - 1, o1 = ty * DT + DT > H - 1 ? H - 1 : ty * DT + DT;
+    r0 = lerp_src(o0, sy, h).i0; r1 = lerp_src(o1, sy, h).i1;
+}
+__device__ __forceinline__ int dw_up_stage(float (*ls)[DW_CH], const DwUp& u, const DwWalk& q, int H, int pl, int cq) {
+    int r0, r1;
+    dw_up_rows(q.ty, H, u.h, u.sy, r0, r1);
+    int cnt = (r1 - r0 + 1) * u.w;
+    if (cnt > DW_UP_PIX) cnt = DW_UP_PIX;
+    const float* src = u.low + ((long long)q.n * u.h + r0) * u.w * u.ldl + q.c;
+    for (int i = pl; i < cnt; i += 16) st4(&ls[i][cq * 4], ld4(src + i * u.ldl));
+    return r0;
+}
+__device__ __forceinline__ f32x4 dw_up_eval(const float (*ls)[DW_CH], const DwUp& u, const DwWalk& q, int r0, int H, int W, int hy, int ix, int cq) {
+    const int oy = q.ty * DT + hy - 1;
+    f32x4 r = {0.f, 0.f, 0.f, 0.f};
+    if ((unsigned)oy < (unsigned)H && (unsigned)ix < (unsigned)W) {
+        const Lerp ly = lerp_src(oy, u.sy, u.h), lx = lerp_src(ix, u.sx, u.w);
+        const float* b0 = &ls[(ly.i0 - r0) * u.w][cq * 4];
+        const float* b1 = &ls[(ly.i1 - r0) * u.w][cq * 4];
+        const f32x4 v00 = ld4(b0 + lx.i0 * DW_CH), v01 = ld4(b0 + lx.i1 * DW_CH);
+        const f32x4 v10 = ld4(b1 + lx.i0 * DW_CH), v11 = ld4(b1 + lx.i1 * DW_CH);
+        r = ly.w0 * (lx.w0 * v00 + lx.w1 * v01) + ly.w1 * (lx.w0 * v10 + lx.w1 * v11);
+    }
+    return r;
 }
 struct DwLin { const float* y; long long ldy; const float* lin; int y_bf; };
 struct DwLinC { f32x4 a, b, mu, d; };
@@ -320,33 +348,41 @@
     }
     return v;
 }
-template <int LIN, int XBF, int YBF>
+template <int LIN, int XBF, int YBF, int UP = 0>
 __device__ __forceinline__ void dw_walk_prologue(float (*xs)[DWR][DW_CH], const float* __restrict__ x, long long ldx, bool aff,
                                                  const f32x4& sc, const f32x4& sh, const DwWalk& q, int H, int W, int tx, int rb, int pl, int cq,
-                                                 const DwLin* L = nullptr, const DwLinC* lc = nullptr) {
+                                                 const DwLin* L = nullptr, const DwLinC* lc = nullptr,
+                                                 const float (*ls)[DW_CH] = nullptr, const DwUp* up = nullptr, int r0 = 0) {
     for (int i = pl; i < (DT + 2) * (DT + 2); i += 16) {
         const int hy = i / (DT + 2), hx = i - hy * (DT + 2), ix = tx * DT + hx - 1;
+        if constexpr (UP) {
+            st4(&xs[hy][dw_slot(rb, hx)][cq * 4], dw_up_eval(ls, *up, q, r0, H, W, hy, ix, cq));
+            continue;
+        }
         f32x4 v = dw_walk_fetch(x, ldx, q, H, W, hy, ix, XBF);
         if constexpr (LIN) v = dw_lin_eval(v, dw_walk_fetch(L->y, L->ldy, q, H, W, hy, ix, YBF), dw_walk_inside(q, H, W, hy, ix), *lc);
         st4(&xs[hy][dw_slot(rb, hx)][cq * 4], dw_walk_act(v, aff, dw_walk_inside(q, H, W, hy, ix), sc, sh));
     }
 }
-template <int MODE, int LIN, int BNB, int BF>
+template <int MODE, int LIN, int BNB, int BF, int UP = 0>
 __global__ __launch_bounds__(256, (LIN && BNB) ? 2 : 3) void dwconv_walk_kernel(const float* __restrict__ x, long long ldx, const float* __restrict__ w,
                                                           float* __restrict__ y, long long ldy, float* __restrict__ partials,
                                                           int N, int H, int W, int C, int accumulate,
                                                           const float* __restrict__ isc, const float* __restrict__ ish, const DwBnb bnb,
-                                                          const DwLin lin, int af) {
+                                                          const DwLin lin, int af, const DwUp up) {
     __shared__ __attribute__((aligned(16))) float xs[DT + 2][DWR][DW_CH];
+    __shared__ __attribute__((aligned(16))) float ls[UP ? DW_UP_PIX : 1][UP ? DW_CH : 4];
     __shared__ float red[16][DW_CH];
     __shared__ float colmean[DW_CH];
     static_assert(MODE == 1 || (LIN == 0 && BNB == 0), "the loader / epilogue hooks belong to the dgrad");
+    static_assert(UP == 0 || (MODE == 0 && BF == 0), "the upsampled chunks belong to the fp32 fprop");
+    [[maybe_unused]] int r0 = 0;
     constexpr int x_bf = MODE == 0 ? (BF & 1) : 0, y_bf = MODE == 0 ? (BF & 2) : 0, ly_bf = MODE == 1 ? (BF & 1) : 0, by_bf = MODE == 1 ? (BF & 2) : 0;
     constexpr bool has_lin = LIN != 0;
     (void)af;
     const int t = threadIdx.x, cq = t & 15, pl = t >> 4;
     DwWalk q;
-    dw_walk_init(q, H, W, C, N, cq);
+    dw_walk_init(q, H, W, C, N, cq, up.ch0, up.nch);
     const DwLinC lc = dw_lin_coefs(lin, C, q.c, q.cok);
     const DwBnbC bc = dw_bnb_coefs(bnb, q.c, q.cok);
     f32x4 wr[9];
@@ -361,13 +397,18 @@
     for (long long tile = q.t0; tile < q.t1; ++tile) {
         if (tile == q.t0 || tx == 0) {
             dw_walk_strip(q, tile / q.tiles_x);
+            if constexpr (UP) {
+                r0 = dw_up_stage(reinterpret_cast<float (*)[DW_CH]>(ls), up, q, H, pl, cq);
+                __syncthreads();
+                dw_walk_prologue<0, 0, 0, 1>(xs, x, ldx, aff, sc, sh, q, H, W, tx, rb, pl, cq, nullptr, nullptr, reinterpret_cast<const float (*)[DW_CH]>(ls), &up, r0);
+            } else
             dw_walk_prologue<LIN, x_bf, ly_bf>(xs, x, ldx, aff, sc, sh, q, H, W, tx, rb, pl, cq, &lin, &lc);
             __syncthreads();
         }
-        f32x4 nx[5];
+        [[maybe_unused]] f32x4 nx[5];
         [[maybe_unused]] f32x4 ny[5];
         const bool more = tx + 1 < q.tiles_x && tile + 1 < q.t1;
-        if (more) {
+        if (more && !UP) {
 #pragma unroll
             for (int it = 0; it < 5; ++it) {
                 const int i = it * 16 + pl;
@@ -430,6 +471,11 @@
 #pragma unroll
             for (int it = 0; it < 5; ++it) {
                 const int i = it * 16 + pl;
+                if constexpr (UP) {
+                    st4(&xs[i >> 3][dw_slot(rb, i & 7)][cq * 4],
+                        dw_up_eval(reinterpret_cast<const float (*)[DW_CH]>(ls), up, q, r0, H, W, i >> 3, tx * DT + 9 + (i & 7), cq));
+                    continue;
+                }
                 const bool inside = dw_walk_inside(q, H, W, i >> 3, tx * DT + 9 + (i & 7));
                 f32x4 v = nx[it];
                 if constexpr (has_lin) v = dw_lin_eval(v, ny[it], inside, lc);
@@ -440,16 +486,20 @@
         if (++tx == q.tiles_x) { tx = 0; rb = 0; } else rb = rb >= 2 ? rb - 2 : rb + 8;
     }
 }
-template <int LIN, int BF>
+template <int LIN, int BF, int UP = 0>
 __global__ __launch_bounds__(256, 3) void dwconv_wgrad_walk_kernel(const float* __restrict__ x, long long ldx, const float* __restrict__ dy,
                                                                long long lddy, float* __restrict__ partials, int N, int H, int W, int C,
-                                                               const float* __restrict__ isc, const float* __restrict__ ish, const DwLin lin) {
+                                                               const float* __restrict__ isc, const float* __restrict__ ish, const DwLin lin,
+                                                               const DwUp up) {
+    static_assert(UP == 0 || (BF & 1) == 0, "the upsampled chunks read an fp32 source");
     constexpr int x_bf = BF & 1, ly_bf = BF & 2;
     __shared__ __attribute__((aligned(16))) float xs[DT + 2][DWR][DW_CH];
+    __shared__ __attribute__((aligned(16))) float ls[UP ? DW_UP_PIX : 1][UP ? DW_CH : 4];
     __shared__ float red[16][DW_CH];
+    [[maybe_unused]] int r0 = 0;
     const int t = threadIdx.x, cq = t & 15, pl = t >> 4;
     DwWalk q;
-    dw_walk_init(q, H, W, C, N, cq);
+    dw_walk_init(q, H, W, C, N, cq, up.ch0, up.nch);
     constexpr bool has_lin = LIN != 0;
     const DwLinC lc = dw_lin_coefs(lin, C, q.c, q.cok);
     f32x4 acc[9];
@@ -477,12 +527,16 @@
     for (long long tile = q.t0; tile < q.t1; ++tile) {
         if (tile == q.t0 || tx == 0) {
             dw_walk_strip(q, tile / q.tiles_x);
-            dw_walk_prologue<0, x_bf, 0>(xs, x, ldx, aff, sc, sh, q, H, W, tx, rb, pl, cq);
+            if constexpr (UP) {
+                r0 = dw_up_stage(reinterpret_cast<float (*)[DW_CH]>(ls), up, q, H, pl, cq);
+                __syncthreads();
+            }
+            dw_walk_prologue<0, x_bf, 0, UP>(xs, x, ldx, aff, sc, sh, q, H, W, tx, rb, pl, cq, nullptr, nullptr, reinterpret_cast<const float (*)[DW_CH]>(ls), &up, r0);
             __syncthreads();
         }
-        f32x4 nx[5];
+        [[maybe_unused]] f32x4 nx[5];
         const bool more = tx + 1 < q.tiles_x && tile + 1 < q.t1;
-        if (more) {
+        if (more && !UP) {
 #pragma unroll
             for (int it = 0; it < 5; ++it) {
                 const int i = it * 16 + pl;
@@ -508,6 +562,10 @@
 #pragma unroll
             for (int it = 0; it < 5; ++it) {
                 const int i = it * 16 + pl;
+                if constexpr (UP)
+                    st4(&xs[i >> 3][dw_slot(rb, i & 7)][cq * 4],
+                        dw_up_eval(reinterpret_cast<const float (*)[DW_CH]>(ls), up, q, r0, H, W, i >> 3, tx * DT + 9 + (i & 7), cq));
+                else
                 st4(&xs[i >> 3][dw_slot(rb, i & 7)][cq * 4],
                     dw_walk_act(nx[it], aff, dw_walk_inside(q, H, W, i >> 3, tx * DT + 9 + (i & 7)), sc, sh));
             }
@@ -525,7 +583,7 @@
             float a = 0.f;
 #pragma unroll
             for (int r = 0; r < 16; ++r) a += red[r][t];
-            if (q.c0 + t < C) partials[((long long)(blockIdx.x / ((C + DW_CH - 1) / DW_CH)) * 9 + k) * C + q.c0 + t] = a;
+            if (q.c0 + t < C) partials[((long long)(blockIdx.x / (up.nch ? up.nch : (C + DW_CH - 1) / DW_CH)) * 9 + k) * C + q.c0 + t] = a;
         }
     }
 }
@@ -651,7 +709,7 @@
     dim3 grid((unsigned)sh_cdiv(M, DW_PIX), (unsigned)sh_cdiv(C, DW_CH));
     if (dil == 1 && H % DT == 0 && W % DT == 0 && dw_walk_on())
         dw_launch_fprop_walk(act_flags, dw_walk_blocks(N, H, W, C) * grid.y, (hipStream_t)stream, x, (long long)ldx, w, y, (long long)ldy, stat_partials, N, H, W, C, 0, in_scale,
-                             in_shift, DwBnb{}, DwLin{}, act_flags);
+                             in_shift, DwBnb{}, DwLin{}, act_flags, DwUp{});
     else if (dil == 1 && H % DT == 0 && W % DT == 0)
         dwconv_tile_kernel<0><<<grid.x * grid.y, 256, 0, (hipStream_t)stream>>>(x, ldx, w, y, ldy, stat_partials, H, W, C, 0, in_scale, in_shift, DwBnb{});
     else
@@ -667,7 +725,7 @@
     dim3 grid((unsigned)sh_cdiv(M, DW_PIX), (unsigned)sh_cdiv(C, DW_CH));
     if (dil == 1 && H % DT == 0 && W % DT == 0 && dw_walk_on())
         dw_launch_dgrad_walk(lin.lin != nullptr, bnb.y != nullptr, (lin.y_bf ? 1 : 0) | (bnb.y_bf ? 2 : 0), dw_walk_blocks(N, H, W, C) * grid.y, (hipStream_t)stream,
-                             dy, (long long)lddy, w, dx, (long long)lddx, (float*)nullptr, N, H, W, C, accumulate, (const float*)nullptr, (const float*)nullptr, bnb, lin, 0);
+                             dy, (long long)lddy, w, dx, (long long)lddx, (float*)nullptr, N, H, W, C, accumulate, (const float*)nullptr, (const float*)nullptr, bnb, lin, 0, DwUp{});
     else if (lin.lin != nullptr || bnb.y_bf) return SH_EUNSUPPORTED;
     else if (dil == 1 && H % DT == 0 && W % DT == 0)
         dwconv_tile_kernel<1><<<grid.x * grid.y, 256, 0, (hipStream_t)stream>>>(dy, lddy, w, dx, lddx, nullptr, H, W, C, accumulate, nullptr, nullptr, bnb);
@@ -703,7 +761,7 @@
     if (dil == 1 && H % DT == 0 && W % DT == 0 && dw_walk_on()) {
         P = (int)dw_walk_blocks(N, H, W, C);
         dw_launch_wgrad_walk(lin != nullptr, act_flags & 3, (unsigned)P * grid.y, (hipStream_t)stream, x, (long long)ldx, dy, (long long)lddy, dw_partials, N, H, W, C, in_scale,
-                             in_shift, DwLin{y_lin, ldyl, lin, (act_flags >> 1) & 1});
+                             in_shift, DwLin{y_lin, ldyl, lin, (act_flags >> 1) & 1}, DwUp{});
     } else if (lin != nullptr) return SH_EUNSUPPORTED;
     else if (dil == 1 && H % DT == 0 && W % DT == 0)
         dwconv_wgrad_tile_kernel<<<grid.x * grid.y, 256, 0, (hipStream_t)stream>>>(x, ldx, dy, lddy, dw_partials, H, W, C, M / (DT * DT), in_scale, in_shift);
@@ -714,3 +772,62 @@
     dwconv_wgrad_reduce_kernel<<<(unsigned)sh_cdiv(9 * C, 64), 256, 0, (hipStream_t)stream>>>(dw_partials, dw, P, C);
     return sh_launch_status();
 }
+
+static bool dw_up_geometry_ok(int N, int h, int w, int H, int W, int A, int C, int dil) {
+    if (!(N > 0 && h > 0 && w > 0 && H > 0 && W > 0 && A > 0 && C >= A && (C & 3) == 0)) return false;
+    if (!(dil == 1 && H % DT == 0 && W % DT == 0 && A % DW_CH == 0 && H >= 2 * h && W >= 2 * w && dw_walk_on())) return false;
+    const float sy = (float)h / (float)H;
+    for (int ty = 0; ty < H / DT; ++ty) {
+        int r0, r1;
+        dw_up_rows(ty, H, h, sy, r0, r1);
+        if ((r1 - r0 + 1) * w > DW_UP_PIX) return false;
+    }
+    return true;
+}
+extern "C" int sh_dwconv_up_ok(int N, int h, int w, int H, int W, int A, int C, int dil) { return dw_up_geometry_ok(N, h, w, H, W, A, C, dil) ? 1 : 0; }
+static bool dw_up_args_ok(const float* low, int ldl, int A, const float* skip, int lds, int C) {
+    return low && ldl >= A && !(ldl & 3) && !((uintptr_t)low & 15) && A > 0 && C >= A &&
+           (C == A || (skip && lds >= C - A && !(lds & 3) && !((uintptr_t)skip & 15)));
+}
+extern "C" int sh_dwconv_fprop_up(const float* low, int ldl, int h, int w, int A, const float* skip, int lds, const float* wt, float* y, int ldy,
+                                  float* stat_partials, int N, int H, int W, int C, int dil, int act_flags, void* stream) {
+    if (!dw_args_ok(low, wt, y, N, H, W, C, dil, ldy, ldy) || h <= 0 || w <= 0 || !dw_up_args_ok(low, ldl, A, skip, lds, C) || (act_flags & ~3)) return SH_EINVAL;
+    if (act_flags || !dw_up_geometry_ok(N, h, w, H, W, A, C, dil)) return SH_EUNSUPPORTED;
+    const int nup = A / DW_CH, nsk = (int)sh_cdiv(C, DW_CH) - nup;
+    const unsigned nb = dw_walk_blocks(N, H, W, C);
+    const DwUp up{low, ldl, h, w, (float)h / (float)H, (float)w / (float)W, 0, nup};
+    dwconv_walk_kernel<0, 0, 0, 0, 1><<<nb * nup, 256, 0, (hipStream_t)stream>>>((const float*)nullptr, 0LL, wt, y, (long long)ldy, stat_partials, N, H, W, C, 0,
+                                                                                (const float*)nullptr, (const float*)nullptr, DwBnb{}, DwLin{}, 0, up);
+    if (nsk > 0) {
+        int rc = sh_launch_status();
+        if (rc != SH_OK) return rc;
+        const unsigned nbs = W / DT >= 8 ? nb * 4 : nb;
+        dwconv_walk_kernel<0, 0, 0, 0><<<nbs * nsk, 256, 0, (hipStream_t)stream>>>(skip - A, (long long)lds, wt, y, (long long)ldy, stat_partials, N, H, W, C, 0,
+                                                                                 (const float*)nullptr, (const float*)nullptr, DwBnb{}, DwLin{}, 0, DwUp{nullptr, 0, 0, 0, 0.f, 0.f, nup, nsk});
+    }
+    return sh_launch_status();
+}
+extern "C" int sh_dwconv_wgrad_up(const float* low, int ldl, int h, int w, int A, const float* skip, int lds, const float* dy, int lddy,
+                                  const float* y_lin, int ldyl, const float* lin, float* dw_partials, float* dw, int N, int H, int W, int C, int dil,
+                                  int act_flags, void* stream) {
+    if (!dw_args_ok(low, dy, dw, N, H, W, C, dil, lddy, lddy) || h <= 0 || w <= 0 || !dw_up_args_ok(low, ldl, A, skip, lds, C) || !dw_partials ||
+        !dw_lin_args_ok(y_lin, ldyl, lin, C) || (act_flags & ~3)) return SH_EINVAL;
+    if (act_flags || !dw_up_geometry_ok(N, h, w, H, W, A, C, dil)) return SH_EUNSUPPORTED;
+    const int nup = A / DW_CH, nsk = (int)sh_cdiv(C, DW_CH) - nup;
+    const int P = (int)dw_walk_blocks(N, H, W, C);
+    const DwUp up{low, ldl, h, w, (float)h / (float)H, (float)w / (float)W, 0, nup}, sk{nullptr, 0, 0, 0, 0.f, 0.f, nup, nsk};
+    const DwLin L{y_lin, ldyl, lin, 0};
+    const float* none = nullptr;
+    hipStream_t st = (hipStream_t)stream;
+    if (lin != nullptr) {
+        dwconv_wgrad_walk_kernel<1, 0, 1><<<(unsigned)P * nup, 256, 0, st>>>(none, 0LL, dy, (long long)lddy, dw_partials, N, H, W, C, none, none, L, up);
+        if (nsk > 0) dwconv_wgrad_walk_kernel<1, 0><<<(unsigned)P * nsk, 256, 0, st>>>(skip - A, (long long)lds, dy, (long long)lddy, dw_partials, N, H, W, C, none, none, L, sk);
+    } else {
+        dwconv_wgrad_walk_kernel<0, 0, 1><<<(unsigned)P * nup, 256, 0, st>>>(none, 0LL, dy, (long long)lddy, dw_partials, N, H, W, C, none, none, L, up);
+        if (nsk > 0) dwconv_wgrad_walk_kernel<0, 0><<<(unsigned)P * nsk, 256, 0, st>>>(skip - A, (long long)lds, dy, (long long)lddy, dw_partials, N, H, W, C, none, none, L, sk);
+    }
+    int rc = sh_launch_status();
+    if (rc != SH_OK) return rc;
+    dwconv_wgrad_reduce_kernel<<<(unsigned)sh_cdiv(9 * C, 64), 256, 0, st>>>(dw_partials, dw, P, C);
+    return sh_launch_status();
+}
diff --git a/seghiero_amd/csrc/loss_common.h b/seghiero_amd/csrc/loss_common.h
--- a/seghiero_amd/csrc/loss_common.h
+++ b/seghiero_amd/csrc/loss_common.h
@@ -4,18 +4,6 @@
 #define IGN 255
 #define LOSS_PIX_PER_BLOCK 1024
 
-struct Lerp { int i0, i1; float w0, w1; };
-__device__ __forceinline__ Lerp lerp_src(int dst, float scale, int in) {
-    float s = scale * ((float)dst + 0.5f) - 0.5f;
-    s = s < 0.f ? 0.f : s;
-    Lerp L;
-    L.i0 = (int)s;
-    if (L.i0 > in - 1) L.i0 = in - 1;
-    L.i1 = L.i0 + (L.i0 < in - 1 ? 1 : 0);
-    L.w1 = s - (float)L.i0;
-    L.w0 = 1.f - L.w1;
-    return L;
-}
 __device__ __forceinline__ void contrib_range(int i, float inv_scale, int out, int& lo, int& hi) {
     lo = (int)floorf(((float)i - 0.5f) * inv_scale - 0.5f);
     hi = (int)ceilf(((float)i + 1.5f) * inv_scale - 0.5f);
diff --git a/seghiero_amd/csrc/pool_resample.hip b/seghiero_amd/csrc/pool_resample.hip
--- a/seghiero_amd/csrc/pool_resample.hip
+++ b/seghiero_amd/csrc/pool_resample.hip
@@ -143,18 +143,6 @@
     return sh_avgpool_bwd(x, y, ldy, N, HW, C, 1.0f, 0, stream);
 }
 
-struct Lerp { int i0, i1; float w0, w1; };
-__device__ __forceinline__ Lerp lerp_src(int dst, float scale, int in) {
-    float s = scale * ((float)dst + 0.5f) - 0.5f;
-    s = s < 0.f ? 0.f : s;
-    Lerp L;
-    L.i0 = (int)s;
-    if (L.i0 > in - 1) L.i0 = in - 1;
-    L.i1 = L.i0 + (L.i0 < in - 1 ? 1 : 0);
-    L.w1 = s - (float)L.i0;
-    L.w0 = 1.f - L.w1;
-    return L;
-}
 __global__ __launch_bounds__(256) void bilinear_fwd_kernel(const float* __restrict__ x, long long ldx, float* __restrict__ y,
                                                            long long ldy, int h, int w, int H, int W, int C4, float sy, float sx,
                                                            long long total, int y_bf) {
diff --git a/seghiero_amd/head.py b/seghiero_amd/head.py
--- a/seghiero_amd/head.py
+++ b/seghiero_amd/head.py
@@ -162,10 +162,15 @@
             if mod.c1_bottleneck is not None:
                 c1 = ops.to_nhwc(c1)
                 c1ch = mod.c1_bottleneck[0].out_channels
-                cat2 = ops.new_act(n, A + c1ch, H1, W1, dev, dtype=stored)
-                _, R["c1"] = L.cba_fwd(c1, mod.c1_bottleneck[0].weight, G1, mod.c1_bottleneck[1], True, training, out=cat2[:, A:])
-                ops.bilinear_fwd(b, cat2[:, :A])
-                xin = cat2
+                if stored == torch.float32 and b.dtype == torch.float32 and ops.upcat_ok(b.shape, (n, c1ch, H1, W1)):
+                    skip = ops.new_act(n, c1ch, H1, W1, dev)
+                    _, R["c1"] = L.cba_fwd(c1, mod.c1_bottleneck[0].weight, G1, mod.c1_bottleneck[1], True, training, out=skip)
+                    xin = ops.UpCat(b, skip)
+                else:
+                    cat2 = ops.new_act(n, A + c1ch, H1, W1, dev, dtype=stored)
+                    _, R["c1"] = L.cba_fwd(c1, mod.c1_bottleneck[0].weight, G1, mod.c1_bottleneck[1], True, training, out=cat2[:, A:])
+                    ops.bilinear_fwd(b, cat2[:, :A])
+                    xin = cat2
             else:
                 xin = b
             for j, ds in enumerate(mod.sep_bottleneck):
diff --git a/seghiero_amd/layers.py b/seghiero_amd/layers.py
--- a/seghiero_amd/layers.py
+++ b/seghiero_amd/layers.py
@@ -231,7 +231,11 @@
     n, c, h, w = x.shape
     y = ops.new_act(n, c, h, w, x.device, dtype=ops.stored_dtype())
     partials = torch.empty((ops.dw_partials_rows(n, h, w), 2, c), device=x.device) if training else None
-    if isinstance(x, Lazy) and x._out is None:
+    if isinstance(x, ops.UpCat):
+        if not (y.dtype == torch.float32 and ops.dwconv_fprop_up(x, weight, y, partials, dil)):
+            x = x.materialize()
+            ops.dwconv_fprop(x, weight, y, partials, dil)
+    elif isinstance(x, Lazy) and x._out is None:
         ops.dwconv_fprop(x.y, weight, y, partials, dil, aff=x.coefs)
     else:
         x = dense(x)
@@ -256,7 +260,10 @@
     dy, dgamma, dbeta, _ = ops.bn_backward(dout, None, rec.y, rec.coefs, W(bn), 2, defer=ops.dw_lin_ok(rec.y.shape, rec.dil),
                                            grad32=True)
     dw = new_grad(rec.weight)
-    if isinstance(rec.x, Lazy) and rec.x._out is None:
+    if isinstance(rec.x, ops.UpCat):
+        if not ops.dwconv_wgrad_up(rec.x, dy, dw, rec.dil, side=True):
+            ops.dwconv_wgrad(rec.x.materialize(), dy, dw, rec.dil, side=True)
+    elif isinstance(rec.x, Lazy) and rec.x._out is None:
         ops.dwconv_wgrad(rec.x.y, dy, dw, rec.dil, side=True, aff=rec.x.coefs)
     else:
         ops.dwconv_wgrad(dense(rec.x), dy, dw, rec.dil, side=True)
diff --git a/seghiero_amd/ops.py b/seghiero_amd/ops.py
--- a/seghiero_amd/ops.py
+++ b/seghiero_amd/ops.py
@@ -688,6 +688,68 @@
     _call("sh_dwconv_fprop", xp, ldx, None if aff is None else _rp(aff, 2), None if aff is None else _rp(aff, 3),
           weight.data_ptr(), yp, ldy, None if partials is None else partials.data_ptr(), n, h, w, c, dil, xb | (yb << 1), _st(),
           key=(None if _PROF is None else f"{n}x{h}x{w} C{c} d{dil}"))
+
+
+FUSE_UPCAT = True
+
+
+class UpCat:
+    __slots__ = ("low", "skip", "_cat")
+
+    def __init__(self, low, skip):
+        self.low, self.skip, self._cat = low, skip, None
+
+    @property
+    def shape(self):
+        n, a = self.low.shape[:2]
+        cs, h, w = self.skip.shape[1:]
+        return torch.Size((n, a + cs, h, w))
+
+    @property
+    def device(self):
+        return self.low.device
+
+    @property
+    def dtype(self):
+        return self.low.dtype
+
+    def materialize(self):
+        if self._cat is None:
+            n, c, h, w = self.shape
+            a = self.low.shape[1]
+            cat = new_act(n, c, h, w, self.device)
+            bilinear_fwd(self.low, cat[:, :a])
+            cat[:, a:].copy_(self.skip)
+            self._cat = cat
+        return self._cat
+
+    def _args(self):
+        lp, ldl = pm(self.low)
+        sp, lds = pm(self.skip)
+        return lp, ldl, self.low.shape[2], self.low.shape[3], self.low.shape[1], sp, lds
+
+
+def upcat_ok(low_shape, skip_shape, dil=1):
+    n, a, h, w = low_shape
+    _, cs, H, W = skip_shape
+    return bool(FUSE_UPCAT and LIB.raw("sh_dwconv_up_ok")(n, h, w, H, W, a, a + cs, dil))
+
+
+def dwconv_fprop_up(x, weight, y, partials, dil=1):
+    n, c, h, w = x.shape
+    yp, ldy, yb = pmx(y)
+    return _call_fused("sh_dwconv_fprop_up", *x._args(), weight.data_ptr(), yp, ldy, None if partials is None else partials.data_ptr(),
+                       n, h, w, c, dil, yb << 1, _st(), key=(None if _PROF is None else f"{n}x{h}x{w} C{c} d{dil} up"))
+
+
+def dwconv_wgrad_up(x, dy, dweight, dil=1, side=False):
+    n, c, h, w = x.shape
+    p = dw_partials_rows(n, h, w)
+    largs, yb = _lin_args(dy)
+    key = None if _PROF is None else f"{n}x{h}x{w} C{c} d{dil} up"
+    launch = lambda: _call_fused("sh_dwconv_wgrad_up", *x._args(), *largs, workspace(p * 9 * c * 4, x.device, "dwwgrad").data_ptr(),
+                                 dweight.data_ptr(), n, h, w, c, dil, yb << 1, _st(), key=key)
+    return _wgrad_launch(side, launch, (x.low, x.skip, dy.g, dweight, dy.y, dy.lin) if isinstance(dy, DeferredDy) else (x.low, x.skip, dy, dweight))
 
 
 def dw_lin_ok(shape, dil):
```

Measured after the change: 487.0 (median of 6 runs). No clear change (+1.0%).
